# friendlymatthew/heif

Hardware: NVIDIA B200
Metric: decoded MP/s (12MP HEIC grid batch) (higher is better)
Workload: dtype u8

## Files before the change

### heif_b200/csrc/cuda/cabac_kernel.cu

```cuda
#include <cuda_runtime.h>

#include <cstdio>
#include <cstdlib>

#include "cabac_parse.cuh"
#include "kernels.h"

namespace heic {
namespace dev {

#if !defined(__CUDA_ARCH__)
extern __shared__ __align__(16) unsigned char heic_cabac_smem[];
#endif

namespace {

constexpr int kMaxRows = 512;
#ifndef HEIC_CABAC_MIN_CTAS
#define HEIC_CABAC_MIN_CTAS 3
#endif

struct CtaShared {
  CabacTabs tabs;
  alignas(16) Arenas arenas;
  int progress[kMaxRows];
  int aborted[32];
  unsigned group_slot[4];
};

static_assert(offsetof(CtaShared, arenas) == kSmemArenasOff, "Parser::arenas() expects the arena pointers right behind the tables");
constexpr size_t kCtaSharedBytes = (sizeof(CtaShared) + 15) & ~(size_t)15;
template <int TILES>
struct ColdBytes {
  static constexpr size_t value = (size_t)Parser<TILES>::CW_COUNT * (TILES == 32 ? 1024 : 64);
};

template <int TILES>
struct SmemSync {
  static constexpr int kSaveStride = 1;
  uint32_t lane, tile;
  int base;
  int use1;

  __device__ __forceinline__ CtaShared* sh() const { return reinterpret_cast<CtaShared*>(heic_cabac_smem); }
  __device__ __forceinline__ volatile int* progress() const { return sh()->progress; }
  __device__ __forceinline__ volatile int* aborted() const { return &sh()->aborted[TILES == 1 ? 0 : lane]; }

  __device__ __forceinline__ bool wait(int row, int n) {
    unsigned ns = 32;
    volatile int* pr = progress();
    if (TILES == 1) {
      while (pr[row] < base + n && *aborted() != use1) {
        __nanosleep(ns);
        if (ns < 2048) ns *= 2;
      }
    } else {
      __syncwarp();
      while (pr[row] < base + n) {
#pragma unroll
        for (int i = 0; i < 16; i++) __nanosleep(2048);
      }
      __syncwarp();
    }
    __threadfence_block();
    return *aborted() != use1;
  }
  __device__ __forceinline__ void publish(int row, int n) {
    __threadfence_block();
    if (TILES == 1) {
      progress()[row] = base + n;
    } else {
      __syncwarp();
      if (lane == 0) progress()[row] = base + n;
    }
  }
  __device__ __forceinline__ uint8_t* save_area(int row) {
    const Arenas& A = sh()->arenas;
    return A.wpp_save + A.tiles[tile].wpp_off + (size_t)row * NUM_CTX_PAD;
  }
  __device__ __forceinline__ void abort(int code) {
    if (code != -100) atomicCAS(&sh()->arenas.status[tile].code, 0, code);
    *aborted() = use1;
    __threadfence_block();
  }
};

}

template <int TILES>
__global__ void __launch_bounds__(TILES == 32 ? 256 : 512, TILES == 32 ? HEIC_CABAC_MIN_CTAS : 1) cabac_kernel(Arenas A, const CabacTabs* __restrict__ gtabs,
                                                    const uint32_t* __restrict__ order, int n_slots, uint32_t n_groups,
                                                    uint32_t* group_counter) {
  extern __shared__ __align__(16) unsigned char smem_raw[];
  CtaShared* sh = reinterpret_cast<CtaShared*>(smem_raw);
  uint8_t* ctx_all = smem_raw + kCtaSharedBytes + ColdBytes<TILES>::value;

  {
    const uint32_t* src = reinterpret_cast<const uint32_t*>(gtabs);
    uint32_t* dst = reinterpret_cast<uint32_t*>(&sh->tabs);
    for (int i = threadIdx.x; i < (int)(sizeof(CabacTabs) / 4); i += blockDim.x) dst[i] = src[i];
    for (int i = threadIdx.x; i < kMaxRows; i += blockDim.x) sh->progress[i] = 0;
    if (threadIdx.x < 32) sh->aborted[threadIdx.x] = 0;
    if (threadIdx.x < 4) sh->group_slot[threadIdx.x] = 0;
    if (threadIdx.x == 0) sh->arenas = A;
  }
  __syncthreads();

  const int slot = threadIdx.x >> 5, lane = threadIdx.x & 31;
  if (TILES == 1 && lane != 0) return;
  for (int use = 0;; use++) {
  uint32_t group = blockIdx.x;
  if (group_counter) {
    uint32_t g = 0;
    if (lane == 0) {
      volatile unsigned* gs = &sh->group_slot[use & 3];
      const unsigned tag = ((unsigned)(use + 1) & 0x7ffu) << 20;
      for (;;) {
        const unsigned e = *gs;
        if ((e & 0x7ff00000u) == tag) {
          if ((e & 0xfffffu) != 0xfffffu) {
            g = e & 0xfffffu;
            break;
          }
          __nanosleep(64);
        } else if (atomicCAS(const_cast<unsigned*>(gs), e, tag | 0xfffffu) == e) {
          g = min(atomicAdd(group_counter, 1u), 0xffffeu);
          *gs = tag | g;
          __threadfence_block();
          break;
        }
      }
    }
    group = __shfl_sync(0xffffffffu, g, 0);
    if (group >= n_groups) break;
  } else if (use > 0) {
    break;
  }
  const uint32_t my = order[group * TILES + (TILES == 1 ? 0 : lane)];
  const bool active = my != 0xffffffffu;
  const uint32_t tile = active ? my : order[group * TILES];
  const TileParams* tp = A.tiles + tile;
  const PicParams* pp = A.pics + tp->pic;

  Parser<TILES> P;
  P.sm = (uint32_t)__cvta_generic_to_shared(smem_raw);
  P.ctx_off = P.sm + (uint32_t)(kCtaSharedBytes + ColdBytes<TILES>::value) + (uint32_t)slot * NUM_CTX_PAD * TILES + (TILES == 1 ? 0u : (uint32_t)lane);
  P.cold_off = P.sm + (uint32_t)kCtaSharedBytes + (TILES == 32 ? threadIdx.x * 4u : (uint32_t)slot * 4u);
  asm volatile("" : "+r"(P.sm), "+r"(P.ctx_off), "+r"(P.cold_off));
  P.cold(Parser<TILES>::CW_TP_LO) = (int)(uint32_t)(unsigned long long)tp;
  P.cold(Parser<TILES>::CW_TP_HI) = (int)(uint32_t)((unsigned long long)tp >> 32);
  P.cold(Parser<TILES>::CW_PP_LO) = (int)(uint32_t)(unsigned long long)pp;
  P.cold(Parser<TILES>::CW_PP_HI) = (int)(uint32_t)((unsigned long long)pp >> 32);
  P.e.data = A.bitstream + tp->bs_off;
  P.err = active ? 0 : -100;

  SmemSync<TILES> sync;
  sync.lane = (uint32_t)lane;
  sync.tile = tile;
  sync.base = use << 12;
  sync.use1 = use + 1;
  if (!active) *sync.aborted() = use + 1;

#if HEIC_CABAC_TRACE
  unsigned long long t_begin;
  asm volatile("mov.u64 %0, %%globaltimer;" : "=l"(t_begin));
#endif
  const uint32_t ctus = parse_rows<TILES>(P, A.substreams + tp->sub_first, slot, n_slots, sync);
#if HEIC_CABAC_TRACE
  {
    unsigned long long t_end;
    asm volatile("mov.u64 %0, %%globaltimer;" : "=l"(t_end));
    const unsigned bins_w = __reduce_add_sync(0xffffffffu, active ? P.e.bins : 0u);
    if (lane == 0) printf("CT %u %u %d %d %llu %llu %u %u\n", blockIdx.x, group, use, slot, t_begin, t_end, bins_w, tp->bs_len);
  }
#endif
  if (active) {
    atomicAdd(&A.status[tile].bins, P.e.bins);
    atomicAdd(&A.status[tile].ctus, ctus);
  }
  }
}

size_t cabac_smem_bytes(int tiles_per_cta, int n_slots) {
  return kCtaSharedBytes + (tiles_per_cta == 32 ? ColdBytes<32>::value : ColdBytes<1>::value) + (size_t)n_slots * NUM_CTX_PAD * tiles_per_cta;
}

cudaError_t launch_cabac(const Arenas& A, const CabacTabs* tabs, const uint32_t* order, uint32_t n_groups,
                         int tiles_per_cta, int n_slots, uint32_t* group_counter, int n_sm, int resident_ctas, cudaStream_t stream) {
  if (!n_groups) return cudaSuccess;
  static const size_t pad = []() { const char* e = getenv("HEIC_B200_CABAC_SMEM_PAD"); return e ? (size_t)atol(e) : (size_t)0; }();
  const size_t smem = cabac_smem_bytes(tiles_per_cta, n_slots) + pad;
  const int threads = 32 * n_slots;
  if (tiles_per_cta == 32) {
    {
      cudaError_t e = cudaFuncSetAttribute(cabac_kernel<32>, cudaFuncAttributeMaxDynamicSharedMemorySize, 200 * 1024);
      if (e != cudaSuccess) return e;
    }
    const uint32_t resident = resident_ctas > 0 ? (uint32_t)resident_ctas : (uint32_t)n_sm * (uint32_t)(HEIC_CABAC_MIN_CTAS * 8 / n_slots);
    if (group_counter && n_groups > resident && n_groups < 0xffff0u)
      cabac_kernel<32><<<resident, threads, smem, stream>>>(A, tabs, order, n_slots, n_groups, group_counter);
    else
      cabac_kernel<32><<<n_groups, threads, smem, stream>>>(A, tabs, order, n_slots, n_groups, nullptr);
  } else {
    cabac_kernel<1><<<n_groups, threads, smem, stream>>>(A, tabs, order, n_slots, n_groups, nullptr);
  }
  return cudaGetLastError();
}

}
}
```

### heif_b200/csrc/cuda/deblock_kernel.cu

```cuda
#include <cuda_runtime.h>

#include "kernels.h"

namespace heic {
namespace dev {

namespace {

__device__ const uint8_t kBetaTable[52] = {0,  0,  0,  0,  0,  0,  0,  0,  0,  0,  0,  0,  0,  0,  0,  0,  6,  7,
                                           8,  9,  10, 11, 12, 13, 14, 15, 16, 17, 18, 20, 22, 24, 26, 28, 30, 32,
                                           34, 36, 38, 40, 42, 44, 46, 48, 50, 52, 54, 56, 58, 60, 62, 64};
__device__ const uint8_t kTcTable[54] = {0, 0, 0, 0, 0, 0, 0, 0, 0, 0, 0,  0,  0,  0,  0,  0,  0,  0,
                                         1, 1, 1, 1, 1, 1, 1, 1, 1, 2, 2,  2,  2,  3,  3,  3,  3,  4,
                                         4, 4, 5, 5, 6, 6, 7, 8, 9, 10, 11, 13, 14, 16, 18, 20, 22, 24};
__device__ const uint8_t kChromaQp[14] = {29, 30, 31, 32, 33, 33, 34, 34, 35, 35, 36, 36, 37, 37};

__device__ __forceinline__ int clip3(int lo, int hi, int v) { return min(hi, max(lo, v)); }
__device__ __forceinline__ int clip8(int v) { return min(255, max(0, v)); }

__device__ __forceinline__ uint32_t interleave4(uint32_t v) {
  v &= 0x0fu;
  v = (v | (v << 2)) & 0x33u;
  v = (v | (v << 1)) & 0x55u;
  return v;
}

struct Pic {
  const uint32_t* tu_map;
  const uint8_t* qp_map;
  int w8, log2_ctb, wctb;
};

__device__ __forceinline__ bool is_tu_edge(const Pic& p, int x, int y, int pos) {
  const int ctb4 = 1 << (p.log2_ctb - 2);
  const int rx = x >> p.log2_ctb, ry = y >> p.log2_ctb;
  const uint32_t z = interleave4((uint32_t)(x >> 2) & (ctb4 - 1)) | (interleave4((uint32_t)(y >> 2) & (ctb4 - 1)) << 1);
  const uint32_t* tu = p.tu_map + (size_t)(ry * p.wctb + rx) * (ctb4 * ctb4);
  const uint32_t w3 = tu[z & ~63u], w2 = tu[z & ~15u];
  const bool in32 = (w3 & 7u) == (TU_ORIGIN | (3u << 1)) && (pos & 31) != 0;
  const bool in16 = (w2 & 7u) == (TU_ORIGIN | (2u << 1)) && (pos & 15) != 0;
  return !(in32 || in16);
}
__device__ __forceinline__ int qp_at(const Pic& p, int x, int y) { return p.qp_map[(y >> 3) * p.w8 + (x >> 3)]; }

__device__ __forceinline__ int dp4(uint32_t samples, uint32_t weights, int acc) {
  int d;
  asm("dp4a.u32.s32 %0, %1, %2, %3;" : "=r"(d) : "r"(samples), "r"(weights), "r"(acc));
  return d;
}
__host__ __device__ constexpr uint32_t W(int a, int b, int c, int d) {
  return ((uint32_t)a & 0xffu) | (((uint32_t)b & 0xffu) << 8) | (((uint32_t)c & 0xffu) << 16) | (((uint32_t)d & 0xffu) << 24);
}
__device__ __forceinline__ int lin(uint32_t P, uint32_t Q, uint32_t wp, uint32_t wq, int c) { return dp4(Q, wq, dp4(P, wp, c)); }

__device__ __forceinline__ bool filter_luma_segment(uint32_t (&rw)[8][2], int qp_sum, int beta_off2, int tc_off2) {
  const int qpl = (qp_sum + 1) >> 1;
  const int beta = kBetaTable[clip3(0, 51, qpl + beta_off2)];
  const int tc = kTcTable[clip3(0, 53, qpl + 2 + tc_off2)];
  const uint32_t P0 = rw[0][0], Q0 = rw[0][1], P3 = rw[3][0], Q3 = rw[3][1];
  const int dp0 = abs(dp4(P0, W(0, 1, -2, 1), 0)), dp3 = abs(dp4(P3, W(0, 1, -2, 1), 0));
  const int dq0 = abs(dp4(Q0, W(1, -2, 1, 0), 0)), dq3 = abs(dp4(Q3, W(1, -2, 1, 0), 0));
  const int dpq0 = dp0 + dq0, dpq3 = dp3 + dq3, dp = dp0 + dp3, dq = dq0 + dq3;
  if (dpq0 + dpq3 >= beta) return false;
  const int tc25 = (5 * tc + 1) >> 1;
  const bool s0 = 2 * dpq0 < (beta >> 2) && abs(dp4(P0, W(1, 0, 0, -1), 0)) + abs(dp4(Q0, W(1, 0, 0, -1), 0)) < (beta >> 3) &&
                  abs(lin(P0, Q0, W(0, 0, 0, 1), W(-1, 0, 0, 0), 0)) < tc25;
  const bool s3 = 2 * dpq3 < (beta >> 2) && abs(dp4(P3, W(1, 0, 0, -1), 0)) + abs(dp4(Q3, W(1, 0, 0, -1), 0)) < (beta >> 3) &&
                  abs(lin(P3, Q3, W(0, 0, 0, 1), W(-1, 0, 0, 0), 0)) < tc25;
  const bool strong = s0 && s3;
  const bool dep = dp < ((beta + (beta >> 1)) >> 3), deq = dq < ((beta + (beta >> 1)) >> 3);
#pragma unroll
  for (int l = 0; l < 4; l++) {
    const uint32_t P = rw[l][0], Q = rw[l][1];
    if (strong) {
      const int t2 = 2 * tc;
      const int e_p0 = clip3(-t2, t2, lin(P, Q, W(0, 1, 2, 2 - 8), W(2, 1, 0, 0), 4) >> 3);
      const int e_p1 = clip3(-t2, t2, lin(P, Q, W(0, 1, 1 - 4, 1), W(1, 0, 0, 0), 2) >> 2);
      const int e_p2 = clip3(-t2, t2, lin(P, Q, W(2, 3 - 8, 1, 1), W(1, 0, 0, 0), 4) >> 3);
      const int e_q0 = clip3(-t2, t2, lin(P, Q, W(0, 0, 1, 2), W(2 - 8, 2, 1, 0), 4) >> 3);
      const int e_q1 = clip3(-t2, t2, lin(P, Q, W(0, 0, 0, 1), W(1, 1 - 4, 1, 0), 2) >> 2);
      const int e_q2 = clip3(-t2, t2, lin(P, Q, W(0, 0, 0, 1), W(1, 1, 3 - 8, 2), 4) >> 3);
      rw[l][0] = P + (uint32_t)e_p2 * 256u + (uint32_t)e_p1 * 65536u + (uint32_t)e_p0 * 16777216u;
      rw[l][1] = Q + (uint32_t)e_q0 + (uint32_t)e_q1 * 256u + (uint32_t)e_q2 * 65536u;
    } else {
      int delta = lin(P, Q, W(0, 0, 3, -9), W(9, -3, 0, 0), 8) >> 4;
      if (abs(delta) < tc * 10) {
        delta = clip3(-tc, tc, delta);
        const int p0 = dp4(P, W(0, 0, 0, 1), 0), q0 = dp4(Q, W(1, 0, 0, 0), 0);
        const int ep = clip8(p0 + delta) - p0, eq = clip8(q0 - delta) - q0;
        uint32_t addp = (uint32_t)ep * 16777216u, addq = (uint32_t)eq;
        if (dep) {
          const int p1 = dp4(P, W(0, 0, 1, 0), 0);
          const int e = clip3(-(tc >> 1), tc >> 1, (((dp4(P, W(0, 1, 0, 1), 1) >> 1) - p1 + delta) >> 1));
          addp += (uint32_t)(clip8(p1 + e) - p1) * 65536u;
        }
        if (deq) {
          const int q1 = dp4(Q, W(0, 1, 0, 0), 0);
          const int e = clip3(-(tc >> 1), tc >> 1, (((dp4(Q, W(1, 0, 1, 0), 1) >> 1) - q1 - delta) >> 1));
          addq += (uint32_t)(clip8(q1 + e) - q1) * 256u;
        }
        rw[l][0] = P + addp;
        rw[l][1] = Q + addq;
      }
    }
  }
  return true;
}

__device__ __forceinline__ bool filter_chroma_segment(uint32_t (&rw)[8][2], int qp_sum, int c_qp_off, int tc_off2) {
  const int qpi = ((qp_sum + 1) >> 1) + c_qp_off;
  const int qpc = qpi < 30 ? qpi : (qpi >= 43 ? qpi - 6 : kChromaQp[qpi - 30]);
  const int tc = kTcTable[clip3(0, 53, qpc + 2 + tc_off2)];
  if (!tc) return false;
#pragma unroll
  for (int l = 0; l < 4; l++) {
    const uint32_t P = rw[l][0], Q = rw[l][1];
    const int delta = clip3(-tc, tc, lin(P, Q, W(0, 0, 1, -4), W(4, -1, 0, 0), 4) >> 3);
    const int p0 = dp4(P, W(0, 0, 0, 1), 0), q0 = dp4(Q, W(1, 0, 0, 0), 0);
    rw[l][0] = P + (uint32_t)(clip8(p0 + delta) - p0) * 16777216u;
    rw[l][1] = Q + (uint32_t)(clip8(q0 - delta) - q0);
  }
  return true;
}

__device__ __forceinline__ void transpose4(uint32_t a, uint32_t b, uint32_t c, uint32_t d, uint32_t& o0, uint32_t& o1, uint32_t& o2, uint32_t& o3) {
  const uint32_t t0 = __byte_perm(a, b, 0x5140), t1 = __byte_perm(c, d, 0x5140);
  const uint32_t t2 = __byte_perm(a, b, 0x7362), t3 = __byte_perm(c, d, 0x7362);
  o0 = __byte_perm(t0, t1, 0x5410);
  o1 = __byte_perm(t0, t1, 0x7632);
  o2 = __byte_perm(t2, t3, 0x5410);
  o3 = __byte_perm(t2, t3, 0x7632);
}
__device__ __forceinline__ void transpose_cell(uint32_t (&rw)[8][2]) {
  uint32_t t[8][2];
  transpose4(rw[0][0], rw[1][0], rw[2][0], rw[3][0], t[0][0], t[1][0], t[2][0], t[3][0]);
  transpose4(rw[4][0], rw[5][0], rw[6][0], rw[7][0], t[0][1], t[1][1], t[2][1], t[3][1]);
  transpose4(rw[0][1], rw[1][1], rw[2][1], rw[3][1], t[4][0], t[5][0], t[6][0], t[7][0]);
  transpose4(rw[4][1], rw[5][1], rw[6][1], rw[7][1], t[4][1], t[5][1], t[6][1], t[7][1]);
#pragma unroll
  for (int r = 0; r < 8; r++) rw[r][0] = t[r][0], rw[r][1] = t[r][1];
}

template <int CIDX>
__device__ __forceinline__ void deblock_cell(const Pic& pic, uint8_t* plane, int pitch, int pw, int ph, int k, int j,
                                             int beta_off2, int tc_off2, int c_qp_off) {
  constexpr int SUB = CIDX ? 1 : 0;
  const int x0 = 8 * k - 4, y0 = 8 * j - 4;
  const bool has_left = k > 0, has_right = 8 * k < pw, has_top = j > 0, has_bottom = 8 * j < ph;
  uint32_t rw[8][2];
#pragma unroll
  for (int r = 0; r < 8; r++) {
    const bool row_ok = r < 4 ? has_top : has_bottom;
    rw[r][0] = rw[r][1] = 0;
    if (row_ok) {
      const uint8_t* row = plane + (size_t)(y0 + r) * pitch;
      if (has_left) rw[r][0] = *reinterpret_cast<const uint32_t*>(row + x0);
      if (has_right) rw[r][1] = *reinterpret_cast<const uint32_t*>(row + x0 + 4);
    }
  }
  const int xe = (8 * k) << SUB, ye = (8 * j) << SUB;
  uint32_t seg_do = 0, seg_qp = 0;
#pragma unroll
  for (int g = 0; g < 4; g++) {
    const bool vert = g < 2;
    const int half = g & 1;
    bool ok;
    if (vert) ok = has_left && has_right && (half == 0 ? has_top : has_bottom);
    else ok = has_top && has_bottom && (half == 0 ? has_left : has_right);
    if (ok) {
      const int xl = vert ? xe : (x0 + 4 * half) << SUB, yl = vert ? (y0 + 4 * half) << SUB : ye;
      seg_qp |= (uint32_t)(qp_at(pic, xl, yl) + (vert ? qp_at(pic, xl - 1, yl) : qp_at(pic, xl, yl - 1))) << (8 * g);
      seg_do |= (is_tu_edge(pic, xl, yl, vert ? xl : yl) ? 1u : 0u) << g;
    }
  }
  if (!seg_do) return;
  bool changed = false;
#pragma unroll 1
  for (int g = 0; g < 4; g++) {
    if ((seg_do >> g) & 1u) {
      const int qp_sum = (int)((seg_qp >> (8 * g)) & 0xffu);
      changed |= CIDX == 0 ? filter_luma_segment(rw, qp_sum, beta_off2, tc_off2) : filter_chroma_segment(rw, qp_sum, c_qp_off, tc_off2);
    }
#pragma unroll
    for (int r = 0; r < 4; r++) {
      uint32_t t0 = rw[r][0], t1 = rw[r][1];
      rw[r][0] = rw[r + 4][0], rw[r][1] = rw[r + 4][1];
      rw[r + 4][0] = t0, rw[r + 4][1] = t1;
    }
    if (g & 1) transpose_cell(rw);
  }
  if (!changed) return;
#pragma unroll
  for (int r = 0; r < 8; r++) {
    const bool row_ok = r < 4 ? has_top : has_bottom;
    if (!row_ok) continue;
    uint8_t* row = plane + (size_t)(y0 + r) * pitch;
    if (has_left) *reinterpret_cast<uint32_t*>(row + x0) = rw[r][0];
    if (has_right) *reinterpret_cast<uint32_t*>(row + x0 + 4) = rw[r][1];
  }
}

#ifndef HEIC_DEBLOCK_MIN_CTAS
#define HEIC_DEBLOCK_MIN_CTAS 12
#endif
template <int KIND>
__global__ void __launch_bounds__(128, HEIC_DEBLOCK_MIN_CTAS) deblock_kernel(Arenas A, uint32_t blocks_per_tile) {
  const uint32_t tile = blockIdx.x / blocks_per_tile;
  const TileParams* tp = A.tiles + tile;
  const PicParams* pp = A.pics + tp->pic;
  if (A.status[tile].code != 0 || tp->deblock_disabled) return;
  if (KIND == 1 && !pp->chroma) return;
  uint32_t g = (blockIdx.x % blocks_per_tile) * blockDim.x + threadIdx.x;
  const int pw = pp->w >> KIND, ph = pp->h >> KIND;
  const uint32_t cx = (uint32_t)((pw + 7) >> 3) + 1, cy = (uint32_t)((ph + 7) >> 3) + 1;
  int cidx = KIND;
  if (g >= cx * cy) {
    if (KIND == 0) return;
    g -= cx * cy;
    cidx = 2;
    if (g >= cx * cy) return;
  }
  const int k = (int)(g % cx), j = (int)(g / cx);
  if (8 * k - 4 >= pw || 8 * j - 4 >= ph) return;
  Pic pic;
  pic.tu_map = A.tu_map + tp->tu_off;
  pic.qp_map = A.qp_map + tp->map8_off;
  pic.w8 = pp->w8;
  pic.log2_ctb = pp->log2_ctb;
  pic.wctb = pp->wctb;
  const int beta_off2 = tp->beta_offset_div2 * 2, tc_off2 = tp->tc_offset_div2 * 2;
  deblock_cell<KIND>(pic, A.recon + tp->plane_off[cidx], KIND ? pp->pitch_c : pp->pitch_y, pw, ph, k, j, beta_off2, tc_off2,
                     cidx == 0 ? 0 : (cidx == 1 ? pp->pps_cb_qp_offset : pp->pps_cr_qp_offset));
}

}

cudaError_t launch_deblock(const Arenas& A, uint32_t max_w, uint32_t max_h, cudaStream_t stream) {
  if (!A.n_tiles) return cudaSuccess;
  const uint32_t cells_y = (((max_w + 7) >> 3) + 1) * (((max_h + 7) >> 3) + 1);
  const uint32_t cells_c = 2 * ((((max_w >> 1) + 7) >> 3) + 1) * ((((max_h >> 1) + 7) >> 3) + 1);
  const uint32_t by = (cells_y + 127) / 128, bc = (cells_c + 127) / 128;
  deblock_kernel<0><<<A.n_tiles * by, 128, 0, stream>>>(A, by);
  deblock_kernel<1><<<A.n_tiles * bc, 128, 0, stream>>>(A, bc);
  return cudaGetLastError();
}

}
}
```

### heif_b200/csrc/cuda/intra_kernel.cu

```cuda
#include <cuda_runtime.h>

#include "kernels.h"

namespace heic {
namespace dev {

namespace {

__constant__ int8_t kIntraPredAngle[35] = {0,   0,   32,  26,  21,  17, 13, 9,  5,  2,  0,  -2, -5, -9, -13, -17, -21, -26,
                                               -32, -26, -21, -17, -13, -9, -5, -2, 0,  2,  5,  9,  13, 17, 21,  26,  32};
__constant__ int16_t kInvAngle[15] = {-4096, -1638, -910, -630, -482, -390, -315, -256,
                                          -315,  -390,  -482, -630, -910, -1638, -4096};

__device__ __forceinline__ uint32_t compact1(uint32_t v) {
  v &= 0x55u;
  v = (v | (v >> 1)) & 0x33u;
  v = (v | (v >> 2)) & 0x0fu;
  return v;
}
__device__ __forceinline__ int clip8(int v) { return min(255, max(0, v)); }

__device__ __forceinline__ void cp_async16s(uint32_t smem_addr, const void* gmem_src) {
  asm volatile("cp.async.cg.shared.global [%0], [%1], 16;\n" ::"r"(smem_addr), "l"(gmem_src) : "memory");
}
__device__ __forceinline__ void cp_async_wait_all() { asm volatile("cp.async.wait_all;\n" ::: "memory"); }

template <class T>
struct SP {
  uint32_t a;
  __device__ __forceinline__ operator T*() const { return reinterpret_cast<T*>(__cvta_shared_to_generic(a)); }
  __device__ __forceinline__ T& operator[](int i) const { return reinterpret_cast<T*>(__cvta_shared_to_generic(a))[i]; }
  __device__ __forceinline__ SP operator+(int i) const { return SP{a + (uint32_t)(i * (int)sizeof(T))}; }
  __device__ __forceinline__ int operator-(SP o) const { return (int)(a - o.a) / (int)sizeof(T); }
};
struct Ctu {
  int w, h, ctb, ctb4, x_ctb, y_ctb;
  SP<uint8_t> buf[3];
  int stride[3];
  SP<uint8_t> ref;
  SP<uint8_t> refa;
  SP<int16_t> res[3];
  SP<uint32_t> tuw;
  int lane;
  int strong_flag;
};
constexpr int kRefSpan = 144, kRefaSpan = 104;
constexpr int kApron = 4;

__device__ __forceinline__ uint32_t pack4(int a, int b, int c, int d) {
  return (uint32_t)a | ((uint32_t)b << 8) | ((uint32_t)c << 16) | ((uint32_t)d << 24);
}

__device__ __forceinline__ uint32_t block_availability(const Ctu& c, int sub, int bx, int by, int log2) {
  const int N = 1 << log2;
  const int units = (c.ctb >> sub) >> log2;
  const int cx = bx >> log2, cy = by >> log2;
  const int X0 = (c.x_ctb >> sub) + bx, Y0 = (c.y_ctb >> sub) + by;
  const bool left_ok = X0 > 0, top_ok = Y0 > 0;
  int n_bl = 0, n_tr = 0;
  if (left_ok && __ffs(cx | units) > __ffs(cy + 1)) n_bl = min(N, max(0, (c.h >> sub) - (Y0 + N)));
  if (top_ok && __ffs(cy | units) >= __ffs(cx + 1)) n_tr = min(N, max(0, (c.w >> sub) - (X0 + N)));
  const int lo = left_ok ? N - n_bl : 2 * N + 1;
  const int hi = top_ok ? 3 * N + n_tr : 2 * N - 1;
  return (uint32_t)lo | ((uint32_t)hi << 8);
}

__device__ __forceinline__ void predict_block(const Ctu& c, bool pair, uint8_t* buf, int buf_delta, int stride, int bx, int by,
                                              int log2, int mode, bool cbf_a, bool cbf_b, const int16_t* __restrict__ resid,
                                              int res_delta, int lo, int hi) {
  const int N = 1 << log2, lane = c.lane;
  const int total = 4 * N, cnt = total + 1;
  uint8_t* ref = c.ref;
  if (log2 == 2) {
    const uint8_t* corner = buf + by * stride + bx + kApron - 1;
    int r = 128, r2 = 128;
    if (lane <= 16 && lo <= hi) {
      const int d = min(max(lane, lo), hi) - 8;
      const int off = d <= 0 ? -d * stride : d;
      r = corner[off];
      if (pair) r2 = corner[off + buf_delta];
    }
    const int x = lane & 3, y = (lane >> 2) & 3;
    const bool luma = !pair;
    int v, v2 = 0;
    const int L = __shfl_sync(0xffffffffu, r, 7 - y), T = __shfl_sync(0xffffffffu, r, 9 + x);
    int L2 = 0, T2 = 0;
    if (pair) L2 = __shfl_sync(0xffffffffu, r2, 7 - y), T2 = __shfl_sync(0xffffffffu, r2, 9 + x);
    if (mode == 0) {
      const int tr = __shfl_sync(0xffffffffu, r, 13), bl = __shfl_sync(0xffffffffu, r, 3);
      v = ((3 - x) * L + (x + 1) * tr + (3 - y) * T + (y + 1) * bl + 4) >> 3;
      if (pair) {
        const int tr2 = __shfl_sync(0xffffffffu, r2, 13), bl2 = __shfl_sync(0xffffffffu, r2, 3);
        v2 = ((3 - x) * L2 + (x + 1) * tr2 + (3 - y) * T2 + (y + 1) * bl2 + 4) >> 3;
      }
    } else if (mode == 1) {
      const bool in_sum = (lane >= 4 && lane <= 7) || (lane >= 9 && lane <= 12);
      const unsigned sums = __reduce_add_sync(0xffffffffu, in_sum ? (unsigned)r | ((unsigned)r2 << 16) : 0u);
      const int dc = ((int)(sums & 0xffffu) + 4) >> 3;
      v = dc;
      v2 = ((int)(sums >> 16) + 4) >> 3;
      if (luma) {
        if (y == 0) v = x == 0 ? (L + 2 * dc + T + 2) >> 2 : (T + 3 * dc + 2) >> 2;
        else if (x == 0) v = (L + 3 * dc + 2) >> 2;
      }
    } else {
      const int angle = kIntraPredAngle[mode];
      const bool vertical = mode >= 18;
      const int dir = vertical ? 1 : -1;
      const int t = ((vertical ? y : x) + 1) * angle, fact = t & 31;
      const int t1 = (vertical ? x : y) + (t >> 5) + 1;
      int la = 8 + dir * t1, lb = la + dir;
      if (angle < 0) {
        const int inv = kInvAngle[mode - 11];
        if (t1 < 0) la = 8 - dir * ((t1 * inv + 128) >> 8);
        if (t1 + 1 < 0) lb = 8 - dir * (((t1 + 1) * inv + 128) >> 8);
      }
      const int a = __shfl_sync(0xffffffffu, r, la), b = __shfl_sync(0xffffffffu, r, lb);
      v = ((32 - fact) * a + fact * b + 16) >> 5;
      if (pair) {
        const int a2 = __shfl_sync(0xffffffffu, r2, la), b2 = __shfl_sync(0xffffffffu, r2, lb);
        v2 = ((32 - fact) * a2 + fact * b2 + 16) >> 5;
      } else if (mode == 26 || mode == 10) {
        const int c0 = __shfl_sync(0xffffffffu, r, 8), t1s = __shfl_sync(0xffffffffu, r, 9), l1s = __shfl_sync(0xffffffffu, r, 7);
        if (mode == 26 && x == 0) v = clip8(t1s + ((L - c0) >> 1));
        if (mode == 10 && y == 0) v = clip8(l1s + ((T - c0) >> 1));
      }
    }
    if (lane < 16) {
      uint8_t* o = buf + (by + 1 + y) * stride + bx + kApron + x;
      if (cbf_a) v = clip8(v + (int)resid[lane]);
      o[0] = (uint8_t)v;
      if (pair) {
        if (cbf_b) v2 = clip8(v2 + (int)resid[res_delta + lane]);
        o[buf_delta] = (uint8_t)v2;
      }
    }
    __syncwarp();
    return;
  }
  {
    const uint8_t* corner = buf + by * stride + bx + kApron - 1;
    const int n_ref = pair ? 2 * cnt : cnt;
    const int lo_d = lo - 2 * N, hi_d = hi - 2 * N;
    if (lo > hi) {
      for (int s = lane; s < 2 * kRefSpan; s += 32) ref[s] = 128;
    } else {
#pragma unroll 1
      for (int s = lane - 2 * N; s < n_ref - 2 * N; s += 32) {
        const bool second = s > 2 * N;
        const int ss = second ? s - cnt : s;
        const int d = min(max(ss, lo_d), hi_d);
        const uint8_t* src = corner + (d <= 0 ? -d * stride : d);
        if (second) src += buf_delta;
        ref[(second ? ss + kRefSpan : ss) + 2 * N] = *src;
      }
    }
  }
  __syncwarp();
  const uint8_t* R = ref;
  if (N > 4 && !pair && mode != 1) {
    const int min_dist = min(abs(mode - 26), abs(mode - 10));
    const int thr = N == 8 ? 7 : (N == 16 ? 1 : 0);
    if (min_dist > thr) {
      const bool strong = N == 32 && c.strong_flag && abs((int)ref[64] + ref[128] - 2 * ref[96]) < 8 &&
                          abs((int)ref[64] + ref[0] - 2 * ref[32]) < 8;
      uint8_t* reff = ref + kRefSpan;
#pragma unroll 1
      for (int s = lane; s <= total; s += 32) {
        int v;
        if (s == 0 || s == total) v = ref[s];
        else if (strong) {
          if (s == 64) v = ref[64];
          else if (s < 64) v = (s * ref[64] + (64 - s) * ref[0] + 32) >> 6;
          else v = ((128 - s) * ref[64] + (s - 64) * ref[128] + 32) >> 6;
        } else {
          v = (ref[s - 1] + 2 * ref[s] + ref[s + 1] + 2) >> 2;
        }
        reff[s] = (uint8_t)v;
      }
      __syncwarp();
      R = reff;
    }
  }
  const int quads = (N * N) >> 2;
  const int n_items = pair ? 2 * quads : quads;
  const int lq = log2 - 2;
  const bool edge = !pair && N < 32;
  uint8_t* out = buf + (by + 1) * stride + bx + kApron;
  int dc_pack = 0;
  const int angle = kIntraPredAngle[mode];
  const bool vertical = mode >= 18;
  if (mode == 1) {
    if (lane < N) {
      dc_pack = (int)R[2 * N - 1 - lane] + R[2 * N + 1 + lane];
      if (pair) dc_pack += ((int)R[kRefSpan + 2 * N - 1 - lane] + R[kRefSpan + 2 * N + 1 + lane]) << 16;
    }
#pragma unroll
    for (int o = 16; o; o >>= 1) dc_pack += __shfl_xor_sync(0xffffffffu, dc_pack, o);
  } else if (mode >= 2) {
    const int top_i = angle < 0 ? N : 2 * N;
    const int dir = vertical ? 1 : -1;
#pragma unroll 1
    for (int second = 0; second < (pair ? 2 : 1); second++) {
      const uint8_t* Rp = R + second * kRefSpan + 2 * N;
      uint8_t* ra = c.refa + second * kRefaSpan;
#pragma unroll 1
      for (int i = lane; i <= top_i; i += 32) ra[i] = Rp[dir * i];
      if (angle < 0) {
        const int last = (N * angle) >> 5;
        const int i = -1 - lane;
        if (last < -1 && i >= last) ra[i] = Rp[-dir * ((i * (int)kInvAngle[mode - 11] + 128) >> 8)];
      }
    }
    __syncwarp();
  }
#pragma unroll 1
  for (int q = lane; q < n_items; q += 32) {
    const int second = q >= quads ? 1 : 0, qq = q - second * quads;
    const int y = qq >> lq, x0 = (qq & ((1 << lq) - 1)) << 2;
    const uint8_t* Rp = R + second * kRefSpan + 2 * N;
    int v0, v1, v2, v3;
    if (mode == 0) {
      const int L = Rp[-1 - y], tr = Rp[1 + N], bl = Rp[-1 - N];
      const int a = N - 1 - y, base = (N - 1 - x0) * L + (x0 + 1) * tr + (y + 1) * bl + N, step = tr - L, sh = log2 + 1;
      v0 = (base + a * Rp[1 + x0]) >> sh;
      v1 = (base + step + a * Rp[2 + x0]) >> sh;
      v2 = (base + 2 * step + a * Rp[3 + x0]) >> sh;
      v3 = (base + 3 * step + a * Rp[4 + x0]) >> sh;
    } else if (mode == 1) {
      const int dc = (((dc_pack >> (16 * second)) & 0xffff) + N) >> (log2 + 1);
      v0 = v1 = v2 = v3 = dc;
      if (edge) {
        if (y == 0) {
          v0 = (Rp[1 + x0] + 3 * dc + 2) >> 2;
          v1 = (Rp[2 + x0] + 3 * dc + 2) >> 2;
          v2 = (Rp[3 + x0] + 3 * dc + 2) >> 2;
          v3 = (Rp[4 + x0] + 3 * dc + 2) >> 2;
          if (x0 == 0) v0 = (Rp[-1] + 2 * dc + Rp[1] + 2) >> 2;
        } else if (x0 == 0) {
          v0 = (Rp[-1 - y] + 3 * dc + 2) >> 2;
        }
      }
    } else {
      const uint8_t* ra = c.refa + second * kRefaSpan;
      if (vertical) {
        const int t = (y + 1) * angle, fact = t & 31;
        const uint8_t* r5 = ra + x0 + (t >> 5) + 1;
        const int a0 = r5[0], a1 = r5[1], a2 = r5[2], a3 = r5[3], a4 = r5[4];
        v0 = ((32 - fact) * a0 + fact * a1 + 16) >> 5;
        v1 = ((32 - fact) * a1 + fact * a2 + 16) >> 5;
        v2 = ((32 - fact) * a2 + fact * a3 + 16) >> 5;
        v3 = ((32 - fact) * a3 + fact * a4 + 16) >> 5;
        if (edge && mode == 26 && x0 == 0) v0 = clip8(Rp[1] + ((Rp[-1 - y] - Rp[0]) >> 1));
      } else {
        const uint8_t* ry = ra + y + 1;
        int t = (x0 + 1) * angle;
        v0 = ((32 - (t & 31)) * ry[t >> 5] + (t & 31) * ry[(t >> 5) + 1] + 16) >> 5;
        t += angle;
        v1 = ((32 - (t & 31)) * ry[t >> 5] + (t & 31) * ry[(t >> 5) + 1] + 16) >> 5;
        t += angle;
        v2 = ((32 - (t & 31)) * ry[t >> 5] + (t & 31) * ry[(t >> 5) + 1] + 16) >> 5;
        t += angle;
        v3 = ((32 - (t & 31)) * ry[t >> 5] + (t & 31) * ry[(t >> 5) + 1] + 16) >> 5;
        if (edge && mode == 10 && y == 0) {
          const int l1 = Rp[-1], c0 = Rp[0];
          v0 = clip8(l1 + ((Rp[1 + x0] - c0) >> 1));
          v1 = clip8(l1 + ((Rp[2 + x0] - c0) >> 1));
          v2 = clip8(l1 + ((Rp[3 + x0] - c0) >> 1));
          v3 = clip8(l1 + ((Rp[4 + x0] - c0) >> 1));
        }
      }
    }
    if (second ? cbf_b : cbf_a) {
      const uint2 r = *reinterpret_cast<const uint2*>(resid + second * res_delta + (qq << 2));
      v0 = clip8(v0 + (int)(int16_t)(r.x & 0xffffu));
      v1 = clip8(v1 + ((int)r.x >> 16));
      v2 = clip8(v2 + (int)(int16_t)(r.y & 0xffffu));
      v3 = clip8(v3 + ((int)r.y >> 16));
    }
    *reinterpret_cast<uint32_t*>(out + second * buf_delta + y * stride + x0) = pack4(v0, v1, v2, v3);
  }
  __syncwarp();
}

struct IntraLayout {
  int res1, res2, tuw, ref, refa, buf0, buf1, buf2;
  int stride_y, stride_c;
  int warp_bytes;
};

#ifndef HEIC_INTRA_MAXNREG
#define HEIC_INTRA_MAXNREG 72
#endif
__global__ void __maxnreg__(HEIC_INTRA_MAXNREG) intra_kernel(Arenas A, const uint32_t* __restrict__ order, int n_slots, IntraLayout L, int clear_coeff) {
  extern __shared__ __align__(16) unsigned char smem_raw[];
  const uint32_t tile = order[blockIdx.x];
  const TileParams* tp = A.tiles + tile;
  const PicParams* pp = A.pics + tp->pic;
  if (A.status[tile].code != 0) {
    if (clear_coeff) {
      uint4* z = reinterpret_cast<uint4*>(A.coeff + tp->coeff_off[0]);
      const size_t n16 = (size_t)pp->n_tu * 24 * 2 / 16;
      for (size_t i = threadIdx.x; i < n16; i += blockDim.x) z[i] = make_uint4(0u, 0u, 0u, 0u);
    }
    return;
  }
  const int wctb = pp->wctb, hctb = pp->hctb;
  volatile int* progress = reinterpret_cast<volatile int*>(smem_raw);
  const int progress_bytes = n_slots > 1 ? ((hctb * 4 + 15) & ~15) : 0;
  if (n_slots > 1) {
    for (int i = threadIdx.x; i < hctb; i += blockDim.x) progress[i] = 0;
    __syncthreads();
  }
  const int slot = threadIdx.x >> 5, lane = threadIdx.x & 31;

  Ctu c;
  c.w = pp->w;
  c.h = pp->h;
  c.ctb = 1 << pp->log2_ctb;
  c.ctb4 = c.ctb >> 2;
  c.lane = lane;
  c.strong_flag = pp->strong_intra_smoothing;
  const int n_planes = pp->chroma ? 3 : 1;
  const int n4sq = c.ctb4 * c.ctb4;
  {
    uint32_t wbase = (uint32_t)progress_bytes + (uint32_t)slot * (uint32_t)L.warp_bytes;
    asm volatile("" : "+r"(wbase));
    uint32_t p = (uint32_t)__cvta_generic_to_shared(smem_raw) + wbase;
    asm volatile("" : "+r"(p));
    c.res[0].a = p;
    c.res[1].a = p + (uint32_t)L.res1;
    c.res[2].a = p + (uint32_t)L.res2;
    c.tuw.a = p + (uint32_t)L.tuw;
    c.ref.a = p + (uint32_t)L.ref;
    c.refa.a = p + (uint32_t)L.refa + 32u;
    c.buf[0].a = p + (uint32_t)L.buf0;
    c.buf[1].a = p + (uint32_t)L.buf1;
    c.buf[2].a = p + (uint32_t)L.buf2;
    c.stride[0] = L.stride_y;
    c.stride[1] = c.stride[2] = L.stride_c;
  }
  const uint32_t* tu_map = A.tu_map + tp->tu_off;
  uint8_t* plane[3] = {A.recon + tp->plane_off[0], A.recon + tp->plane_off[1], A.recon + tp->plane_off[2]};
  const int pitch[3] = {pp->pitch_y, pp->pitch_c, pp->pitch_c};

  for (int ry = slot; ry < hctb; ry += n_slots) {
    for (int rx = 0; rx < wctb; rx++) {
      const uint32_t ctb_addr = (uint32_t)(ry * wctb + rx);
      {
        const char* g0 = reinterpret_cast<const char*>(A.coeff + tp->coeff_off[0] + (size_t)ctb_addr * n4sq * 16);
        for (int i = lane * 16; i < n4sq * 32; i += 512) cp_async16s(c.res[0].a + i, g0 + i);
        if (n_planes == 3) {
          const char* g1 = reinterpret_cast<const char*>(A.coeff + tp->coeff_off[1] + (size_t)ctb_addr * n4sq * 4);
          const char* g2 = reinterpret_cast<const char*>(A.coeff + tp->coeff_off[2] + (size_t)ctb_addr * n4sq * 4);
          for (int i = lane * 16; i < n4sq * 8; i += 512) {
            cp_async16s(c.res[1].a + i, g1 + i);
            cp_async16s(c.res[2].a + i, g2 + i);
          }
        }
        const char* gt = reinterpret_cast<const char*>(tu_map + (size_t)ctb_addr * n4sq);
        for (int i = lane * 16; i < n4sq * 4; i += 512) cp_async16s(c.tuw.a + i, gt + i);
      }
      if (n_slots > 1 && ry > 0) {
        const int need = min(rx + 2, wctb);
        if (lane == 0) {
          unsigned ns = 32;
          while (progress[ry - 1] < need) {
            __nanosleep(ns);
            if (ns < 1024) ns *= 2;
          }
        }
        __syncwarp();
        __threadfence_block();
      }
      c.x_ctb = rx * c.ctb;
      c.y_ctb = ry * c.ctb;
#pragma unroll
      for (int pl = 0; pl < 3; pl++) {
        if (pl >= n_planes) break;
        const int sub = pl ? 1 : 0, cs = c.ctb >> sub, st = c.stride[pl];
        uint8_t* b = c.buf[pl];
        if (rx > 0)
          for (int y = lane; y < cs; y += 32) b[(y + 1) * st + kApron - 1] = b[(y + 1) * st + kApron + cs - 1];
        if (ry > 0) {
          const int wp = c.w >> sub, x0 = (c.x_ctb >> sub) - 1, y0 = (c.y_ctb >> sub) - 1;
          const uint8_t* src = plane[pl] + (size_t)y0 * pitch[pl];
          for (int j = lane; j <= cs / 2; j += 32) {
            const int x = x0 - 3 + 4 * j;
            if (x >= 0 && x < wp) *reinterpret_cast<uint32_t*>(b + kApron - 4 + 4 * j) = __ldcg(reinterpret_cast<const uint32_t*>(src + x));
          }
        }
      }
      cp_async_wait_all();
      __syncwarp();
      if (clear_coeff) {
        const uint4 zero = make_uint4(0u, 0u, 0u, 0u);
        char* g0 = reinterpret_cast<char*>(A.coeff + tp->coeff_off[0] + (size_t)ctb_addr * n4sq * 16);
        for (int i = lane * 16; i < n4sq * 32; i += 512) *reinterpret_cast<uint4*>(g0 + i) = zero;
        if (n_planes == 3) {
          char* g1 = reinterpret_cast<char*>(A.coeff + tp->coeff_off[1] + (size_t)ctb_addr * n4sq * 4);
          char* g2 = reinterpret_cast<char*>(A.coeff + tp->coeff_off[2] + (size_t)ctb_addr * n4sq * 4);
          for (int i = lane * 16; i < n4sq * 8; i += 512) {
            *reinterpret_cast<uint4*>(g1 + i) = zero;
            *reinterpret_cast<uint4*>(g2 + i) = zero;
          }
        }
      }
      {
        const int buf_delta = (int)(c.buf[2] - c.buf[1]), res_delta = (int)(c.res[2] - c.res[1]);
#pragma unroll 1
        for (int base = 0; base < n4sq; base += 32) {
          const int idx_l = base + lane;
          const uint32_t wl = idx_l < n4sq ? c.tuw[idx_l] : 0u;
          uint32_t pa = 0, pb = 0, pc = 0;
          if (wl & TU_ORIGIN) {
            const int lg = (int)tu_log2(wl);
            const int bxl = (int)compact1((uint32_t)idx_l) << 2, byl = (int)compact1((uint32_t)idx_l >> 1) << 2;
            pa = (uint32_t)bxl | ((uint32_t)byl << 6) | ((uint32_t)lg << 12) | (tu_luma_mode(wl) << 15) | ((wl & TU_CBF_Y) ? 1u << 21 : 0u);
            pb = block_availability(c, 0, bxl, byl, lg);
            if ((wl & TU_HAS_CHROMA) && n_planes == 3) {
              const int lgc = lg > 2 ? lg - 1 : 2;
              const int bxc = (lg > 2 ? bxl : bxl - 4) >> 1, byc = (lg > 2 ? byl : byl - 4) >> 1;
              pa |= (1u << 22) | ((wl & TU_CBF_CB) ? 1u << 23 : 0u) | ((wl & TU_CBF_CR) ? 1u << 24 : 0u);
              pb |= block_availability(c, 1, bxc, byc, lgc) << 16;
              pc = tu_chroma_mode(wl) | ((uint32_t)bxc << 6) | ((uint32_t)byc << 12) | ((uint32_t)lgc << 18);
            }
          }
          uint32_t todo = __ballot_sync(0xffffffffu, (wl & TU_ORIGIN) != 0);
          while (todo) {
            const int src = __ffs(todo) - 1;
            todo &= todo - 1;
            const uint32_t a = __shfl_sync(0xffffffffu, pa, src), b = __shfl_sync(0xffffffffu, pb, src);
            const uint32_t cc = __shfl_sync(0xffffffffu, pc, src);
            const int idx = base + src;
            const int n_calls = (int)((a >> 22) & 1u) + 1;
#pragma unroll 1
            for (int k = 0; k < n_calls; k++) {
              const bool pr = k != 0;
              const uint32_t geo = pr ? cc >> 6 : a;
              const uint32_t av = pr ? b >> 16 : b;
              predict_block(c, pr, pr ? c.buf[1] : c.buf[0], pr ? buf_delta : 0, pr ? c.stride[1] : c.stride[0], (int)(geo & 63u),
                            (int)((geo >> 6) & 63u), (int)((geo >> 12) & 7u), (int)((pr ? cc : a >> 15) & 63u), ((a >> (pr ? 23 : 21)) & 1u) != 0,
                            pr && ((a >> 24) & 1u), pr ? c.res[1] + (idx >> 2) * 16 : c.res[0] + idx * 16, pr ? res_delta : 0,
                            (int)(av & 0xffu), (int)((av >> 8) & 0xffu));
            }
          }
        }
      }
#pragma unroll
      for (int pl = 0; pl < 3; pl++) {
        if (pl >= n_planes) break;
        const int sub = pl ? 1 : 0, cs = c.ctb >> sub, st = c.stride[pl];
        const int xo = c.x_ctb >> sub, yo = c.y_ctb >> sub;
        const int wv = min(cs, (c.w >> sub) - xo), hv = min(cs, (c.h >> sub) - yo);
        const int lw = pp->log2_ctb - sub - 2;
        const uint8_t* b = c.buf[pl];
        for (int i = lane; i < (hv << lw); i += 32) {
          const int y = i >> lw, xw = (i & ((1 << lw) - 1)) << 2;
          if (xw < wv)
            *reinterpret_cast<uint32_t*>(plane[pl] + (size_t)(yo + y) * pitch[pl] + xo + xw) =
                *reinterpret_cast<const uint32_t*>(b + (y + 1) * st + kApron + xw);
        }
      }
      if (n_slots > 1) {
        __threadfence_block();
        __syncwarp();
        if (lane == 0) progress[ry] = rx + 1;
      } else {
        __syncwarp();
      }
    }
  }
}

IntraLayout intra_layout(int log2_ctb) {
  const int ctb = 1 << log2_ctb, n4 = (ctb >> 2) * (ctb >> 2);
  IntraLayout L;
  int o = n4 * 16 * 2;
  L.res1 = o;
  o += n4 * 4 * 2;
  L.res2 = o;
  o += n4 * 4 * 2;
  L.tuw = o;
  o += n4 * 4;
  L.ref = o;
  o += 2 * kRefSpan;
  L.refa = o;
  o += 2 * kRefaSpan;
  L.stride_y = 2 * ctb + kApron;
  L.stride_c = ctb + kApron;
  L.buf0 = o;
  o += (ctb + 1) * L.stride_y;
  L.buf1 = o;
  o += (ctb / 2 + 1) * L.stride_c;
  L.buf2 = o;
  o += (ctb / 2 + 1) * L.stride_c;
  L.warp_bytes = (o + 15) & ~15;
  return L;
}

}

cudaError_t launch_intra(const Arenas& A, const uint32_t* order, int max_log2_ctb, int max_hctb, int n_slots, bool clear_coeff,
                         cudaStream_t stream) {
  if (!A.n_tiles) return cudaSuccess;
  const IntraLayout L = intra_layout(max_log2_ctb);
  const size_t smem = (n_slots > 1 ? (((size_t)max_hctb * 4 + 15) & ~(size_t)15) : 0) + (size_t)n_slots * L.warp_bytes;
  if (smem > 48 * 1024) {
    cudaError_t e = cudaFuncSetAttribute(intra_kernel, cudaFuncAttributeMaxDynamicSharedMemorySize, (int)smem);
    if (e != cudaSuccess) return e;
  }
  intra_kernel<<<A.n_tiles, 32 * n_slots, smem, stream>>>(A, order, n_slots, L, clear_coeff ? 1 : 0);
  return cudaGetLastError();
}

}
}
```

### heif_b200/csrc/cuda/kernels.h

```cpp
#pragma once
#include <cuda_runtime.h>

#include "dev_types.h"

namespace heic {
namespace dev {

struct CabacTabs;

size_t cabac_smem_bytes(int tiles_per_cta, int n_slots);
cudaError_t launch_cabac(const Arenas& A, const CabacTabs* tabs, const uint32_t* order, uint32_t n_groups,
                         int tiles_per_cta, int n_slots, uint32_t* group_counter, int n_sm, int resident_ctas ,
                         cudaStream_t stream);

cudaError_t launch_unescape(const Arenas& A, TileParams* tiles, uint32_t* substreams, cudaStream_t stream);
cudaError_t launch_transform(const Arenas& A, uint32_t max_tu_per_tile, int max_log2_tb, int n_sm, cudaStream_t stream);
size_t transform_list_layout(size_t total_tu, uint32_t off[LIST_CLASSES]);
int transform_launches(int max_log2_tb);

cudaError_t launch_intra(const Arenas& A, const uint32_t* order, int max_log2_ctb, int max_hctb, int n_slots, bool clear_coeff,
                         cudaStream_t stream);

cudaError_t launch_deblock(const Arenas& A, uint32_t max_w, uint32_t max_h, cudaStream_t stream);

cudaError_t launch_sao(const Arenas& A, uint32_t max_pitch, uint32_t max_h, cudaStream_t stream);
cudaError_t launch_sao_sparse(const Arenas& A, int max_hctb, cudaStream_t stream);

struct ColorJob {
  const uint8_t* planes;
  uint64_t tile_stride;
  uint64_t cb_off, cr_off;
  uint32_t pitch_y, pitch_c;
  uint32_t tile_w, tile_h;
  uint32_t grid_cols, grid_rows;
  uint32_t out_w, out_h;
  uint32_t n_images;
  uint32_t chroma;
  uint32_t full_range, matrix_coeffs;
  uint32_t orientation;
  uint8_t* rgb;
  uint64_t pitch, image_stride;
  uint32_t fused;
  const uint8_t* planes_sao;
  const uint32_t* sao;
  uint32_t sao_stride;
  uint32_t log2_ctb, wctb;
};
struct ColorWindow {
  uint32_t crop_x, crop_y, crop_w, crop_h;
  uint32_t win_x, win_y;
};
cudaError_t launch_color(const ColorJob& job, const ColorWindow& win, cudaStream_t stream);

}
}
```

### heif_b200/csrc/cuda/pipeline.cu

```cuda
#include <cuda_runtime.h>

#include <chrono>
#include <cstdio>
#include <cstdlib>

#include <algorithm>
#include <cstdlib>
#include <cstring>
#include <map>
#include <memory>
#include <string>
#include <tuple>
#include <vector>

#include "../host/capi_common.h"
#include "../host/heic_decoder.h"
#include "cabac_tables.h"
#include "host_params.h"
#include "kernels.h"

using namespace heic;
using namespace heic::dev;

namespace {

[[noreturn]] void cuda_fail(cudaError_t e, const char* what) {
  int code = (e == cudaErrorNoDevice || e == cudaErrorInsufficientDriver || e == cudaErrorInvalidDevice) ? HEIC_E_NO_DEVICE
             : (e == cudaErrorMemoryAllocation)                                                          ? HEIC_E_NOMEM
                                                                                                         : HEIC_E_CUDA;
  bail(code, std::string(what) + ": " + cudaGetErrorString(e));
}
#define CU(call)                               \
  do {                                         \
    cudaError_t e__ = (call);                  \
    if (e__ != cudaSuccess) cuda_fail(e__, #call); \
  } while (0)

struct DevBuf {
  void* p = nullptr;
  size_t cap = 0;
  void ensure(size_t n) {
    if (n <= cap) return;
    if (p) cudaFree(p);
    p = nullptr;
    cap = 0;
    size_t want = n + n / 8 + 256;
    CU(cudaMalloc(&p, want));
    cap = want;
  }
  ~DevBuf() {
    if (p) cudaFree(p);
  }
};
struct PinnedBuf {
  void* p = nullptr;
  size_t cap = 0;
  void ensure(size_t n) {
    if (n <= cap) return;
    if (p) cudaFreeHost(p);
    p = nullptr;
    cap = 0;
    size_t want = n + n / 8 + 256;
    CU(cudaMallocHost(&p, want));
    cap = want;
  }
  ~PinnedBuf() {
    if (p) cudaFreeHost(p);
  }
};

size_t up(size_t v, size_t a) { return (v + a - 1) / a * a; }

int env_int(const char* name, int dflt) {
  const char* s = std::getenv(name);
  return (s && *s) ? std::atoi(s) : dflt;
}

}

struct heic_b200_job {
  heic_b200_ctx* ctx = nullptr;
  heic_tile_status* status = nullptr;
  std::vector<heic_tile_status> local;
  size_t n_tiles = 0;
};

struct PipePending {
  heic_b200_job* job = nullptr;
  size_t tile0 = 0, n_tiles = 0;
  cudaEvent_t ev[5] = {};
  double host_ms = 0;
};

struct heic_b200_ctx {
  int device = 0;
  int n_sm = 148;
  cudaStream_t stream = nullptr;
  CabacTabs* d_tabs = nullptr;
  uint64_t launches = 0;
  int cabac_tiles_per_cta = 32;
  int cabac_slots = 0;
  int low_latency_tiles = 384;
  int cabac_group_factor = 1;
  int intra_slots = 0;
  int intra_single_warp_tiles = 2048;
  int cabac_group_cap_pct = 0;
  int cabac_plain_sort = 0;
  int cabac_resident = 0;
  int cabac_persistent = 1;
  int fuse_sao = 1;
  static constexpr int kPipe = 16;
  int pipe_chunk = 0;
  int pipe_slots = 0;
  cudaEvent_t trace_base = nullptr;
  int pipe_order = 1;
  cudaEvent_t ev_cabac = nullptr, ev_d2h = nullptr;
  bool d2h_recorded = false;
  cudaStream_t pipe_stream[kPipe] = {};
  std::unique_ptr<heic_b200_batch> pipe_batch[kPipe];
  PipePending pipe_pending[kPipe];
  uint32_t pipe_next = 0;
  ~heic_b200_ctx();
};

struct ImageInfo {
  uint32_t first_tile, n_tiles, pic;
  uint32_t grid_rows, grid_cols, out_w, out_h, rot_w, rot_h;
  uint32_t tile_w, tile_h, win_x, win_y;
  uint32_t crop_x, crop_y, crop_w, crop_h, orientation;
  uint32_t full_range, matrix_coeffs;
};

namespace {

struct TileWindow {
  uint32_t x, y, w, h;
};

void image_geometry(const heic_image_desc& im, PicParams& pp, TileWindow& tw, uint32_t& out_w, uint32_t& out_h) {
  if (!im.tiles || im.n_tiles == 0 || im.n_tiles != im.grid_rows * im.grid_cols)
    bail(HEIC_E_INVALID_ARG, "image descriptor: n_tiles must equal grid_rows * grid_cols");
  make_pic_params(im.sps, im.pps, pp);
  tw = {0, 0, (uint32_t)pp.w, (uint32_t)pp.h};
  if (im.sps.conformance_window_flag) {
    const uint64_t sub = pp.chroma ? 2 : 1;
    const uint64_t l = sub * im.sps.conf_win_left_offset, r = sub * im.sps.conf_win_right_offset;
    const uint64_t t = sub * im.sps.conf_win_top_offset, b = sub * im.sps.conf_win_bottom_offset;
    if (l + r >= (uint64_t)pp.w || t + b >= (uint64_t)pp.h) bail(HEIC_E_BITSTREAM, "conformance window is empty");
    tw = {(uint32_t)l, (uint32_t)t, (uint32_t)(pp.w - l - r), (uint32_t)(pp.h - t - b)};
  }
  const uint64_t mosaic_w = (uint64_t)im.grid_cols * tw.w, mosaic_h = (uint64_t)im.grid_rows * tw.h;
  const uint64_t ow = im.output_width ? im.output_width : mosaic_w, oh = im.output_height ? im.output_height : mosaic_h;
  if (ow > mosaic_w || oh > mosaic_h) bail(HEIC_E_BITSTREAM, "grid canvas is larger than the tile mosaic");
  out_w = (uint32_t)ow;
  out_h = (uint32_t)oh;
}

void check_transform(const heic_image_transform& x, uint32_t out_w, uint32_t out_h) {
  if (x.orientation > 7 || !x.crop_w || !x.crop_h || (uint64_t)x.crop_x + x.crop_w > out_w || (uint64_t)x.crop_y + x.crop_h > out_h)
    bail(HEIC_E_INVALID_ARG, "image transform: crop rectangle not inside the canvas, or orientation above 7");
}

std::vector<heic_image_transform> canvas_transforms(const heic_image_desc* imgs, uint32_t n_imgs, int32_t apply_transforms) {
  if (!imgs) bail(HEIC_E_INVALID_ARG, "null argument");
  std::vector<heic_image_transform> x(n_imgs);
  for (uint32_t i = 0; i < n_imgs; i++) {
    PicParams pp;
    TileWindow tw;
    uint32_t ow, oh;
    image_geometry(imgs[i], pp, tw, ow, oh);
    x[i] = {0, 0, ow, oh, apply_transforms ? (imgs[i].rotation_ccw_quarter_turns & 3u) : 0u};
  }
  return x;
}

}

struct CabacClass {
  int n_slots, hctb;
  uint32_t order_off, n_groups, n_tiles;
};

struct heic_b200_batch {
  heic_b200_ctx* ctx = nullptr;
  cudaStream_t stream = nullptr;
  int tiles_per_cta = 32;
  std::vector<PicParams> pics;
  std::vector<ScalingSet> scaling;
  std::vector<TileParams> tiles;
  std::vector<ImageInfo> images;
  std::vector<uint32_t> substreams, order, heavy_first;
  std::vector<CabacClass> classes;
  size_t raw_bytes = 0;
  bool any_plain = false;
  size_t bs_bytes = 0, tu_words = 0, coeff_elems = 0, plane_bytes = 0, map4_bytes = 0, map8_bytes = 0, sao_words = 0, wpp_bytes = 0;
  size_t rgb_pitch = 0, rgb_image_stride = 0;
  uint32_t max_tu = 0, max_w = 0, max_h = 0, max_pitch = 0;
  int max_log2_ctb = 4, max_log2_tb = 2, intra_slots = 1, max_hctb = 1;
  uint32_t stages_run = 0;
  bool final_stale = false;
  bool coeff_clean = false;
  PinnedBuf h_bitstream, h_status, h_params;
  size_t off_sub = 0, off_order = 0, off_heavy = 0, off_pics = 0, off_tiles = 0, off_scaling = 0;
  DevBuf d_bitstream, d_params, d_tu, d_coeff, d_recon, d_final, d_ipm, d_ctd,
      d_qp, d_sao, d_wpp, d_status, d_rgb, d_list, d_list_count, d_raw, d_counters;
  PinnedBuf h_raw;
  uint32_t list_off[LIST_CLASSES] = {};
  Arenas arenas() const {
    Arenas a;
    a.bitstream = (const uint8_t*)d_bitstream.p;
    a.raw = (const uint8_t*)d_raw.p;
    const uint8_t* pb = (const uint8_t*)d_params.p;
    a.substreams = (const uint32_t*)(pb + off_sub);
    a.pics = (const PicParams*)(pb + off_pics);
    a.tiles = (const TileParams*)(pb + off_tiles);
    a.scaling = (const ScalingSet*)(pb + off_scaling);
    a.tu_map = (uint32_t*)d_tu.p;
    a.coeff = (int16_t*)d_coeff.p;
    a.recon = (uint8_t*)d_recon.p;
    a.final_ = (uint8_t*)d_final.p;
    a.ipm = (uint8_t*)d_ipm.p;
    a.ct_depth = (uint8_t*)d_ctd.p;
    a.qp_map = (uint8_t*)d_qp.p;
    a.sao = (uint32_t*)d_sao.p;
    a.wpp_save = (uint8_t*)d_wpp.p;
    a.status = (TileStatusDev*)d_status.p;
    a.n_tiles = (uint32_t)tiles.size();
    a.tu_list = (uint2_t*)d_list.p;
    a.list_count = (uint32_t*)d_list_count.p;
    for (int k = 0; k < LIST_CLASSES; k++) a.list_off[k] = list_off[k];
    return a;
  }
  void load(const heic_image_desc* imgs, const heic_image_transform* xforms, uint32_t n_imgs, bool with_rgb);
  void run(uint32_t mask);
};

heic_b200_ctx::~heic_b200_ctx() {
  if (trace_base) cudaEventDestroy(trace_base);
  if (ev_cabac) cudaEventDestroy(ev_cabac);
  if (ev_d2h) cudaEventDestroy(ev_d2h);
  for (int i = 0; i < kPipe; i++) {
    for (cudaEvent_t e : pipe_pending[i].ev)
      if (e) cudaEventDestroy(e);
    pipe_batch[i].reset();
    if (pipe_stream[i]) cudaStreamDestroy(pipe_stream[i]);
  }
  if (d_tabs) cudaFree(d_tabs);
  if (stream) cudaStreamDestroy(stream);
}

void heic_b200_batch::load(const heic_image_desc* imgs, const heic_image_transform* xforms, uint32_t n_imgs, bool with_rgb) {
  pics.clear();
  scaling.clear();
  tiles.clear();
  images.clear();
  substreams.clear();
  order.clear();
  heavy_first.clear();
  classes.clear();
  raw_bytes = 0;
  any_plain = false;
  bs_bytes = tu_words = coeff_elems = plane_bytes = map4_bytes = map8_bytes = sao_words = wpp_bytes = 0;
  max_tu = max_w = max_h = max_pitch = 0;
  max_log2_ctb = 4;
  max_log2_tb = 2;
  intra_slots = 1;
  max_hctb = 1;
  stages_run = 0;
  size_t max_rgb_rows = 0, max_rgb_pitch = 0, n_tiles_hint = 0;
  for (uint32_t i = 0; i < n_imgs; i++) n_tiles_hint += imgs[i].n_tiles;
  for (uint32_t i = 0; i < n_imgs; i++) {
    const heic_image_desc& im = imgs[i];
    if (!im.tiles || im.n_tiles == 0 || im.n_tiles != im.grid_rows * im.grid_cols)
      bail(HEIC_E_INVALID_ARG, "image descriptor: n_tiles must equal grid_rows * grid_cols");
    PicParams pp;
    TileWindow win;
    uint32_t out_w, out_h;
    image_geometry(im, pp, win, out_w, out_h);
    const heic_image_transform& xf = xforms[i];
    check_transform(xf, out_w, out_h);
    ScalingSet ss;
    build_scaling_set(im.sps, im.pps, ss);
    size_t s = 0;
    for (; s < scaling.size(); s++)
      if (!std::memcmp(&scaling[s], &ss, sizeof ss)) break;
    if (s == scaling.size()) scaling.push_back(ss);
    pp.scaling_set = (int)s;
    if (pics.empty() || std::memcmp(&pics.back(), &pp, sizeof pp)) pics.push_back(pp);
    const uint32_t pic = (uint32_t)pics.size() - 1;
    ImageInfo info;
    info.first_tile = (uint32_t)tiles.size();
    info.n_tiles = im.n_tiles;
    info.pic = pic;
    info.grid_rows = im.grid_rows;
    info.grid_cols = im.grid_cols;
    info.out_w = out_w;
    info.out_h = out_h;
    info.tile_w = win.w;
    info.tile_h = win.h;
    info.win_x = win.x;
    info.win_y = win.y;
    info.crop_x = xf.crop_x;
    info.crop_y = xf.crop_y;
    info.crop_w = xf.crop_w;
    info.crop_h = xf.crop_h;
    info.orientation = xf.orientation;
    info.rot_w = (xf.orientation & 1u) ? xf.crop_h : xf.crop_w;
    info.rot_h = (xf.orientation & 1u) ? xf.crop_w : xf.crop_h;
    info.full_range = im.sps.vui_parameters_present_flag ? im.sps.video_full_range_flag : 0u;
    info.matrix_coeffs = im.sps.vui_parameters_present_flag ? im.sps.matrix_coeffs : 2u;
    images.push_back(info);
    const size_t pitch = up((size_t)info.rot_w * 3, 16);
    max_rgb_pitch = std::max(max_rgb_pitch, pitch);
    max_rgb_rows = std::max(max_rgb_rows, (size_t)info.rot_h);
    const int ctb4 = 1 << (pp.log2_ctb - 2);
    for (uint32_t t = 0; t < im.n_tiles; t++) {
      TileParams tp;
      std::memset(&tp, 0, sizeof tp);
      make_tile_params(pp, im.pps, im.tiles[t], tp);
      tp.pic = pic;
      tp.image = i;
      tp.tile_in_image = t;
      tp.bs_off = (uint32_t)bs_bytes;
      bs_bytes = up(bs_bytes + tp.bs_len + 8, 16);
      tp.escaped = im.tiles[t].escaped ? 1u : 0u;
      if (tp.escaped) {
        tp.raw_off = raw_bytes;
        raw_bytes = up(raw_bytes + tp.bs_len + 8, 16);
      } else {
        any_plain = true;
      }
      if (bs_bytes > 0xfff00000ull) bail(HEIC_E_UNSUPPORTED, "more than 4 GiB of slice data in one batch");
      tp.sub_first = (uint32_t)substreams.size();
      for (uint32_t k = 0; k < tp.n_sub; k++) substreams.push_back(im.tiles[t].header.substream_offset[k]);
      tp.tu_off = tu_words;
      tu_words += (size_t)pp.n_tu;
      tp.coeff_off[0] = coeff_elems;
      tp.coeff_off[1] = tp.coeff_off[0] + (size_t)pp.n_tu * 16;
      tp.coeff_off[2] = tp.coeff_off[1] + (size_t)pp.n_tu * 4;
      coeff_elems = tp.coeff_off[2] + (size_t)pp.n_tu * 4;
      const size_t ysz = (size_t)pp.pitch_y * (size_t)pp.h, csz = (size_t)pp.pitch_c * (size_t)(pp.h >> 1);
      tp.plane_off[0] = plane_bytes;
      tp.plane_off[1] = tp.plane_off[0] + ysz;
      tp.plane_off[2] = tp.plane_off[1] + csz;
      plane_bytes = up(tp.plane_off[2] + csz, 256);
      tp.map4_off = map4_bytes;
      map4_bytes = up(map4_bytes + (size_t)pp.w4 * pp.h4, 64);
      tp.map8_off = map8_bytes;
      map8_bytes = up(map8_bytes + (size_t)pp.w8 * pp.h8, 64);
      tp.sao_off = sao_words;
      sao_words += (size_t)pp.wctb * pp.hctb * 4;
      tp.wpp_off = wpp_bytes;
      wpp_bytes += (size_t)pp.hctb * NUM_CTX_PAD;
      tiles.push_back(tp);
      (void)ctb4;
    }
    max_tu = std::max(max_tu, (uint32_t)pp.n_tu);
    max_w = std::max(max_w, (uint32_t)pp.w);
    max_h = std::max(max_h, (uint32_t)pp.h);
    max_pitch = std::max(max_pitch, (uint32_t)pp.pitch_y);
    max_log2_ctb = std::max(max_log2_ctb, pp.log2_ctb);
    max_log2_tb = std::max(max_log2_tb, pp.log2_max_tb);
    max_hctb = std::max(max_hctb, pp.hctb);
    intra_slots = std::max(intra_slots, std::min(8, std::min(pp.hctb, (pp.wctb + 1) / 2 + 1)));
  }
  rgb_pitch = max_rgb_pitch;
  rgb_image_stride = up(max_rgb_pitch * max_rgb_rows, 256);
  if (tiles.size() >= (1u << 24)) bail(HEIC_E_UNSUPPORTED, "more than 2^24 tiles in one batch (the transform lists keep the tile index in 24 bits)");

  tiles_per_cta = (ctx->cabac_tiles_per_cta == 32 && n_tiles_hint > (size_t)ctx->low_latency_tiles) ? 32 : 1;
  const int tpc = tiles_per_cta;
  std::vector<uint64_t> fingerprint(tiles.size(), 0);
  {
    size_t t = 0;
    for (uint32_t i = 0; i < n_imgs; i++)
      for (uint32_t k = 0; k < imgs[i].n_tiles; k++, t++) {
        const uint8_t* p = imgs[i].tiles[k].rbsp;
        const size_t len = imgs[i].tiles[k].rbsp_len;
        uint64_t h = 0x9e3779b97f4a7c15ull ^ len;
        if (len >= 8)
          for (int q = 0; q < 4; q++) {
            uint64_t w8;
            std::memcpy(&w8, p + (len - 8) * q / 3, 8);
            h = (h ^ w8) * 0xbf58476d1ce4e5b9ull;
            h ^= h >> 29;
          }
        fingerprint[t] = h;
      }
  }
  std::map<std::tuple<int, int, int, int>, std::vector<uint32_t>> by_shape;
  for (uint32_t t = 0; t < tiles.size(); t++) {
    const PicParams& pp = pics[tiles[t].pic];
    by_shape[std::make_tuple(pp.wpp, pp.wctb, pp.hctb, pp.log2_ctb)].push_back(t);
  }
  for (auto& kv : by_shape) {
    std::vector<uint32_t>& v = kv.second;
    std::stable_sort(v.begin(), v.end(), [&](uint32_t a, uint32_t b) {
      return tiles[a].bs_len != tiles[b].bs_len ? tiles[a].bs_len > tiles[b].bs_len : fingerprint[a] < fingerprint[b];
    });
    const int wpp = std::get<0>(kv.first), wctb = std::get<1>(kv.first), hctb = std::get<2>(kv.first);
    CabacClass c;
    c.n_slots = wpp ? std::max(1, std::min(hctb, (wctb + 1) / 2)) : 1;
    if (ctx->cabac_slots > 0 && wpp) c.n_slots = std::min(hctb, ctx->cabac_slots);
    c.n_slots = std::min(c.n_slots, tpc == 32 ? 8 : 16);
    c.order_off = (uint32_t)order.size();
    c.n_groups = 0;
    if (tpc == 1) {
      for (uint32_t t : v) order.push_back(t);
      c.n_groups = (uint32_t)v.size();
    } else {
      if (ctx->cabac_group_factor == 1) {
        struct Run {
          size_t first, left;
        };
        std::vector<Run> runs;
        for (size_t i = 0; i < v.size();) {
          size_t j = i + 1;
          while (!ctx->cabac_plain_sort && j < v.size() && tiles[v[j]].bs_len == tiles[v[i]].bs_len && fingerprint[v[j]] == fingerprint[v[i]]) j++;
          runs.push_back({i, j - i});
          i = j;
        }
        uint64_t cap = ~0ull;
        if (ctx->cabac_group_cap_pct > 0) {
          uint64_t total = 0;
          for (uint32_t t : v) total += tiles[t].bs_len;
          cap = total / (uint64_t)(ctx->n_sm * 3) * (uint64_t)ctx->cabac_group_cap_pct / 100u;
        }
        size_t head = 0;
        while (head < runs.size()) {
          int n = 0;
          uint64_t wsum = 0;
          for (size_t r = head; r < runs.size() && n < tpc; r++) {
            if (!runs[r].left) continue;
            if (n > 0 && wsum + tiles[v[runs[r].first]].bs_len > cap) break;
            wsum += tiles[v[runs[r].first]].bs_len;
            order.push_back(v[runs[r].first++]);
            runs[r].left--;
            n++;
          }
          while (head < runs.size() && !runs[head].left) head++;
          if (!n) break;
          for (; n < tpc; n++) order.push_back(0xffffffffu);
          c.n_groups++;
        }
      } else {
        uint64_t total = 0;
        for (uint32_t t : v) total += tiles[t].bs_len;
        const uint64_t target_groups = std::max<uint64_t>(1, (uint64_t)ctx->cabac_group_factor * ((v.size() + tpc - 1) / tpc));
        const uint64_t w_target = std::max<uint64_t>(1, total / target_groups);
        size_t i = 0;
        while (i < v.size()) {
          uint64_t wsum = 0;
          int n = 0;
          while (i < v.size() && n < tpc && (n == 0 || wsum + tiles[v[i]].bs_len <= w_target)) {
            wsum += tiles[v[i]].bs_len;
            order.push_back(v[i]);
            i++;
            n++;
          }
          for (; n < tpc; n++) order.push_back(0xffffffffu);
          c.n_groups++;
        }
      }
    }
    c.hctb = hctb;
    c.n_tiles = (uint32_t)v.size();
    classes.push_back(c);
  }

  heavy_first.resize(tiles.size());
  for (uint32_t t = 0; t < tiles.size(); t++) heavy_first[t] = t;
  std::stable_sort(heavy_first.begin(), heavy_first.end(), [&](uint32_t a, uint32_t b) { return tiles[a].bs_len > tiles[b].bs_len; });

  cudaStream_t st = stream;
  if (any_plain) h_bitstream.ensure(bs_bytes + 16);
  if (raw_bytes) h_raw.ensure(raw_bytes + 16);
  {
    size_t t = 0;
    uint8_t* hb = (uint8_t*)h_bitstream.p;
    uint8_t* hr = (uint8_t*)h_raw.p;
    for (uint32_t i = 0; i < n_imgs; i++)
      for (uint32_t k = 0; k < imgs[i].n_tiles; k++, t++) {
        const size_t len = imgs[i].tiles[k].rbsp_len;
        if (tiles[t].escaped) {
          std::memcpy(hr + tiles[t].raw_off, imgs[i].tiles[k].rbsp, len);
          std::memset(hr + tiles[t].raw_off + len, 0, up(len + 8, 16) - len);
          continue;
        }
        std::memcpy(hb + tiles[t].bs_off, imgs[i].tiles[k].rbsp, len);
        const size_t end = tiles[t].bs_off + len;
        const size_t next = t + 1 < tiles.size() ? tiles[t + 1].bs_off : bs_bytes + 16;
        std::memset(hb + end, 0, next - end);
      }
  }
  off_sub = 0;
  off_order = up(off_sub + substreams.size() * 4, 256);
  off_heavy = up(off_order + order.size() * 4, 256);
  off_pics = up(off_heavy + heavy_first.size() * 4, 256);
  off_tiles = up(off_pics + pics.size() * sizeof(PicParams), 256);
  off_scaling = up(off_tiles + tiles.size() * sizeof(TileParams), 256);
  const size_t params_bytes = up(off_scaling + scaling.size() * sizeof(ScalingSet), 256);
  h_params.ensure(params_bytes);
  {
    uint8_t* hp = (uint8_t*)h_params.p;
    std::memcpy(hp + off_sub, substreams.data(), substreams.size() * 4);
    std::memcpy(hp + off_order, order.data(), order.size() * 4);
    std::memcpy(hp + off_heavy, heavy_first.data(), heavy_first.size() * 4);
    std::memcpy(hp + off_pics, pics.data(), pics.size() * sizeof(PicParams));
    std::memcpy(hp + off_tiles, tiles.data(), tiles.size() * sizeof(TileParams));
    std::memcpy(hp + off_scaling, scaling.data(), scaling.size() * sizeof(ScalingSet));
  }
  d_bitstream.ensure(bs_bytes + 16);
  d_params.ensure(params_bytes);
  d_tu.ensure(tu_words * 4);
  if (tu_words >= (1ull << 31)) bail(HEIC_E_UNSUPPORTED, "batch too large: more than 2^31 4x4 blocks in one load");
  d_list.ensure(transform_list_layout(tu_words, list_off) * sizeof(uint2_t));
  d_list_count.ensure(LIST_CLASSES * LIST_COUNT_STRIDE * sizeof(uint32_t));
  if (coeff_elems * 2 > d_coeff.cap) coeff_clean = false;
  d_coeff.ensure(coeff_elems * 2);
  d_recon.ensure(plane_bytes);
  d_final.ensure(plane_bytes);
  d_ipm.ensure(map4_bytes);
  d_ctd.ensure(map8_bytes);
  d_qp.ensure(map8_bytes);
  d_sao.ensure(sao_words * 4);
  d_wpp.ensure(wpp_bytes);
  d_status.ensure(tiles.size() * sizeof(TileStatusDev));
  h_status.ensure(tiles.size() * sizeof(TileStatusDev));
  if (with_rgb) d_rgb.ensure(rgb_image_stride * images.size());
  d_raw.ensure(raw_bytes ? raw_bytes + 16 : 0);
  if (any_plain) CU(cudaMemcpyAsync(d_bitstream.p, h_bitstream.p, bs_bytes + 16, cudaMemcpyHostToDevice, st));
  if (raw_bytes) CU(cudaMemcpyAsync(d_raw.p, h_raw.p, raw_bytes + 16, cudaMemcpyHostToDevice, st));
  CU(cudaMemcpyAsync(d_params.p, h_params.p, params_bytes, cudaMemcpyHostToDevice, st));
}

void heic_b200_batch::run(uint32_t mask) {
  cudaStream_t st = stream;
  const Arenas A = arenas();
  if (!A.n_tiles) return;
  if (mask & HEIC_STAGE_CABAC) {
    CU(cudaMemsetAsync(d_tu.p, 0, tu_words * 4, st));
    if (!coeff_clean) CU(cudaMemsetAsync(d_coeff.p, 0, coeff_elems * 2, st));
    coeff_clean = false;
    CU(cudaMemsetAsync(d_status.p, 0, tiles.size() * sizeof(TileStatusDev), st));
    CU(cudaMemsetAsync(d_sao.p, 0, sao_words * 4, st));
    if (raw_bytes) {
      uint8_t* pb = (uint8_t*)d_params.p;
      CU(launch_unescape(A, (TileParams*)(pb + off_tiles), (uint32_t*)(pb + off_sub), st));
      ctx->launches++;
    }
    constexpr size_t kCounters = 64;
    d_counters.ensure(kCounters * sizeof(uint32_t));
    const bool persistent = ctx->cabac_persistent && classes.size() <= kCounters;
    if (persistent) CU(cudaMemsetAsync(d_counters.p, 0, kCounters * sizeof(uint32_t), st));
    size_t ci = 0;
    for (const CabacClass& c : classes) {
      CU(launch_cabac(A, ctx->d_tabs, (const uint32_t*)((const uint8_t*)d_params.p + off_order) + c.order_off, c.n_groups, tiles_per_cta,
                      c.n_slots, (persistent && c.hctb > c.n_slots) ? (uint32_t*)d_counters.p + ci : nullptr, ctx->n_sm, ctx->cabac_resident, st));
      ctx->launches++;
      ci++;
    }
  }
  if (mask & HEIC_STAGE_TRANSFORM) {
    CU(launch_transform(A, max_tu, max_log2_tb, ctx->n_sm, st));
    ctx->launches += transform_launches(max_log2_tb);
  }
  if (mask & HEIC_STAGE_INTRA) {
    int slots = tiles.size() >= (size_t)ctx->intra_single_warp_tiles ? 1 : intra_slots;
    if (ctx->intra_slots > 0) slots = std::min(ctx->intra_slots, std::max(1, max_hctb));
    CU(launch_intra(A, (const uint32_t*)((const uint8_t*)d_params.p + off_heavy), max_log2_ctb, max_hctb, slots, true, st));
    coeff_clean = true;
    ctx->launches++;
  }
  if (mask & HEIC_STAGE_DEBLOCK) {
    CU(launch_deblock(A, max_w, max_h, st));
    ctx->launches += 2;
  }
  const bool fuse = ctx->fuse_sao && (mask & HEIC_STAGE_SAO) && (mask & HEIC_STAGE_COLOR) && d_rgb.p;
  if ((mask & HEIC_STAGE_SAO) && !fuse) {
    CU(launch_sao(A, max_pitch, max_h, st));
    final_stale = false;
    ctx->launches++;
  }
  if (fuse) {
    CU(launch_sao_sparse(A, max_hctb, st));
    ctx->launches++;
    final_stale = true;
  }
  if ((mask & HEIC_STAGE_COLOR) && d_rgb.p) {
    size_t i = 0;
    while (i < images.size()) {
      size_t j = i + 1;
      auto same = [&](const ImageInfo& a, const ImageInfo& b) {
        return a.pic == b.pic && a.n_tiles == b.n_tiles && a.grid_cols == b.grid_cols && a.out_w == b.out_w &&
               a.out_h == b.out_h && a.tile_w == b.tile_w && a.tile_h == b.tile_h && a.win_x == b.win_x && a.win_y == b.win_y &&
               a.crop_x == b.crop_x && a.crop_y == b.crop_y && a.crop_w == b.crop_w && a.crop_h == b.crop_h &&
               a.orientation == b.orientation && a.full_range == b.full_range && a.matrix_coeffs == b.matrix_coeffs;
      };
      while (j < images.size() && same(images[i], images[j])) j++;
      const ImageInfo& im = images[i];
      const PicParams& pp = pics[im.pic];
      const TileParams& t0 = tiles[im.first_tile];
      ColorJob job;
      job.planes = (const uint8_t*)(fuse ? d_recon.p : d_final.p) + t0.plane_off[0];
      job.fused = fuse ? 1u : 0u;
      job.planes_sao = (const uint8_t*)d_final.p + t0.plane_off[0];
      job.sao = A.sao + t0.sao_off;
      job.sao_stride = (uint32_t)((size_t)pp.wctb * pp.hctb * 4);
      job.log2_ctb = (uint32_t)pp.log2_ctb;
      job.wctb = (uint32_t)pp.wctb;
      job.tile_stride = im.n_tiles > 1 || j - i > 1
                            ? (size_t)(tiles[std::min<size_t>(im.first_tile + 1, tiles.size() - 1)].plane_off[0] - t0.plane_off[0])
                            : 0;
      job.cb_off = t0.plane_off[1] - t0.plane_off[0];
      job.cr_off = t0.plane_off[2] - t0.plane_off[0];
      job.pitch_y = (uint32_t)pp.pitch_y;
      job.pitch_c = (uint32_t)pp.pitch_c;
      job.tile_w = im.tile_w;
      job.tile_h = im.tile_h;
      job.grid_cols = im.grid_cols;
      job.grid_rows = im.grid_rows;
      job.out_w = im.out_w;
      job.out_h = im.out_h;
      job.n_images = (uint32_t)(j - i);
      job.chroma = (uint32_t)pp.chroma;
      job.full_range = im.full_range;
      job.matrix_coeffs = im.matrix_coeffs;
      job.orientation = im.orientation;
      job.rgb = (uint8_t*)d_rgb.p + i * rgb_image_stride;
      job.pitch = rgb_pitch;
      job.image_stride = rgb_image_stride;
      const ColorWindow win = {im.crop_x, im.crop_y, im.crop_w, im.crop_h, im.win_x, im.win_y};
      CU(launch_color(job, win, st));
      ctx->launches++;
      i = j;
    }
  }
  stages_run |= mask;
}

namespace {

void collect_status(heic_b200_batch* b, heic_tile_status* status) {
  cudaStream_t st = b->stream;
  const size_t n = b->tiles.size();
  CU(cudaMemcpyAsync(b->h_status.p, b->d_status.p, n * sizeof(TileStatusDev), cudaMemcpyDeviceToHost, st));
  CU(cudaStreamSynchronize(st));
  const TileStatusDev* s = (const TileStatusDev*)b->h_status.p;
  for (size_t i = 0; i < n; i++) {
    status[i].code = s[i].code;
    status[i].bins_decoded = s[i].bins;
    status[i].ctus_decoded = s[i].ctus;
    status[i].reserved = 0;
  }
}

}

extern "C" {

int32_t heic_b200_create(int32_t device, heic_b200_ctx** out_ctx) {
  return static_cast<int32_t>(guard([&]() -> int64_t {
    if (!out_ctx) bail(HEIC_E_INVALID_ARG, "null argument");
    *out_ctx = nullptr;
    int n = 0;
    cudaError_t e = cudaGetDeviceCount(&n);
    if (e != cudaSuccess || n == 0)
      bail(HEIC_E_NO_DEVICE, std::string("no CUDA device (this library has no CPU path): ") + cudaGetErrorString(e));
    auto c = std::make_unique<heic_b200_ctx>();
    if (device < 0) CU(cudaGetDevice(&c->device));
    else c->device = device;
    CU(cudaSetDevice(c->device));
    cudaDeviceProp prop;
    CU(cudaGetDeviceProperties(&prop, c->device));
    if (prop.major < 10)
      bail(HEIC_E_NO_DEVICE, std::string("device '") + prop.name + "' is not sm_100 class; the kernels are built for sm_100a only");
    CU(cudaDeviceGetAttribute(&c->n_sm, cudaDevAttrMultiProcessorCount, c->device));
    CU(cudaStreamCreateWithFlags(&c->stream, cudaStreamNonBlocking));
    static CabacTabs tabs;
    build_cabac_tabs(tabs);
    CU(cudaMalloc((void**)&c->d_tabs, sizeof(CabacTabs)));
    CU(cudaMemcpy(c->d_tabs, &tabs, sizeof tabs, cudaMemcpyHostToDevice));
    c->cabac_tiles_per_cta = env_int("HEIC_B200_CABAC_TILES_PER_CTA", 32) == 1 ? 1 : 32;
    c->cabac_slots = env_int("HEIC_B200_CABAC_SLOTS", 0);
    c->intra_slots = std::min(8, env_int("HEIC_B200_INTRA_SLOTS", 0));
    c->cabac_group_factor = std::max(1, env_int("HEIC_B200_CABAC_GROUP_FACTOR", 1));
    c->pipe_chunk = std::max(0, env_int("HEIC_B200_PIPE_CHUNK", 0));
    c->low_latency_tiles = env_int("HEIC_B200_LOW_LATENCY_TILES", 384);
    c->fuse_sao = env_int("HEIC_B200_FUSE_SAO", 1) != 0;
    c->cabac_persistent = env_int("HEIC_B200_CABAC_PERSISTENT", 1) != 0;
    c->cabac_resident = std::max(0, env_int("HEIC_B200_CABAC_RESIDENT", 0));
    c->cabac_plain_sort = env_int("HEIC_B200_CABAC_PLAIN_SORT", 0) != 0;
    c->cabac_group_cap_pct = std::max(0, env_int("HEIC_B200_CABAC_GROUP_CAP", 0));
    c->pipe_slots = std::min((int)heic_b200_ctx::kPipe, std::max(0, env_int("HEIC_B200_PIPE_SLOTS", 0)));
    c->pipe_order = env_int("HEIC_B200_PIPE_ORDER", 1) != 0;
    *out_ctx = c.release();
    return 0;
  }));
}

void heic_b200_destroy(heic_b200_ctx* ctx) {
  if (!ctx) return;
  cudaSetDevice(ctx->device);
  if (ctx->stream) cudaStreamSynchronize(ctx->stream);
  delete ctx;
}

uint64_t heic_b200_launch_count(const heic_b200_ctx* ctx) { return ctx ? ctx->launches : 0; }

int32_t heic_b200_batch_create(heic_b200_ctx* ctx, const heic_image_desc* imgs, uint32_t n_imgs, heic_b200_batch** out) {
  return heic_b200_batch_create_ex(ctx, imgs, n_imgs, 0, out);
}

static int64_t batch_create(heic_b200_ctx* ctx, const heic_image_desc* imgs, const heic_image_transform* xforms, uint32_t n_imgs,
                            heic_b200_batch** out) {
  if (!ctx || !imgs || !xforms || !out || !n_imgs) bail(HEIC_E_INVALID_ARG, "null argument");
  *out = nullptr;
  CU(cudaSetDevice(ctx->device));
  auto b = std::make_unique<heic_b200_batch>();
  b->ctx = ctx;
  b->stream = ctx->stream;
  b->load(imgs, xforms, n_imgs, true);
  CU(cudaStreamSynchronize(ctx->stream));
  *out = b.release();
  return 0;
}

int32_t heic_b200_batch_create_ex(heic_b200_ctx* ctx, const heic_image_desc* imgs, uint32_t n_imgs, int32_t apply_transforms,
                                  heic_b200_batch** out) {
  return static_cast<int32_t>(guard([&]() -> int64_t {
    if (!ctx || !imgs || !out || !n_imgs) bail(HEIC_E_INVALID_ARG, "null argument");
    *out = nullptr;
    return batch_create(ctx, imgs, canvas_transforms(imgs, n_imgs, apply_transforms).data(), n_imgs, out);
  }));
}

int32_t heic_b200_batch_create_transformed(heic_b200_ctx* ctx, const heic_image_desc* imgs, const heic_image_transform* xforms,
                                           uint32_t n_imgs, heic_b200_batch** out) {
  return static_cast<int32_t>(guard([&]() -> int64_t { return batch_create(ctx, imgs, xforms, n_imgs, out); }));
}

void heic_b200_batch_destroy(heic_b200_batch* b) {
  if (!b) return;
  cudaSetDevice(b->ctx->device);
  cudaStreamSynchronize(b->stream);
  delete b;
}

int32_t heic_b200_batch_run_stages(heic_b200_batch* b, uint32_t stage_mask) {
  return static_cast<int32_t>(guard([&]() -> int64_t {
    if (!b) bail(HEIC_E_INVALID_ARG, "null batch");
    CU(cudaSetDevice(b->ctx->device));
    b->run(stage_mask & HEIC_STAGE_ALL);
    return 0;
  }));
}

int32_t heic_b200_batch_decode(heic_b200_batch* b) { return heic_b200_batch_run_stages(b, HEIC_STAGE_ALL); }

int32_t heic_b200_batch_sync(heic_b200_batch* b) {
  return static_cast<int32_t>(guard([&]() -> int64_t {
    if (!b) bail(HEIC_E_INVALID_ARG, "null batch");
    CU(cudaStreamSynchronize(b->stream));
    return 0;
  }));
}

void* heic_b200_batch_stream(heic_b200_batch* b) { return b ? (void*)b->stream : nullptr; }

int32_t heic_b200_batch_rgb(heic_b200_batch* b, void** dev_ptr, size_t* pitch, size_t* image_stride) {
  if (!b) {
    set_last_error("null batch");
    return HEIC_E_INVALID_ARG;
  }
  if (dev_ptr) *dev_ptr = b->d_rgb.p;
  if (pitch) *pitch = b->rgb_pitch;
  if (image_stride) *image_stride = b->rgb_image_stride;
  return 0;
}

int32_t heic_b200_batch_download_rgb(heic_b200_batch* b, uint8_t* rgb_out, size_t pitch, size_t image_stride) {
  return static_cast<int32_t>(guard([&]() -> int64_t {
    if (!b || !rgb_out) bail(HEIC_E_INVALID_ARG, "null argument");
    CU(cudaSetDevice(b->ctx->device));
    cudaStream_t st = b->stream;
    for (size_t i = 0; i < b->images.size(); i++) {
      const ImageInfo& im = b->images[i];
      if (pitch < (size_t)im.rot_w * 3) bail(HEIC_E_INVALID_ARG, "output pitch smaller than a row of RGB");
      if (b->images.size() > 1 && (size_t)im.rot_h * pitch > image_stride)
        bail(HEIC_E_INVALID_ARG, "image_stride smaller than one image (rows x pitch)");
    }
    for (size_t i = 0; i < b->images.size(); i++) {
      const ImageInfo& im = b->images[i];
      CU(cudaMemcpy2DAsync(rgb_out + i * image_stride, pitch, (const uint8_t*)b->d_rgb.p + i * b->rgb_image_stride,
                           b->rgb_pitch, (size_t)im.rot_w * 3, im.rot_h, cudaMemcpyDeviceToHost, st));
    }
    CU(cudaStreamSynchronize(st));
    return 0;
  }));
}

int32_t heic_b200_batch_download_image(heic_b200_batch* b, uint32_t image_index, uint8_t* rgb_out, size_t pitch) {
  return static_cast<int32_t>(guard([&]() -> int64_t {
    if (!b || !rgb_out || image_index >= b->images.size()) bail(HEIC_E_INVALID_ARG, "invalid argument");
    if (!b->d_rgb.p) bail(HEIC_E_INVALID_ARG, "the batch has no RGB output");
    CU(cudaSetDevice(b->ctx->device));
    const ImageInfo& im = b->images[image_index];
    if (pitch < (size_t)im.rot_w * 3) bail(HEIC_E_INVALID_ARG, "output pitch smaller than a row of RGB");
    CU(cudaMemcpy2DAsync(rgb_out, pitch, (const uint8_t*)b->d_rgb.p + (size_t)image_index * b->rgb_image_stride, b->rgb_pitch,
                         (size_t)im.rot_w * 3, im.rot_h, cudaMemcpyDeviceToHost, b->stream));
    CU(cudaStreamSynchronize(b->stream));
    return 0;
  }));
}

int32_t heic_b200_batch_status(heic_b200_batch* b, heic_tile_status* status) {
  return static_cast<int32_t>(guard([&]() -> int64_t {
    if (!b || !status) bail(HEIC_E_INVALID_ARG, "null argument");
    CU(cudaSetDevice(b->ctx->device));
    collect_status(b, status);
    return 0;
  }));
}

uint32_t heic_b200_batch_tile_count(const heic_b200_batch* b) { return b ? (uint32_t)b->tiles.size() : 0; }

size_t heic_b200_batch_cabac_order(const heic_b200_batch* b, uint32_t* out, size_t cap, uint32_t* tiles_per_group) {
  if (!b) return 0;
  if (tiles_per_group) *tiles_per_group = (uint32_t)b->tiles_per_cta;
  if (out)
    for (size_t i = 0; i < b->order.size() && i < cap; i++) out[i] = b->order[i];
  return b->order.size();
}

int32_t heic_b200_batch_dump_tile(heic_b200_batch* b, uint32_t tile_index, heic_tile_dump* dump) {
  return static_cast<int32_t>(guard([&]() -> int64_t {
    if (!b || !dump || tile_index >= b->tiles.size()) bail(HEIC_E_INVALID_ARG, "invalid argument");
    CU(cudaSetDevice(b->ctx->device));
    cudaStream_t st = b->stream;
    CU(cudaStreamSynchronize(st));
    const TileParams& tp = b->tiles[tile_index];
    const PicParams& pp = b->pics[tp.pic];
    if (dump->tu_map) {
      if (dump->tu_map_len < (uint32_t)pp.n_tu) bail(HEIC_E_INVALID_ARG, "tu_map buffer too small");
      CU(cudaMemcpy(dump->tu_map, (const uint32_t*)b->d_tu.p + tp.tu_off, (size_t)pp.n_tu * 4, cudaMemcpyDeviceToHost));
    }
    for (int c = 0; c < (pp.chroma ? 3 : 1); c++)
      if (dump->coeff[c]) {
        const size_t n = (size_t)pp.n_tu * (c ? 4 : 16);
        if (dump->coeff_len[c] < n) bail(HEIC_E_INVALID_ARG, "coefficient buffer too small");
        CU(cudaMemcpy(dump->coeff[c], (const int16_t*)b->d_coeff.p + tp.coeff_off[c], n * 2, cudaMemcpyDeviceToHost));
      }
    if (dump->qp_map) {
      const size_t wq = (size_t)pp.w >> 3, hq = (size_t)pp.h >> 3;
      if (dump->qp_map_len < wq * hq) bail(HEIC_E_INVALID_ARG, "qp_map buffer too small");
      CU(cudaMemcpy2D(dump->qp_map, wq, (const uint8_t*)b->d_qp.p + tp.map8_off, (size_t)pp.w8, wq, hq, cudaMemcpyDeviceToHost));
    }
    if (dump->sao) {
      const size_t n = (size_t)pp.wctb * pp.hctb * 4;
      if (dump->sao_len < n) bail(HEIC_E_INVALID_ARG, "sao buffer too small");
      CU(cudaMemcpy(dump->sao, (const uint32_t*)b->d_sao.p + tp.sao_off, n * 4, cudaMemcpyDeviceToHost));
    }
    if ((b->stages_run & HEIC_STAGE_SAO) && b->final_stale) {
      CU(launch_sao(b->arenas(), b->max_pitch, b->max_h, b->stream));
      CU(cudaStreamSynchronize(b->stream));
      b->final_stale = false;
    }
    const uint8_t* src = (const uint8_t*)((b->stages_run & HEIC_STAGE_SAO) ? b->d_final.p : b->d_recon.p);
    for (int c = 0; c < (pp.chroma ? 3 : 1); c++)
      if (dump->plane[c]) {
        const size_t w = (size_t)pp.w >> (c ? 1 : 0), h = (size_t)pp.h >> (c ? 1 : 0);
        if (dump->plane_len[c] < w * h) bail(HEIC_E_INVALID_ARG, "plane buffer too small");
        CU(cudaMemcpy2D(dump->plane[c], w, src + tp.plane_off[c], (size_t)(c ? pp.pitch_c : pp.pitch_y), w, h,
                        cudaMemcpyDeviceToHost));
      }
    return 0;
  }));
}

static void harvest_slot(heic_b200_ctx* ctx, int slot) {
  PipePending& pd = ctx->pipe_pending[slot];
  if (!pd.job) return;
  heic_b200_batch* b = ctx->pipe_batch[slot].get();
  CU(cudaStreamSynchronize(b->stream));
  if (pd.ev[0] && ctx->trace_base) {
    float t[5];
    for (int k = 0; k < 5; k++) cudaEventElapsedTime(&t[k], ctx->trace_base, pd.ev[k]);
    std::fprintf(stderr, "[heic_b200] chunk slot %2d tiles %6zu: queued %8.1f  h2d %8.1f  cabac %8.1f  kernels %8.1f  d2h %8.1f ms\n", slot,
                 pd.n_tiles, t[0], t[1], t[2], t[3], t[4]);
  }
  const TileStatusDev* s = (const TileStatusDev*)b->h_status.p;
  heic_tile_status* out = pd.job->status + pd.tile0;
  for (size_t i = 0; i < pd.n_tiles; i++) {
    out[i].code = s[i].code;
    out[i].bins_decoded = s[i].bins;
    out[i].ctus_decoded = s[i].ctus;
    out[i].reserved = 0;
  }
  pd.job = nullptr;
}

static heic_b200_job* submit_grids(heic_b200_ctx* ctx, const heic_image_desc* imgs, const heic_image_transform* xforms,
                                   uint32_t n_imgs, uint8_t* rgb_out, size_t pitch, size_t image_stride, uint8_t* y_out,
                                   uint8_t* cb_out, uint8_t* cr_out, heic_tile_status* status) {
  if (!ctx || !imgs || !xforms || !n_imgs) bail(HEIC_E_INVALID_ARG, "null argument");
  CU(cudaSetDevice(ctx->device));
  std::vector<size_t> first_tile(n_imgs + 1, 0), y_off(n_imgs + 1, 0), c_off(n_imgs + 1, 0);
  for (uint32_t i = 0; i < n_imgs; i++) {
    const heic_image_desc& im = imgs[i];
    PicParams pp;
    TileWindow win;
    uint32_t out_w, out_h;
    image_geometry(im, pp, win, out_w, out_h);
    check_transform(xforms[i], out_w, out_h);
    TileParams tp;
    for (uint32_t t = 0; t < im.n_tiles; t++) make_tile_params(pp, im.pps, im.tiles[t], tp);
    const size_t ow = out_w, oh = out_h;
    if (rgb_out) {
      const bool turn = xforms[i].orientation & 1u;
      const size_t rw = turn ? xforms[i].crop_h : xforms[i].crop_w, rh = turn ? xforms[i].crop_w : xforms[i].crop_h;
      if (pitch < rw * 3) bail(HEIC_E_INVALID_ARG, "output pitch smaller than a row of RGB");
      if (n_imgs > 1 && rh * pitch > image_stride) bail(HEIC_E_INVALID_ARG, "image_stride smaller than one image (rows x pitch)");
    }
    first_tile[i + 1] = first_tile[i] + im.n_tiles;
    y_off[i + 1] = y_off[i] + ow * oh;
    c_off[i + 1] = c_off[i] + ((ow + 1) / 2) * ((oh + 1) / 2);
  }
  static const bool trace = std::getenv("HEIC_B200_TRACE") != nullptr;
  static const bool trace2 = trace && std::atoi(std::getenv("HEIC_B200_TRACE")) >= 2;
  using clk = std::chrono::steady_clock;
  auto ms_since = [](clk::time_point t0) { return std::chrono::duration<double, std::milli>(clk::now() - t0).count(); };
  const clk::time_point t_call = clk::now();
  double t_wait = 0, t_load = 0, t_run = 0;
  auto job = std::make_unique<heic_b200_job>();
  job->ctx = ctx;
  job->n_tiles = first_tile[n_imgs];
  job->status = status;
  if (!job->status) {
    job->local.resize(job->n_tiles);
    job->status = job->local.data();
  }
  uint32_t chunk = (uint32_t)std::max(0, ctx->pipe_chunk);
  if (chunk == 0) {
    const uint32_t parts = (n_imgs + 295u) / 296u;
    chunk = (n_imgs + parts - 1) / parts;
  }
  const uint32_t n_slots_use = ctx->pipe_slots > 0 ? (uint32_t)ctx->pipe_slots : std::min(8u, std::max(3u, 900u / chunk));
  std::vector<uint32_t> chunk_start;
  for (uint32_t i = 0; i < n_imgs; i += chunk) chunk_start.push_back(i);
  chunk_start.push_back(n_imgs);
  const uint32_t n_chunks = (uint32_t)chunk_start.size() - 1;
  try {
  for (uint32_t k = 0; k < n_chunks; k++) {
    const int slot = (int)(ctx->pipe_next++ % n_slots_use);
    const uint32_t i0 = chunk_start[k], cnt = chunk_start[k + 1] - i0;
    if (!ctx->pipe_stream[slot]) CU(cudaStreamCreateWithFlags(&ctx->pipe_stream[slot], cudaStreamNonBlocking));
    if (!ctx->pipe_batch[slot]) {
      ctx->pipe_batch[slot] = std::make_unique<heic_b200_batch>();
      ctx->pipe_batch[slot]->ctx = ctx;
      ctx->pipe_batch[slot]->stream = ctx->pipe_stream[slot];
    }
    clk::time_point t0 = clk::now();
    harvest_slot(ctx, slot);
    t_wait += ms_since(t0);
    heic_b200_batch* b = ctx->pipe_batch[slot].get();
    cudaStream_t st = b->stream;
    t0 = clk::now();
    b->load(imgs + i0, xforms + i0, cnt, rgb_out != nullptr);
    t_load += ms_since(t0);
    t0 = clk::now();
    PipePending& pend = ctx->pipe_pending[slot];
    if (trace2) {
      if (!ctx->trace_base) {
        CU(cudaEventCreate(&ctx->trace_base));
        CU(cudaEventRecord(ctx->trace_base, st));
      }
      for (int e = 0; e < 5; e++)
        if (!pend.ev[e]) CU(cudaEventCreate(&pend.ev[e]));
      CU(cudaEventRecord(pend.ev[0], st));
      CU(cudaEventRecord(pend.ev[1], st));
    }
    if (ctx->pipe_order) {
      if (!ctx->ev_cabac) {
        CU(cudaEventCreateWithFlags(&ctx->ev_cabac, cudaEventDisableTiming));
        CU(cudaEventCreateWithFlags(&ctx->ev_d2h, cudaEventDisableTiming));
      } else {
        CU(cudaStreamWaitEvent(st, ctx->ev_cabac, 0));
      }
    }
    b->run(HEIC_STAGE_CABAC);
    if (ctx->pipe_order) CU(cudaEventRecord(ctx->ev_cabac, st));
    if (trace2) CU(cudaEventRecord(pend.ev[2], st));
    b->run((rgb_out ? HEIC_STAGE_ALL : (HEIC_STAGE_ALL & ~HEIC_STAGE_COLOR)) & ~HEIC_STAGE_CABAC);
    if (trace2) CU(cudaEventRecord(pend.ev[3], st));
    if (ctx->pipe_order && ctx->d2h_recorded) CU(cudaStreamWaitEvent(st, ctx->ev_d2h, 0));
    t_run += ms_since(t0);
    if (rgb_out) {
      bool one_copy = image_stride == b->rgb_image_stride && pitch == b->rgb_pitch;
      for (size_t i = 0; i < b->images.size() && one_copy; i++)
        one_copy = (size_t)b->images[i].rot_w * 3 == pitch && (size_t)b->images[i].rot_h * pitch == image_stride;
      if (one_copy) {
        CU(cudaMemcpyAsync(rgb_out + (size_t)i0 * image_stride, b->d_rgb.p, (size_t)cnt * image_stride, cudaMemcpyDeviceToHost, st));
      } else {
        for (size_t i = 0; i < b->images.size(); i++) {
          const ImageInfo& im = b->images[i];
          if (pitch < (size_t)im.rot_w * 3) bail(HEIC_E_INVALID_ARG, "output pitch smaller than a row of RGB");
          CU(cudaMemcpy2DAsync(rgb_out + (i0 + i) * image_stride, pitch, (const uint8_t*)b->d_rgb.p + i * b->rgb_image_stride,
                               b->rgb_pitch, (size_t)im.rot_w * 3, im.rot_h, cudaMemcpyDeviceToHost, st));
        }
      }
    } else {
      for (size_t i = 0; i < b->images.size(); i++) {
        const ImageInfo& im = b->images[i];
        const PicParams& pp = b->pics[im.pic];
        const size_t yo = y_off[i0 + i], co = c_off[i0 + i];
        const size_t cw = (im.out_w + 1) / 2, chh = (im.out_h + 1) / 2;
        const uint8_t* fin = (const uint8_t*)b->d_final.p;
        for (uint32_t t = 0; t < im.n_tiles; t++) {
          const TileParams& tp = b->tiles[im.first_tile + t];
          const size_t tx = (size_t)(t % im.grid_cols) * im.tile_w, ty = (size_t)(t / im.grid_cols) * im.tile_h;
          if (tx >= im.out_w || ty >= im.out_h) continue;
          const size_t w = std::min<size_t>(im.tile_w, im.out_w - tx), h = std::min<size_t>(im.tile_h, im.out_h - ty);
          CU(cudaMemcpy2DAsync(y_out + yo + ty * im.out_w + tx, im.out_w,
                               fin + tp.plane_off[0] + (size_t)im.win_y * pp.pitch_y + im.win_x, pp.pitch_y, w, h,
                               cudaMemcpyDeviceToHost, st));
          if (pp.chroma && cb_out && cr_out) {
            const size_t wc = std::min<size_t>(im.tile_w / 2, cw - tx / 2), hc = std::min<size_t>(im.tile_h / 2, chh - ty / 2);
            const size_t wo = (size_t)(im.win_y / 2) * pp.pitch_c + im.win_x / 2;
            CU(cudaMemcpy2DAsync(cb_out + co + (ty / 2) * cw + tx / 2, cw, fin + tp.plane_off[1] + wo, pp.pitch_c, wc, hc,
                                 cudaMemcpyDeviceToHost, st));
            CU(cudaMemcpy2DAsync(cr_out + co + (ty / 2) * cw + tx / 2, cw, fin + tp.plane_off[2] + wo, pp.pitch_c, wc, hc,
                                 cudaMemcpyDeviceToHost, st));
          }
        }
      }
    }
    CU(cudaMemcpyAsync(b->h_status.p, b->d_status.p, b->tiles.size() * sizeof(TileStatusDev), cudaMemcpyDeviceToHost, st));
    if (ctx->pipe_order) {
      CU(cudaEventRecord(ctx->ev_d2h, st));
      ctx->d2h_recorded = true;
    }
    if (trace2) CU(cudaEventRecord(pend.ev[4], st));
    ctx->pipe_pending[slot].job = job.get();
    ctx->pipe_pending[slot].tile0 = first_tile[i0];
    ctx->pipe_pending[slot].n_tiles = b->tiles.size();
  }
  } catch (...) {
    for (int slot = 0; slot < heic_b200_ctx::kPipe; slot++) {
      if (!ctx->pipe_stream[slot]) continue;
      if (ctx->pipe_pending[slot].job == job.get() || !ctx->pipe_pending[slot].job) cudaStreamSynchronize(ctx->pipe_stream[slot]);
      if (ctx->pipe_pending[slot].job == job.get()) ctx->pipe_pending[slot].job = nullptr;
    }
    throw;
  }
  if (trace)
    std::fprintf(stderr, "[heic_b200] submit %u images: %.1f ms on the host (slot wait %.1f, load %.1f, launch %.1f)\n", n_imgs,
                 ms_since(t_call), t_wait, t_load, t_run);
  return job.release();
}

static int64_t job_wait(heic_b200_job* job) {
  std::unique_ptr<heic_b200_job> owner(job);
  heic_b200_ctx* ctx = job->ctx;
  CU(cudaSetDevice(ctx->device));
  for (int slot = 0; slot < heic_b200_ctx::kPipe; slot++)
    if (ctx->pipe_pending[slot].job == job) harvest_slot(ctx, slot);
  size_t bad = 0;
  for (size_t i = 0; i < job->n_tiles; i++)
    if (job->status[i].code != 0) bad++;
  if (bad) {
    set_last_error(std::to_string(bad) + " tile(s) failed to decode (malformed slice data); see the per-tile status");
    return HEIC_E_BITSTREAM;
  }
  return 0;
}

static int64_t decode_grids_impl(heic_b200_ctx* ctx, const heic_image_desc* imgs, const heic_image_transform* xforms,
                                 uint32_t n_imgs, uint8_t* rgb_out, size_t pitch, size_t image_stride, uint8_t* y_out,
                                 uint8_t* cb_out, uint8_t* cr_out, heic_tile_status* status) {
  return job_wait(submit_grids(ctx, imgs, xforms, n_imgs, rgb_out, pitch, image_stride, y_out, cb_out, cr_out, status));
}

int32_t heic_b200_decode_grids(heic_b200_ctx* ctx, const heic_image_desc* imgs, uint32_t n_imgs, uint8_t* rgb_out,
                               size_t pitch, size_t image_stride, int32_t apply_transforms, heic_tile_status* status) {
  return static_cast<int32_t>(guard([&]() -> int64_t {
    if (!ctx || !rgb_out) bail(HEIC_E_INVALID_ARG, "null argument");
    return decode_grids_impl(ctx, imgs, canvas_transforms(imgs, n_imgs, apply_transforms).data(), n_imgs, rgb_out, pitch,
                             image_stride, nullptr, nullptr, nullptr, status);
  }));
}

int32_t heic_b200_decode_grids_transformed(heic_b200_ctx* ctx, const heic_image_desc* imgs, const heic_image_transform* xforms,
                                           uint32_t n_imgs, uint8_t* rgb_out, size_t pitch, size_t image_stride,
                                           heic_tile_status* status) {
  return static_cast<int32_t>(guard([&]() -> int64_t {
    if (!rgb_out) bail(HEIC_E_INVALID_ARG, "null output buffer");
    return decode_grids_impl(ctx, imgs, xforms, n_imgs, rgb_out, pitch, image_stride, nullptr, nullptr, nullptr, status);
  }));
}

int32_t heic_b200_decode_grids_submit(heic_b200_ctx* ctx, const heic_image_desc* imgs, uint32_t n_imgs, uint8_t* rgb_out,
                                      size_t pitch, size_t image_stride, int32_t apply_transforms, heic_tile_status* status,
                                      heic_b200_job** out_job) {
  return static_cast<int32_t>(guard([&]() -> int64_t {
    if (!ctx || !rgb_out || !out_job) bail(HEIC_E_INVALID_ARG, "null argument");
    *out_job = submit_grids(ctx, imgs, canvas_transforms(imgs, n_imgs, apply_transforms).data(), n_imgs, rgb_out, pitch,
                            image_stride, nullptr, nullptr, nullptr, status);
    return 0;
  }));
}

int32_t heic_b200_decode_grids_submit_transformed(heic_b200_ctx* ctx, const heic_image_desc* imgs,
                                                  const heic_image_transform* xforms, uint32_t n_imgs, uint8_t* rgb_out,
                                                  size_t pitch, size_t image_stride, heic_tile_status* status,
                                                  heic_b200_job** out_job) {
  return static_cast<int32_t>(guard([&]() -> int64_t {
    if (!rgb_out || !out_job) bail(HEIC_E_INVALID_ARG, "null argument");
    *out_job = submit_grids(ctx, imgs, xforms, n_imgs, rgb_out, pitch, image_stride, nullptr, nullptr, nullptr, status);
    return 0;
  }));
}

int32_t heic_b200_job_wait(heic_b200_job* job) {
  return static_cast<int32_t>(guard([&]() -> int64_t {
    if (!job) bail(HEIC_E_INVALID_ARG, "null job");
    return job_wait(job);
  }));
}

int32_t heic_b200_decode_grids_yuv(heic_b200_ctx* ctx, const heic_image_desc* imgs, uint32_t n_imgs, uint8_t* y_out,
                                   uint8_t* cb_out, uint8_t* cr_out, heic_tile_status* status) {
  return static_cast<int32_t>(guard([&]() -> int64_t {
    if (!ctx || !y_out) bail(HEIC_E_INVALID_ARG, "null argument");
    return decode_grids_impl(ctx, imgs, canvas_transforms(imgs, n_imgs, 0).data(), n_imgs, nullptr, 0, 0, y_out, cb_out, cr_out,
                             status);
  }));
}

int32_t heic_b200_decode_file(heic_b200_ctx* ctx, const uint8_t* data, size_t len, uint8_t* rgb_out, size_t pitch,
                              int32_t apply_transforms) {
  return static_cast<int32_t>(guard([&]() -> int64_t {
    if (!ctx || !data || !rgb_out) bail(HEIC_E_INVALID_ARG, "null argument");
    std::unique_ptr<HeicFile> f = HeicDecoder::open(data, len);
    const heic_image_transform xf = apply_transforms ? f->primary.transform : canvas_transforms(&f->primary.desc, 1, 0)[0];
    return decode_grids_impl(ctx, &f->primary.desc, &xf, 1, rgb_out, pitch, 0, nullptr, nullptr, nullptr, nullptr);
  }));
}

int32_t heic_b200_unescape(heic_b200_ctx* ctx, const uint8_t* nal_payload, size_t len, uint32_t slice_data_byte_offset,
                           const uint32_t* substream_offset, uint32_t n_substreams, uint8_t* rbsp_out, size_t* rbsp_len,
                           uint32_t* slice_data_byte_offset_out, uint32_t* substream_offset_out) {
  return static_cast<int32_t>(guard([&]() -> int64_t {
    if (!ctx || !nal_payload || !rbsp_out || !rbsp_len || (n_substreams && (!substream_offset || !substream_offset_out)))
      bail(HEIC_E_INVALID_ARG, "null argument");
    if (len > 0x7fffffffu || slice_data_byte_offset > len) bail(HEIC_E_INVALID_ARG, "payload too large or data offset outside it");
    CU(cudaSetDevice(ctx->device));
    const size_t padded = up(len + 8, 16) + 16;
    DevBuf d_raw, d_out, d_tile, d_sub, d_status;
    d_raw.ensure(padded);
    d_out.ensure(padded);
    d_tile.ensure(sizeof(TileParams));
    d_sub.ensure((size_t)std::max(1u, n_substreams) * 4);
    d_status.ensure(sizeof(TileStatusDev));
    TileParams tp;
    std::memset(&tp, 0, sizeof tp);
    tp.bs_len = (uint32_t)len;
    tp.data_off = slice_data_byte_offset;
    tp.n_sub = n_substreams;
    tp.escaped = 1;
    cudaStream_t st = ctx->stream;
    CU(cudaMemsetAsync(d_raw.p, 0, padded, st));
    CU(cudaMemsetAsync(d_status.p, 0, sizeof(TileStatusDev), st));
    CU(cudaMemcpyAsync(d_raw.p, nal_payload, len, cudaMemcpyHostToDevice, st));
    CU(cudaMemcpyAsync(d_tile.p, &tp, sizeof tp, cudaMemcpyHostToDevice, st));
    if (n_substreams) CU(cudaMemcpyAsync(d_sub.p, substream_offset, (size_t)n_substreams * 4, cudaMemcpyHostToDevice, st));
    Arenas A;
    std::memset(&A, 0, sizeof A);
    A.raw = (const uint8_t*)d_raw.p;
    A.bitstream = (const uint8_t*)d_out.p;
    A.status = (TileStatusDev*)d_status.p;
    A.n_tiles = 1;
    CU(launch_unescape(A, (TileParams*)d_tile.p, (uint32_t*)d_sub.p, st));
    ctx->launches++;
    TileStatusDev sd;
    CU(cudaMemcpyAsync(&tp, d_tile.p, sizeof tp, cudaMemcpyDeviceToHost, st));
    CU(cudaMemcpyAsync(&sd, d_status.p, sizeof sd, cudaMemcpyDeviceToHost, st));
    CU(cudaStreamSynchronize(st));
    if (sd.code != 0) bail(HEIC_E_BITSTREAM, "more emulation prevention bytes in one NAL unit than the GPU path handles");
    *rbsp_len = tp.bs_len;
    if (slice_data_byte_offset_out) *slice_data_byte_offset_out = tp.data_off;
    CU(cudaMemcpy(rbsp_out, d_out.p, tp.bs_len, cudaMemcpyDeviceToHost));
    if (n_substreams) CU(cudaMemcpy(substream_offset_out, d_sub.p, (size_t)n_substreams * 4, cudaMemcpyDeviceToHost));
    return 0;
  }));
}

int32_t heic_b200_color_stitch(heic_b200_ctx* ctx, const void* dev_planes, uint32_t n_images, uint32_t grid_rows,
                               uint32_t grid_cols, uint32_t tile_w, uint32_t tile_h, uint32_t out_w, uint32_t out_h,
                               uint32_t full_range, uint32_t matrix_coeffs, void* dev_rgb, size_t pitch,
                               size_t image_stride) {
  return static_cast<int32_t>(guard([&]() -> int64_t {
    if (!ctx || !dev_planes || !dev_rgb) bail(HEIC_E_INVALID_ARG, "null argument");
    if (!n_images || !grid_rows || !grid_cols || (tile_w & 7) || (tile_h & 1) || !tile_w || !tile_h)
      bail(HEIC_E_INVALID_ARG, "tile width must be a multiple of 8 and tile height even");
    if (out_w > grid_cols * tile_w || out_h > grid_rows * tile_h || pitch < (size_t)out_w * 3)
      bail(HEIC_E_INVALID_ARG, "canvas larger than the tile mosaic, or pitch too small");
    CU(cudaSetDevice(ctx->device));
    ColorJob job;
    job.planes = (const uint8_t*)dev_planes;
    job.fused = 0;
    job.planes_sao = nullptr;
    job.sao = nullptr;
    job.sao_stride = 0;
    job.log2_ctb = job.wctb = 0;
    job.tile_stride = (size_t)tile_w * tile_h * 3 / 2;
    job.cb_off = (size_t)tile_w * tile_h;
    job.cr_off = job.cb_off + (size_t)(tile_w / 2) * (tile_h / 2);
    job.pitch_y = tile_w;
    job.pitch_c = tile_w / 2;
    job.tile_w = tile_w;
    job.tile_h = tile_h;
    job.grid_cols = grid_cols;
    job.grid_rows = grid_rows;
    job.out_w = out_w;
    job.out_h = out_h;
    job.n_images = n_images;
    job.chroma = 1;
    job.full_range = full_range;
    job.matrix_coeffs = matrix_coeffs;
    job.orientation = 0;
    job.rgb = (uint8_t*)dev_rgb;
    job.pitch = pitch;
    job.image_stride = image_stride;
    CU(launch_color(job, ColorWindow{0, 0, out_w, out_h, 0, 0}, ctx->stream));
    ctx->launches++;
    CU(cudaStreamSynchronize(ctx->stream));
    return 0;
  }));
}

}
```

### heif_b200/csrc/cuda/sao_kernel.cu

```cuda
#include <cuda_runtime.h>

#include "kernels.h"
#include "sao_common.cuh"

namespace heic {
namespace dev {

namespace {

using sao::sao8;

__global__ void __launch_bounds__(256) sao_kernel(Arenas A, uint32_t blocks_per_tile) {
  const uint32_t tile = blockIdx.x / blocks_per_tile;
  const TileParams* tp = A.tiles + tile;
  const PicParams* pp = A.pics + tp->pic;
  if (A.status[tile].code != 0) return;
  uint32_t g = (blockIdx.x % blocks_per_tile) * blockDim.x + threadIdx.x;
  const uint32_t gy = (uint32_t)(pp->w + 15) >> 4, gc = (uint32_t)((pp->w >> 1) + 15) >> 4;
  const uint32_t n_y = gy * (uint32_t)pp->h, n_c = pp->chroma ? gc * (uint32_t)(pp->h >> 1) : 0u;
  int cidx = 0;
  if (g >= n_y) {
    g -= n_y;
    cidx = 1;
    if (g >= n_c) {
      g -= n_c;
      cidx = 2;
      if (g >= n_c) return;
    }
  }
  const uint32_t gpr = cidx ? gc : gy;
  const int y = (int)(g / gpr);
  const int sub = cidx ? 1 : 0;
  const int pw = pp->w >> sub, ph = pp->h >> sub, pitch = cidx ? pp->pitch_c : pp->pitch_y;
  const int x = (int)(g % gpr) * 16;
  const uint8_t* src = A.recon + tp->plane_off[cidx];
  uint8_t* dst = A.final_ + tp->plane_off[cidx];
  const uint8_t* row = src + (size_t)y * pitch;
  const int log2_cs = pp->log2_ctb - sub;
  const bool enabled = cidx == 0 ? tp->sao_luma : tp->sao_chroma;
  const uint32_t* sao_row = A.sao + tp->sao_off + (size_t)((y >> log2_cs) * pp->wctb) * 4 + cidx;
  const uint4 center = *reinterpret_cast<const uint4*>(row + x);
  uint32_t lo[2] = {center.x, center.y}, hi[2] = {center.z, center.w};
  if (enabled) {
    const uint32_t w0 = sao_row[(size_t)(x >> log2_cs) * 4];
    if (w0 & 3u) sao8(lo, row, x, y, pw, ph, pitch, w0, (int)(w0 & 3u));
    if (x + 8 < pw) {
      const uint32_t w1 = sao_row[(size_t)((x + 8) >> log2_cs) * 4];
      if (w1 & 3u) sao8(hi, row, x + 8, y, pw, ph, pitch, w1, (int)(w1 & 3u));
    }
  }
  uint8_t* o = dst + (size_t)y * pitch + x;
  if (x + 16 <= pw) {
    *reinterpret_cast<uint4*>(o) = make_uint4(lo[0], lo[1], hi[0], hi[1]);
  } else {
    const int n = pw - x;
    *reinterpret_cast<uint32_t*>(o) = lo[0];
    if (n > 4) *reinterpret_cast<uint32_t*>(o + 4) = lo[1];
    if (n > 8) *reinterpret_cast<uint32_t*>(o + 8) = hi[0];
  }
}

__global__ void __launch_bounds__(128) sao_sparse_kernel(Arenas A, uint32_t max_hctb) {
  const uint32_t tile = blockIdx.x / max_hctb, ry = blockIdx.x % max_hctb;
  const TileParams* tp = A.tiles + tile;
  const PicParams* pp = A.pics + tp->pic;
  if (A.status[tile].code != 0 || ry >= (uint32_t)pp->hctb) return;
  const int lane = threadIdx.x & 31, warp = threadIdx.x >> 5;
  const int n_comp = pp->chroma ? 3 : 1;
  for (int rx = warp; rx < pp->wctb; rx += 4) {
    const uint4 sp = *reinterpret_cast<const uint4*>(A.sao + tp->sao_off + (size_t)(ry * pp->wctb + rx) * 4);
    if (!((sp.x | sp.y | sp.z) & 3u)) continue;
#pragma unroll 1
    for (int c = 0; c < n_comp; c++) {
      const uint32_t word = c == 0 ? sp.x : (c == 1 ? sp.y : sp.z);
      if (!(word & 3u)) continue;
      const int sub = c ? 1 : 0;
      const int cs = 1 << (pp->log2_ctb - sub), pw = pp->w >> sub, ph = pp->h >> sub, pitch = c ? pp->pitch_c : pp->pitch_y;
      const int x_ctb = rx * cs, y_ctb = (int)ry * cs;
      const uint8_t* src = A.recon + tp->plane_off[c];
      uint8_t* dst = A.final_ + tp->plane_off[c];
      const int gpr = cs >> 3;
#pragma unroll 1
      for (int it = lane; it < gpr * cs; it += 32) {
        const int x = x_ctb + (it % gpr) * 8, y = y_ctb + it / gpr;
        if (x >= pw || y >= ph) continue;
        const uint8_t* row = src + (size_t)y * pitch;
        const uint2 in = *reinterpret_cast<const uint2*>(row + x);
        uint32_t o[2] = {in.x, in.y};
        sao8(o, row, x, y, pw, ph, pitch, word, (int)(word & 3u));
        uint8_t* out = dst + (size_t)y * pitch + x;
        *reinterpret_cast<uint32_t*>(out) = o[0];
        if (x + 4 < pw) *reinterpret_cast<uint32_t*>(out + 4) = o[1];
      }
    }
  }
}

}

cudaError_t launch_sao_sparse(const Arenas& A, int max_hctb, cudaStream_t stream) {
  if (!A.n_tiles || max_hctb <= 0) return cudaSuccess;
  sao_sparse_kernel<<<A.n_tiles * (uint32_t)max_hctb, 128, 0, stream>>>(A, (uint32_t)max_hctb);
  return cudaGetLastError();
}

cudaError_t launch_sao(const Arenas& A, uint32_t max_pitch, uint32_t max_h, cudaStream_t stream) {
  if (!A.n_tiles) return cudaSuccess;
  const uint32_t groups = ((max_pitch + 15) / 16) * max_h * 2;
  const uint32_t bpt = (groups + 255) / 256;
  sao_kernel<<<A.n_tiles * bpt, 256, 0, stream>>>(A, bpt);
  return cudaGetLastError();
}

}
}
```

### heif_b200/csrc/cuda/transform_kernel.cu

```cuda
#include <cuda_runtime.h>

#include <algorithm>
#include <cstdlib>

#include "kernels.h"

namespace heic {
namespace dev {

namespace {

__host__ __device__ constexpr int dct_quarter(int m) {
  constexpr int q[33] = {64, 90, 90, 90, 89, 88, 87, 85, 83, 82, 80, 78, 75, 73, 70, 67, 64,
                         61, 57, 54, 50, 46, 43, 38, 36, 31, 25, 22, 18, 13, 9,  4,  0};
  return q[m];
}
__host__ __device__ constexpr int dct32(int k, int n) {
  int m = (k * (2 * n + 1)) & 127;
  return m <= 32 ? dct_quarter(m) : m <= 64 ? -dct_quarter(64 - m) : m < 96 ? -dct_quarter(m - 64) : dct_quarter(128 - m);
}

template <int N, int NZ>
struct Idct {
  static __device__ __forceinline__ void run(const int (&x)[N], int (&y)[N]) {
    constexpr int H = N / 2, HZ = (NZ + 1) / 2;
    int xe[H], e[H];
#pragma unroll
    for (int j = 0; j < H; j++) xe[j] = x[2 * j];
    Idct<H, (HZ < 1 ? 1 : HZ)>::run(xe, e);
#pragma unroll
    for (int k = 0; k < H; k++) {
      int o = 0;
#pragma unroll
      for (int j = 1; j < N; j += 2)
        if (j < NZ) o += dct32(j * (32 / N), k) * x[j];
      y[k] = e[k] + o;
      y[N - 1 - k] = e[k] - o;
    }
  }
};
template <int NZ>
struct Idct<2, NZ> {
  static __device__ __forceinline__ void run(const int (&x)[2], int (&y)[2]) {
    int a = 64 * x[0], b = NZ > 1 ? 64 * x[1] : 0;
    y[0] = a + b;
    y[1] = a - b;
  }
};

__device__ __forceinline__ void dst4(const int (&x)[4], int (&y)[4]) {
  y[0] = 29 * x[0] + 74 * x[1] + 84 * x[2] + 55 * x[3];
  y[1] = 55 * x[0] + 74 * x[1] - 29 * x[2] - 84 * x[3];
  y[2] = 74 * x[0] - 74 * x[2] + 74 * x[3];
  y[3] = 84 * x[0] - 74 * x[1] + 55 * x[2] - 29 * x[3];
}

__device__ __forceinline__ int clip16(int v) { return min(32767, max(-32768, v)); }

template <int N, bool DST>
__device__ __forceinline__ void transform_1d(const int (&x)[N], int (&y)[N], int nz) {
  if (DST) {
    int xx[4] = {x[0], x[1], x[2], x[3]}, yy[4];
    dst4(xx, yy);
#pragma unroll
    for (int i = 0; i < 4; i++) y[i] = yy[i];
  } else if (N >= 16 && nz <= N / 4) {
    Idct<N, (N / 4 < 1 ? 1 : N / 4)>::run(x, y);
  } else if (N >= 8 && nz <= N / 2) {
    Idct<N, N / 2>::run(x, y);
  } else {
    Idct<N, N>::run(x, y);
  }
}

__device__ const uint8_t kLevelScale[6] = {40, 45, 51, 57, 64, 72};
__device__ const uint8_t kChromaQp[14] = {29, 30, 31, 32, 33, 33, 34, 34, 35, 35, 36, 36, 37, 37};

constexpr int kWarpsPerCta = 8;
constexpr int kTmpPerWarp = 32 * 34;

constexpr int kListThreads = 256;
constexpr int kListIter = 4;
constexpr int kListPerCta = 4 * kListThreads * kListIter;

__device__ __forceinline__ uint32_t classify(uint32_t w, bool chroma) {
  uint32_t cy = 7, cb = 7, cr = 7;
  if (w & TU_ORIGIN) {
    const int lg = (int)tu_log2(w);
    if (w & TU_CBF_Y) cy = 5 - lg;
    if (chroma && (lg > 2 || (w & TU_HAS_CHROMA))) {
      const uint32_t cc = lg == 5 ? LIST_16 : lg == 4 ? LIST_8 : LIST_4C;
      if (w & TU_CBF_CB) cb = cc;
      if (w & TU_CBF_CR) cr = cc;
    }
  }
  return cy | (cb << 3) | (cr << 6);
}

#ifndef HEIC_LIST_MIN_CTAS
#define HEIC_LIST_MIN_CTAS 1
#endif
__global__ void __launch_bounds__(kListThreads, HEIC_LIST_MIN_CTAS) tu_list_kernel(Arenas A, uint32_t blocks_per_tile) {
  __shared__ uint32_t cta_cnt[LIST_CLASSES], cta_base[LIST_CLASSES], warp_base[kListThreads / 32][LIST_CLASSES];
  const uint32_t tile = blockIdx.x / blocks_per_tile;
  const uint32_t first = (blockIdx.x % blocks_per_tile) * kListPerCta;
  const TileParams* tp = A.tiles + tile;
  const PicParams* pp = A.pics + tp->pic;
  const int lane = threadIdx.x & 31, warp = threadIdx.x >> 5;
  if (A.status[tile].code != 0 || first >= (uint32_t)pp->n_tu) return;
  if (threadIdx.x < LIST_CLASSES) cta_cnt[threadIdx.x] = 0;
  __syncthreads();
  const bool chroma = pp->chroma != 0;
  uint32_t cls[kListIter][4], w_all[kListIter][4];
  unsigned long long mine = 0;
#pragma unroll
  for (int it = 0; it < kListIter; it++) {
    const uint32_t i0 = first + (uint32_t)it * (4 * kListThreads) + threadIdx.x * 4;
    uint4 wv = make_uint4(0u, 0u, 0u, 0u);
    if (i0 < (uint32_t)pp->n_tu) wv = *reinterpret_cast<const uint4*>(A.tu_map + tp->tu_off + i0);
    const uint32_t w[4] = {wv.x, wv.y, wv.z, wv.w};
#pragma unroll
    for (int e = 0; e < 4; e++) {
      w_all[it][e] = w[e];
      cls[it][e] = 0x1ffu;
      if (w[e]) {
        cls[it][e] = classify(w[e], chroma);
#pragma unroll
        for (int c = 0; c < 3; c++) {
          const uint32_t k = (cls[it][e] >> (3 * c)) & 7u;
          if (k < LIST_CLASSES) mine += 1ull << (12 * k);
        }
      }
    }
  }
  unsigned long long incl = mine;
#pragma unroll
  for (int o = 1; o < 32; o <<= 1) {
    const unsigned long long v = __shfl_up_sync(0xffffffffu, incl, o);
    if (lane >= o) incl += v;
  }
  const unsigned long long total = __shfl_sync(0xffffffffu, incl, 31);
  if (lane < LIST_CLASSES) {
    const uint32_t n = (uint32_t)(total >> (12 * lane)) & 0xfffu;
    warp_base[warp][lane] = n ? atomicAdd(cta_cnt + lane, n) : 0u;
  }
  __syncthreads();
  if (threadIdx.x < LIST_CLASSES)
    cta_base[threadIdx.x] = A.list_off[threadIdx.x] +
                            (cta_cnt[threadIdx.x] ? atomicAdd(A.list_count + threadIdx.x * LIST_COUNT_STRIDE, cta_cnt[threadIdx.x]) : 0u);
  __syncthreads();
  if (!mine) return;
  unsigned long long run = incl - mine;
#pragma unroll
  for (int it = 0; it < kListIter; it++) {
    const uint32_t i0 = first + (uint32_t)it * (4 * kListThreads) + threadIdx.x * 4;
#pragma unroll
    for (int e = 0; e < 4; e++) {
      if (cls[it][e] == 0x1ffu) continue;
#pragma unroll
      for (int c = 0; c < 3; c++) {
        const uint32_t k = (cls[it][e] >> (3 * c)) & 7u;
        if (k < LIST_CLASSES) {
          const uint32_t we = w_all[it][e];
          uint2_t v;
          v.x = tile | (tu_qp(we) << 24) | (tu_tskip(we, c) << 30);
          v.y = (i0 + e) | ((uint32_t)c << 30);
          A.tu_list[(size_t)cta_base[k] + warp_base[warp][k] + ((uint32_t)(run >> (12 * k)) & 0xfffu)] = v;
          run += 1ull << (12 * k);
        }
      }
    }
  }
}

struct Item {
  const PicParams* pp;
  const TileParams* tp;
  int16_t* blk;
  int qp, tskip;
  int cidx;
};
__device__ __forceinline__ Item fetch_item(const Arenas& A, uint2_t it) {
  Item r;
  r.tp = A.tiles + (it.x & 0xffffffu);
  r.pp = A.pics + r.tp->pic;
  const uint32_t entry = it.y & 0x3fffffffu;
  r.cidx = (int)(it.y >> 30);
  r.qp = (int)((it.x >> 24) & 63u);
  r.tskip = (int)((it.x >> 30) & 1u);
  r.blk = A.coeff + r.tp->coeff_off[r.cidx] + (r.cidx ? (size_t)(entry & ~3u) * 4 : (size_t)entry * 16);
  return r;
}
__device__ __forceinline__ int item_scale(const Item& t) {
  int qp = t.qp;
  if (t.cidx) {
    int qpi = qp + (t.cidx == 1 ? t.pp->pps_cb_qp_offset + t.tp->slice_cb_qp_offset : t.pp->pps_cr_qp_offset + t.tp->slice_cr_qp_offset);
    qpi = min(57, max(0, qpi));
    qp = qpi < 30 ? qpi : (qpi >= 43 ? qpi - 6 : kChromaQp[qpi - 30]);
  }
  return (int)kLevelScale[qp % 6] << (qp / 6);
}

template <int N>
__global__ void __launch_bounds__(kWarpsPerCta * 32) transform_kernel(Arenas A, int cls) {
  constexpr int K = 32 / N;
  constexpr int LOG2 = N == 8 ? 3 : N == 16 ? 4 : 5;
  constexpr int S = N + 2;
  __shared__ __align__(16) int16_t tmp_all[kWarpsPerCta][kTmpPerWarp];
  __shared__ int16_t* blk_of[kWarpsPerCta][4];
  const int warp = threadIdx.x >> 5, lane = threadIdx.x & 31;
  const int k = lane / N, col = lane % N;
  const uint32_t count = A.list_count[cls * LIST_COUNT_STRIDE];
  const uint2_t* list = A.tu_list + A.list_off[cls];
  int16_t* tmp = tmp_all[warp];
  int16_t* t = tmp + k * (N * S);
  const uint32_t steps = (count + K - 1) / K;
  for (uint32_t step = blockIdx.x * kWarpsPerCta + warp; step < steps; step += gridDim.x * kWarpsPerCta) {
    const uint32_t idx = step * K + k;
    const bool active = idx < count;
    uint2_t it;
    it.x = it.y = 0;
    if (active) it = list[idx];
    const Item item = fetch_item(A, it);
    int16_t* blk = item.blk;
    if (col == 0) blk_of[warp][k] = blk;
    const bool tskip = active && item.tskip;
    int x[N], y[N];
#pragma unroll
    for (int j = 0; j < N; j++) x[j] = active ? (int)blk[j * N + col] : 0;
    {
      int any_other = 0;
#pragma unroll
      for (int j = 0; j < N; j++) any_other |= (j == 0 && col == 0) ? 0 : x[j];
      if (!__any_sync(0xffffffffu, any_other != 0 || tskip)) {
        int v = 0;
        if (active && col == 0) {
          const int lvl = x[0];
          const int scale = item_scale(item);
          int mf = 16;
          if (item.pp->scaling_enabled) {
            const ScalingSet* sc = A.scaling + item.pp->scaling_set;
            mf = N == 8 ? sc->f8[item.cidx][0] : N == 16 ? sc->f16[item.cidx][0] : sc->f32[item.cidx][0];
          }
          constexpr int BD_SHIFT = LOG2 + 3;
          long long p = ((long long)lvl * (mf * scale) + (1ll << (BD_SHIFT - 1))) >> BD_SHIFT;
          const int dc = (int)min(32767ll, max(-32768ll, p));
          const int t1 = clip16((64 * dc + 64) >> 7);
          v = clip16((64 * t1 + 2048) >> 12);
        }
        v = __shfl_sync(0xffffffffu, v, k * N);
        const uint32_t vv = ((uint32_t)v & 0xffffu) * 0x10001u;
        constexpr int PAIRS = N * N / 2;
        const uint32_t n_active = min((uint32_t)K, count - step * K);
#pragma unroll
        for (int g = 0; g < K; g++) {
          if ((uint32_t)g >= n_active) break;
          const uint32_t vg = __shfl_sync(0xffffffffu, vv, g * N);
          uint4* dst = reinterpret_cast<uint4*>(__shfl_sync(0xffffffffu, (unsigned long long)blk, g * N));
#pragma unroll 4
          for (int q = lane; q < PAIRS / 4; q += 32) dst[q] = make_uint4(vg, vg, vg, vg);
        }
        continue;
      }
    }
    int nz2 = 0;
    constexpr int UNROLL = N == 32 ? 1 : 2;
#pragma unroll UNROLL
    for (int pass = 0; pass < 2; pass++) {
      int nz;
      if (pass == 0) {
        int nz_rows = 0;
#pragma unroll
        for (int j = 0; j < N; j++) nz_rows = x[j] ? j + 1 : nz_rows;
        int nz1 = nz_rows;
#pragma unroll
        for (int o = 16; o; o >>= 1) nz1 = max(nz1, __shfl_xor_sync(0xffffffffu, nz1, o));
        const uint32_t col_mask = __ballot_sync(0xffffffffu, nz_rows > 0);
#pragma unroll
        for (int g = 0; g < K; g++) {
          uint32_t mg = (col_mask >> (g * N)) & (N == 32 ? 0xffffffffu : ((1u << N) - 1u));
          nz2 = max(nz2, 32 - __clz(mg));
        }
        if (active) {
          const int scale = item_scale(item);
          const uint8_t* m = nullptr;
          if (item.pp->scaling_enabled && !tskip) {
            const ScalingSet* sc = A.scaling + item.pp->scaling_set;
            m = N == 8 ? sc->f8[item.cidx] : N == 16 ? sc->f16[item.cidx] : sc->f32[item.cidx];
          }
          constexpr int BD_SHIFT = LOG2 + 3;
#pragma unroll
          for (int j = 0; j < N; j++) {
            if (j < nz1) {
              const int lvl = x[j];
              const int ms = (m ? (int)m[j * N + col] : 16) * scale;
              int v;
              if ((unsigned)(lvl + 255) <= 510u) {
                v = (lvl * ms + (1 << (BD_SHIFT - 1))) >> BD_SHIFT;
              } else {
                long long p = (long long)lvl * ms + (1ll << (BD_SHIFT - 1));
                p >>= BD_SHIFT;
                v = (int)min(32767ll, max(-32768ll, p));
              }
              x[j] = min(32767, max(-32768, v));
            }
          }
        }
        nz = nz1;
      } else {
        const int16_t* row = t + col * S;
#pragma unroll
        for (int j = 0; j < N; j += 2) {
          uint32_t two = *reinterpret_cast<const uint32_t*>(row + j);
          x[j] = (int)(int16_t)(two & 0xffffu);
          x[j + 1] = (int)(int16_t)(two >> 16);
        }
        nz = nz2;
      }
      if (tskip) {
#pragma unroll
        for (int i = 0; i < N; i++) y[i] = pass ? ((x[i] << 7) + 2048) >> 12 : x[i];
      } else {
        transform_1d<N, false>(x, y, nz);
        const int add = pass ? 2048 : 64, sh = pass ? 12 : 7;
#pragma unroll
        for (int i = 0; i < N; i++) y[i] = clip16((y[i] + add) >> sh);
      }
      __syncwarp();
      if (pass == 0) {
#pragma unroll
        for (int i = 0; i < N; i++) t[i * S + col] = (int16_t)y[i];
      } else {
        int16_t* row = t + col * S;
#pragma unroll
        for (int j = 0; j < N; j += 2)
          *reinterpret_cast<uint32_t*>(row + j) = ((uint32_t)y[j] & 0xffffu) | ((uint32_t)y[j + 1] << 16);
      }
      __syncwarp();
    }
    {
      constexpr int PAIRS = N * N / 2;
      const uint32_t n_active = min((uint32_t)K, count - step * K);
#pragma unroll
      for (int g = 0; g < K; g++) {
        if ((uint32_t)g >= n_active) break;
        uint32_t* dst = reinterpret_cast<uint32_t*>(blk_of[warp][g]);
        const int16_t* src = tmp + g * (N * S);
#pragma unroll 4
        for (int q = lane; q < PAIRS; q += 32) {
          const int r = q / (N / 2), cp = q % (N / 2);
          dst[q] = *reinterpret_cast<const uint32_t*>(src + r * S + 2 * cp);
        }
      }
    }
    __syncwarp();
  }
}

struct DctBytes {
  int8_t m[32][32];
};
constexpr DctBytes make_dct_bytes() {
  DctBytes t{};
  for (int j = 0; j < 32; j++)
    for (int i = 0; i < 32; i++) t.m[j][i] = (int8_t)dct32(j, i);
  return t;
}
__device__ const DctBytes kDctBytes = make_dct_bytes();

__device__ __forceinline__ void mma_k32(int (&d)[4], uint32_t a0, uint32_t a1, uint32_t a2, uint32_t a3, uint32_t b0, uint32_t b1, int a_unsigned,
                                        int b_unsigned) {
  if (b_unsigned)
    asm volatile("mma.sync.aligned.m16n8k32.row.col.s32.s8.u8.s32 {%0,%1,%2,%3}, {%4,%5,%6,%7}, {%8,%9}, {%0,%1,%2,%3};"
                 : "+r"(d[0]), "+r"(d[1]), "+r"(d[2]), "+r"(d[3])
                 : "r"(a0), "r"(a1), "r"(a2), "r"(a3), "r"(b0), "r"(b1));
  else if (a_unsigned)
    asm volatile("mma.sync.aligned.m16n8k32.row.col.s32.u8.s8.s32 {%0,%1,%2,%3}, {%4,%5,%6,%7}, {%8,%9}, {%0,%1,%2,%3};"
                 : "+r"(d[0]), "+r"(d[1]), "+r"(d[2]), "+r"(d[3])
                 : "r"(a0), "r"(a1), "r"(a2), "r"(a3), "r"(b0), "r"(b1));
  else
    asm volatile("mma.sync.aligned.m16n8k32.row.col.s32.s8.s8.s32 {%0,%1,%2,%3}, {%4,%5,%6,%7}, {%8,%9}, {%0,%1,%2,%3};"
                 : "+r"(d[0]), "+r"(d[1]), "+r"(d[2]), "+r"(d[3])
                 : "r"(a0), "r"(a1), "r"(a2), "r"(a3), "r"(b0), "r"(b1));
}
__device__ __forceinline__ void mma_k16(int (&d)[4], uint32_t a0, uint32_t a1, uint32_t b0, int a_unsigned, int b_unsigned) {
  if (b_unsigned)
    asm volatile("mma.sync.aligned.m16n8k16.row.col.s32.s8.u8.s32 {%0,%1,%2,%3}, {%4,%5}, {%6}, {%0,%1,%2,%3};"
                 : "+r"(d[0]), "+r"(d[1]), "+r"(d[2]), "+r"(d[3])
                 : "r"(a0), "r"(a1), "r"(b0));
  else if (a_unsigned)
    asm volatile("mma.sync.aligned.m16n8k16.row.col.s32.u8.s8.s32 {%0,%1,%2,%3}, {%4,%5}, {%6}, {%0,%1,%2,%3};"
                 : "+r"(d[0]), "+r"(d[1]), "+r"(d[2]), "+r"(d[3])
                 : "r"(a0), "r"(a1), "r"(b0));
  else
    asm volatile("mma.sync.aligned.m16n8k16.row.col.s32.s8.s8.s32 {%0,%1,%2,%3}, {%4,%5}, {%6}, {%0,%1,%2,%3};"
                 : "+r"(d[0]), "+r"(d[1]), "+r"(d[2]), "+r"(d[3])
                 : "r"(a0), "r"(a1), "r"(b0));
}
__device__ __forceinline__ uint32_t hi_bytes(uint32_t p01, uint32_t p23) { return __byte_perm(p01, p23, 0x7531); }
__device__ __forceinline__ uint32_t lo_bytes(uint32_t p01, uint32_t p23) { return __byte_perm(p01, p23, 0x6420); }

__device__ __forceinline__ uint32_t sat_pack16(int lo, int hi) {
  uint32_t d;
  asm("cvt.pack.sat.s16.s32 %0, %1, %2;" : "=r"(d) : "r"(hi), "r"(lo));
  return d;
}

template <int BD_SHIFT, bool WIDE, bool TSKIP>
__device__ __forceinline__ uint4 scale_piece(uint4 raw, uint2 mm, int scale) {
  uint32_t w[4] = {raw.x, raw.y, raw.z, raw.w};
#pragma unroll
  for (int k = 0; k < 4; k++) {
    int v2[2];
#pragma unroll
    for (int hh = 0; hh < 2; hh++) {
      const int lvl = hh ? (int)w[k] >> 16 : (int)(int16_t)(w[k] & 0xffffu);
      const int mi = 2 * k + hh;
      const int ms = (int)(((mi < 4 ? mm.x : mm.y) >> (8 * (mi & 3))) & 0xffu) * scale;
      int v;
      if (!WIDE) {
        v = (lvl * ms + (1 << (BD_SHIFT - 1))) >> BD_SHIFT;
      } else {
        long long p = ((long long)lvl * ms + (1ll << (BD_SHIFT - 1))) >> BD_SHIFT;
        v = (int)min(32767ll, max(-32768ll, p));
      }
      if (TSKIP) v = ((clip16(v) << 7) + 2048) >> 12;
      v2[hh] = v;
    }
    w[k] = sat_pack16(v2[0], v2[1]);
  }
  return make_uint4(w[0], w[1], w[2], w[3]);
}
__device__ __forceinline__ bool products_fit(uint32_t mag, int max_ms) { return (32 - __clz(mag)) + (32 - __clz((uint32_t)max_ms)) <= 30; }
__device__ __forceinline__ uint32_t mag_bits(uint32_t w) {
  const int lo = (int)(int16_t)(w & 0xffffu), hi = (int)w >> 16;
  return (uint32_t)(lo ^ (lo >> 31)) | (uint32_t)(hi ^ (hi >> 31));
}

template <int N>
__global__ void __launch_bounds__(kWarpsPerCta * 32, N == 32 ? 4 : 8) transform_mma_kernel(Arenas A, int cls) {
  constexpr int LOG2 = N == 16 ? 4 : 5;
  constexpr int NT = N / 8;
  constexpr int MT = N / 16;
  constexpr int SB = 2 * N + 16;
  constexpr int VEC = N * N / 8 / 32;
  __shared__ __align__(16) unsigned char tile_all[kWarpsPerCta][N * SB];
  const int warp = threadIdx.x >> 5, lane = threadIdx.x & 31;
  const int g = lane >> 2, t = lane & 3;
  const uint32_t count = A.list_count[cls * LIST_COUNT_STRIDE];
  const uint2_t* list = A.tu_list + A.list_off[cls];
  unsigned char* tile = tile_all[warp];
  const uint32_t tile_s = (uint32_t)__cvta_generic_to_shared(tile);
  uint32_t cb[N / 16][NT];
#pragma unroll
  for (int h = 0; h < N / 16; h++)
#pragma unroll
    for (int n = 0; n < NT; n++) {
      uint32_t v = 0;
#pragma unroll
      for (int s4 = 0; s4 < 4; s4++) {
        const int j = 16 * h + 2 * t + (s4 & 1) + 8 * (s4 >> 1);
        v |= (uint32_t)(uint8_t)kDctBytes.m[j * (32 / N)][8 * n + g] << (8 * s4);
      }
      cb[h][n] = v;
    }
  for (uint32_t idx = blockIdx.x * kWarpsPerCta + warp; idx < count; idx += gridDim.x * kWarpsPerCta) {
    const Item item = fetch_item(A, list[idx]);
    uint4* blk = reinterpret_cast<uint4*>(item.blk);
    uint4 raw[VEC];
#pragma unroll
    for (int q = 0; q < VEC; q++) raw[q] = blk[q * 32 + lane];
    const bool tskip = item.tskip != 0;
    uint32_t other = 0, mag = 0;
#pragma unroll
    for (int q = 0; q < VEC; q++) {
      other |= (q == 0 && lane == 0 ? raw[q].x & 0xffff0000u : raw[q].x) | raw[q].y | raw[q].z | raw[q].w;
      mag |= mag_bits(raw[q].x) | mag_bits(raw[q].y) | mag_bits(raw[q].z) | mag_bits(raw[q].w);
    }
    const int scale = item_scale(item);
    const uint8_t* m = nullptr;
    if (item.pp->scaling_enabled && !tskip) {
      const ScalingSet* sc = A.scaling + item.pp->scaling_set;
      m = N == 16 ? sc->f16[item.cidx] : sc->f32[item.cidx];
    }
    constexpr int BD_SHIFT = LOG2 + 3;
    if (!__any_sync(0xffffffffu, other != 0) && !tskip) {
      const int lvl = (int)(int16_t)(__shfl_sync(0xffffffffu, raw[0].x, 0) & 0xffffu);
      const long long p = ((long long)lvl * ((m ? (int)m[0] : 16) * scale) + (1ll << (BD_SHIFT - 1))) >> BD_SHIFT;
      const int dc = (int)min(32767ll, max(-32768ll, p));
      const int t1 = clip16((64 * dc + 64) >> 7);
      const uint32_t vv = ((uint32_t)clip16((64 * t1 + 2048) >> 12) & 0xffffu) * 0x10001u;
#pragma unroll
      for (int q = 0; q < VEC; q++) blk[q * 32 + lane] = make_uint4(vv, vv, vv, vv);
      continue;
    }
    const bool narrow = products_fit(__reduce_or_sync(0xffffffffu, mag), (m ? 255 : 16) * scale);
    if (tskip) {
#pragma unroll
      for (int q = 0; q < VEC; q++) blk[q * 32 + lane] = scale_piece<BD_SHIFT, true, true>(raw[q], make_uint2(0x10101010u, 0x10101010u), scale);
      continue;
    }
#pragma unroll
    for (int q = 0; q < VEC; q++) {
      const int e0 = (q * 32 + lane) * 8;
      uint2 mm = make_uint2(0x10101010u, 0x10101010u);
      if (m) mm = *reinterpret_cast<const uint2*>(m + e0);
      const uint4 sc4 = narrow ? scale_piece<BD_SHIFT, false, false>(raw[q], mm, scale) : scale_piece<BD_SHIFT, true, false>(raw[q], mm, scale);
      *reinterpret_cast<uint4*>(tile + (e0 / N) * SB + (e0 % N) * 2) = sc4;
    }
    __syncwarp();
    int acc[MT][NT][4];
#pragma unroll
    for (int n = 0; n < NT; n++) {
      uint32_t r[4];
      if (N == 32) {
        asm volatile("ldmatrix.sync.aligned.m8n8.x4.trans.shared.b16 {%0,%1,%2,%3}, [%4];"
                     : "=r"(r[0]), "=r"(r[1]), "=r"(r[2]), "=r"(r[3])
                     : "r"(tile_s + (uint32_t)(lane * SB + n * 16)));
      } else {
        asm volatile("ldmatrix.sync.aligned.m8n8.x2.trans.shared.b16 {%0,%1}, [%2];"
                     : "=r"(r[0]), "=r"(r[1])
                     : "r"(tile_s + (uint32_t)((lane & 15) * SB + n * 16)));
        r[2] = r[3] = 0;
      }
      const uint32_t h0 = hi_bytes(r[0], r[1]), l0 = lo_bytes(r[0], r[1]);
      const uint32_t h1 = hi_bytes(r[2], r[3]), l1 = lo_bytes(r[2], r[3]);
#pragma unroll
      for (int mt = 0; mt < MT; mt++) {
#pragma unroll
        for (int k = 0; k < 4; k++) acc[mt][n][k] = 0;
        if (N == 32) {
          mma_k32(acc[mt][n], cb[0][2 * mt], cb[0][2 * mt + 1], cb[1][2 * mt], cb[1][2 * mt + 1], h0, h1, 0, 0);
#pragma unroll
          for (int k = 0; k < 4; k++) acc[mt][n][k] = acc[mt][n][k] * 256 + 64;
          mma_k32(acc[mt][n], cb[0][2 * mt], cb[0][2 * mt + 1], cb[1][2 * mt], cb[1][2 * mt + 1], l0, l1, 0, 1);
        } else {
          mma_k16(acc[mt][n], cb[0][2 * mt], cb[0][2 * mt + 1], h0, 0, 0);
#pragma unroll
          for (int k = 0; k < 4; k++) acc[mt][n][k] = acc[mt][n][k] * 256 + 64;
          mma_k16(acc[mt][n], cb[0][2 * mt], cb[0][2 * mt + 1], l0, 0, 1);
        }
      }
    }
#pragma unroll
    for (int mt = 0; mt < MT; mt++) {
      uint32_t ah[4], al[4];
#pragma unroll
      for (int hf = 0; hf < N / 16; hf++)
#pragma unroll
        for (int up = 0; up < 2; up++) {
          const uint32_t p01 = sat_pack16(acc[mt][2 * hf][2 * up] >> 7, acc[mt][2 * hf][2 * up + 1] >> 7);
          const uint32_t p23 = sat_pack16(acc[mt][2 * hf + 1][2 * up] >> 7, acc[mt][2 * hf + 1][2 * up + 1] >> 7);
          ah[2 * hf + up] = hi_bytes(p01, p23);
          al[2 * hf + up] = lo_bytes(p01, p23);
        }
#pragma unroll
      for (int n = 0; n < NT; n++) {
        int d[4] = {0, 0, 0, 0};
        if (N == 32) {
          mma_k32(d, ah[0], ah[1], ah[2], ah[3], cb[0][n], cb[1][n], 0, 0);
#pragma unroll
          for (int k = 0; k < 4; k++) d[k] = d[k] * 256 + 2048;
          mma_k32(d, al[0], al[1], al[2], al[3], cb[0][n], cb[1][n], 1, 0);
        } else {
          mma_k16(d, ah[0], ah[1], cb[0][n], 0, 0);
#pragma unroll
          for (int k = 0; k < 4; k++) d[k] = d[k] * 256 + 2048;
          mma_k16(d, al[0], al[1], cb[0][n], 1, 0);
        }
        uint32_t* out = reinterpret_cast<uint32_t*>(item.blk);
        out[((16 * mt + g) * N + 8 * n + 2 * t) >> 1] = sat_pack16(d[0] >> 12, d[1] >> 12);
        out[((16 * mt + g + 8) * N + 8 * n + 2 * t) >> 1] = sat_pack16(d[2] >> 12, d[3] >> 12);
      }
    }
    __syncwarp();
  }
}

__global__ void __launch_bounds__(kWarpsPerCta * 32, 8) transform_mma8_kernel(Arenas A, int cls) {
  __shared__ __align__(16) unsigned char tile_all[kWarpsPerCta][4 * 128];
  const int warp = threadIdx.x >> 5, lane = threadIdx.x & 31;
  const int g = lane >> 2, t = lane & 3;
  const uint32_t count = A.list_count[cls * LIST_COUNT_STRIDE];
  const uint2_t* list = A.tu_list + A.list_off[cls];
  unsigned char* tile = tile_all[warp];
  const uint32_t tile_s = (uint32_t)__cvta_generic_to_shared(tile);
  const uint32_t c2 = (uint32_t)(uint8_t)kDctBytes.m[4 * (2 * t)][g] | ((uint32_t)(uint8_t)kDctBytes.m[4 * (2 * t + 1)][g] << 8);
  const uint32_t c_lo = c2, c_hi = c2 << 16;
  const uint32_t steps = (count + 3) / 4;
  const int kb = lane >> 3;
  for (uint32_t step = blockIdx.x * kWarpsPerCta + warp; step < steps; step += gridDim.x * kWarpsPerCta) {
    const uint32_t idx = step * 4 + kb;
    const bool active = idx < count;
    uint2_t it;
    it.x = it.y = 0;
    if (active) it = list[idx];
    const Item item = fetch_item(A, it);
    uint4* row = reinterpret_cast<uint4*>(item.blk) + (lane & 7);
    uint4 raw = make_uint4(0u, 0u, 0u, 0u);
    if (active) raw = *row;
    const int scale = item_scale(item);
    const bool tskip = active && item.tskip;
    uint2 mm = make_uint2(0x10101010u, 0x10101010u);
    if (item.pp->scaling_enabled && !tskip) mm = *reinterpret_cast<const uint2*>((A.scaling + item.pp->scaling_set)->f8[item.cidx] + (lane & 7) * 8);
    const uint32_t mag = mag_bits(raw.x) | mag_bits(raw.y) | mag_bits(raw.z) | mag_bits(raw.w);
    const bool narrow = products_fit(__reduce_or_sync(0xffffffffu, mag), __reduce_max_sync(0xffffffffu, (item.pp->scaling_enabled ? 255 : 16) * scale));
    const bool any_tskip = __any_sync(0xffffffffu, tskip);
    uint4 sc4;
    if (any_tskip) {
      sc4 = tskip ? scale_piece<6, true, true>(raw, mm, scale) : scale_piece<6, true, false>(raw, mm, scale);
      if (tskip) {
        *row = sc4;
        sc4 = make_uint4(0u, 0u, 0u, 0u);
      }
    } else {
      sc4 = narrow ? scale_piece<6, false, false>(raw, mm, scale) : scale_piece<6, true, false>(raw, mm, scale);
    }
    *reinterpret_cast<uint4*>(tile + lane * 16) = sc4;
    __syncwarp();
    uint32_t r[4];
    asm volatile("ldmatrix.sync.aligned.m8n8.x4.trans.shared.b16 {%0,%1,%2,%3}, [%4];"
                 : "=r"(r[0]), "=r"(r[1]), "=r"(r[2]), "=r"(r[3])
                 : "r"(tile_s + (uint32_t)(lane * 16)));
#pragma unroll
    for (int pr = 0; pr < 2; pr++) {
      int acc[4] = {0, 0, 0, 0};
      mma_k16(acc, c_lo, c_hi, hi_bytes(r[2 * pr], r[2 * pr + 1]), 0, 0);
#pragma unroll
      for (int k = 0; k < 4; k++) acc[k] = acc[k] * 256 + 64;
      mma_k16(acc, c_lo, c_hi, lo_bytes(r[2 * pr], r[2 * pr + 1]), 0, 1);
      const uint32_t p0 = sat_pack16(acc[0] >> 7, acc[1] >> 7), p1 = sat_pack16(acc[2] >> 7, acc[3] >> 7);
      int d[4] = {0, 0, 0, 0};
      mma_k16(d, hi_bytes(p0, 0u), hi_bytes(p1, 0u), c_lo, 0, 0);
#pragma unroll
      for (int k = 0; k < 4; k++) d[k] = d[k] * 256 + 2048;
      mma_k16(d, lo_bytes(p0, 0u), lo_bytes(p1, 0u), c_lo, 1, 0);
#pragma unroll
      for (int b2 = 0; b2 < 2; b2++) {
        const int b = 2 * pr + b2;
        const bool b_active = step * 4 + b < count;
        const bool b_tskip = (__ballot_sync(0xffffffffu, tskip) >> (8 * b)) & 1u;
        uint32_t* out = reinterpret_cast<uint32_t*>(__shfl_sync(0xffffffffu, (unsigned long long)item.blk, 8 * b));
        if (b_active && !b_tskip) out[(g * 8 + 2 * t) >> 1] = sat_pack16(d[2 * b2] >> 12, d[2 * b2 + 1] >> 12);
      }
    }
    __syncwarp();
  }
}

__device__ __forceinline__ void idct4(const int (&x)[4], int (&y)[4]) {
  const int e0 = 64 * (x[0] + x[2]), e1 = 64 * (x[0] - x[2]);
  const int o0 = 83 * x[1] + 36 * x[3], o1 = 36 * x[1] - 83 * x[3];
  y[0] = e0 + o0;
  y[1] = e1 + o1;
  y[2] = e1 - o1;
  y[3] = e0 - o0;
}

template <bool DST>
__global__ void __launch_bounds__(256) transform4_kernel(Arenas A, int cls) {
  const uint32_t count = A.list_count[cls * LIST_COUNT_STRIDE];
  const uint2_t* list = A.tu_list + A.list_off[cls];
  for (uint32_t idx = blockIdx.x * blockDim.x + threadIdx.x; idx < count; idx += gridDim.x * blockDim.x) {
    const Item item = fetch_item(A, list[idx]);
    int16_t* blk = item.blk;
    const uint4 in0 = reinterpret_cast<const uint4*>(blk)[0], in1 = reinterpret_cast<const uint4*>(blk)[1];
    const uint32_t raw[8] = {in0.x, in0.y, in0.z, in0.w, in1.x, in1.y, in1.z, in1.w};
    const int scale = item_scale(item);
    uint32_t mraw[4] = {0x10101010u, 0x10101010u, 0x10101010u, 0x10101010u};
    if (item.pp->scaling_enabled) {
      const uint4 mv = *reinterpret_cast<const uint4*>((A.scaling + item.pp->scaling_set)->f4[item.cidx]);
      mraw[0] = mv.x, mraw[1] = mv.y, mraw[2] = mv.z, mraw[3] = mv.w;
    }
    int d[16];
#pragma unroll
    for (int i = 0; i < 16; i++) {
      const int lvl = (int)(int16_t)((raw[i >> 1] >> (16 * (i & 1))) & 0xffffu);
      const int ms = (int)((mraw[i >> 2] >> (8 * (i & 3))) & 0xffu) * scale;
      int v;
      if ((unsigned)(lvl + 255) <= 510u) {
        v = (lvl * ms + 16) >> 5;
      } else {
        long long p = ((long long)lvl * ms + 16) >> 5;
        v = (int)min(32767ll, max(-32768ll, p));
      }
      d[i] = min(32767, max(-32768, v));
    }
    int out[16];
    if (item.tskip) {
#pragma unroll
      for (int i = 0; i < 16; i++) out[i] = ((d[i] << 7) + 2048) >> 12;
    } else {
      int t[16];
#pragma unroll
      for (int cc = 0; cc < 4; cc++) {
        const int x[4] = {d[cc], d[4 + cc], d[8 + cc], d[12 + cc]};
        int y[4];
        if (DST) dst4(x, y);
        else idct4(x, y);
#pragma unroll
        for (int i = 0; i < 4; i++) t[i * 4 + cc] = clip16((y[i] + 64) >> 7);
      }
#pragma unroll
      for (int r = 0; r < 4; r++) {
        const int x[4] = {t[r * 4], t[r * 4 + 1], t[r * 4 + 2], t[r * 4 + 3]};
        int y[4];
        if (DST) dst4(x, y);
        else idct4(x, y);
#pragma unroll
        for (int i = 0; i < 4; i++) out[r * 4 + i] = clip16((y[i] + 2048) >> 12);
      }
    }
    uint32_t pk[8];
#pragma unroll
    for (int i = 0; i < 8; i++) pk[i] = ((uint32_t)out[2 * i] & 0xffffu) | ((uint32_t)out[2 * i + 1] << 16);
    reinterpret_cast<uint4*>(blk)[0] = make_uint4(pk[0], pk[1], pk[2], pk[3]);
    reinterpret_cast<uint4*>(blk)[1] = make_uint4(pk[4], pk[5], pk[6], pk[7]);
  }
}

}

size_t transform_list_layout(size_t total_tu, uint32_t off[LIST_CLASSES]) {
  const size_t cap[LIST_CLASSES] = {total_tu / 64 + 1, total_tu / 16 + total_tu / 32 + 1, total_tu / 4 + total_tu / 8 + 1,
                                    total_tu + 1, total_tu / 2 + 1};
  size_t o = 0;
  for (int k = 0; k < LIST_CLASSES; k++) {
    off[k] = (uint32_t)o;
    o += cap[k];
  }
  return o;
}

cudaError_t launch_transform(const Arenas& A, uint32_t max_tu_per_tile, int max_log2_tb, int n_sm, cudaStream_t stream) {
  if (!A.n_tiles) return cudaSuccess;
  cudaError_t e = cudaMemsetAsync(A.list_count, 0, LIST_CLASSES * LIST_COUNT_STRIDE * sizeof(uint32_t), stream);
  if (e != cudaSuccess) return e;
  const uint32_t bpt = (max_tu_per_tile + kListPerCta - 1) / kListPerCta;
  tu_list_kernel<<<A.n_tiles * bpt, kListThreads, 0, stream>>>(A, bpt);
  const size_t total = (size_t)A.n_tiles * max_tu_per_tile;
  auto grid = [&](size_t max_steps, int resident) {
    return (unsigned)std::max<size_t>(1, std::min<size_t>((max_steps + kWarpsPerCta - 1) / kWarpsPerCta, (size_t)n_sm * resident));
  };
  static const bool use_mma = []() { const char* e = getenv("HEIC_B200_TRANSFORM_MMA"); return !e || atoi(e) != 0; }();
  if (use_mma) {
    if (max_log2_tb >= 5) transform_mma_kernel<32><<<grid(total / 64 + 1, 4), kWarpsPerCta * 32, 0, stream>>>(A, LIST_32);
    if (max_log2_tb >= 4) transform_mma_kernel<16><<<grid(total / 16 + 1, 8), kWarpsPerCta * 32, 0, stream>>>(A, LIST_16);
  } else {
    if (max_log2_tb >= 5) transform_kernel<32><<<grid(total / 64 + 1, 3), kWarpsPerCta * 32, 0, stream>>>(A, LIST_32);
    if (max_log2_tb >= 4) transform_kernel<16><<<grid(total / 32 + 1, 4), kWarpsPerCta * 32, 0, stream>>>(A, LIST_16);
  }
  if (use_mma) transform_mma8_kernel<<<grid(total / 16 + 1, 8), kWarpsPerCta * 32, 0, stream>>>(A, LIST_8);
  else transform_kernel<8><<<grid(total / 16 + 1, 6), kWarpsPerCta * 32, 0, stream>>>(A, LIST_8);
  transform4_kernel<true><<<grid(total / 32 + 1, 8), 256, 0, stream>>>(A, LIST_4Y);
  transform4_kernel<false><<<grid(total / 64 + 1, 8), 256, 0, stream>>>(A, LIST_4C);
  return cudaGetLastError();
}
int transform_launches(int max_log2_tb) { return 4 + (max_log2_tb >= 4 ? 1 : 0) + (max_log2_tb >= 5 ? 1 : 0); }

}
}
```

Measured before the change: 29060.

## Split CABAC into two phases and overlap phase-A reconstruction with phase-B parsing

Tile groups are split per class into phase A (resident CTAs plus a configurable share of the rest) and phase B, with each phase's CABAC launched on its own stream. Reconstruction (transform, intra, deblock, fused SAO) for phase-A tiles runs on a high-priority side stream while phase-B parsing continues. Transform lists, list counters and CTA-group counters are duplicated per phase, and the reconstruction kernels now take a tile-id indirection list. The aim is to hide the serial CABAC tail behind reconstruction work, at the cost of extra launches and of the two phases competing for SMs.

New measurement: 28210 (median of 6 runs). -2.9%, worse.

```diff
diff --git a/heif_b200/csrc/cuda/cabac_kernel.cu b/heif_b200/csrc/cuda/cabac_kernel.cu
--- a/heif_b200/csrc/cuda/cabac_kernel.cu
+++ b/heif_b200/csrc/cuda/cabac_kernel.cu
@@ -185,6 +185,10 @@
   return kCtaSharedBytes + (tiles_per_cta == 32 ? ColdBytes<32>::value : ColdBytes<1>::value) + (size_t)n_slots * NUM_CTX_PAD * tiles_per_cta;
 }
 
+uint32_t cabac_resident_ctas(int n_slots, int n_sm, int resident_ctas) {
+  return resident_ctas > 0 ? (uint32_t)resident_ctas : (uint32_t)n_sm * (uint32_t)(HEIC_CABAC_MIN_CTAS * 8 / n_slots);
+}
+
 cudaError_t launch_cabac(const Arenas& A, const CabacTabs* tabs, const uint32_t* order, uint32_t n_groups,
                          int tiles_per_cta, int n_slots, uint32_t* group_counter, int n_sm, int resident_ctas, cudaStream_t stream) {
   if (!n_groups) return cudaSuccess;
@@ -196,7 +200,7 @@
       cudaError_t e = cudaFuncSetAttribute(cabac_kernel<32>, cudaFuncAttributeMaxDynamicSharedMemorySize, 200 * 1024);
       if (e != cudaSuccess) return e;
     }
-    const uint32_t resident = resident_ctas > 0 ? (uint32_t)resident_ctas : (uint32_t)n_sm * (uint32_t)(HEIC_CABAC_MIN_CTAS * 8 / n_slots);
+    const uint32_t resident = cabac_resident_ctas(n_slots, n_sm, resident_ctas);
     if (group_counter && n_groups > resident && n_groups < 0xffff0u)
       cabac_kernel<32><<<resident, threads, smem, stream>>>(A, tabs, order, n_slots, n_groups, group_counter);
     else
diff --git a/heif_b200/csrc/cuda/deblock_kernel.cu b/heif_b200/csrc/cuda/deblock_kernel.cu
--- a/heif_b200/csrc/cuda/deblock_kernel.cu
+++ b/heif_b200/csrc/cuda/deblock_kernel.cu
@@ -204,8 +204,9 @@
 #define HEIC_DEBLOCK_MIN_CTAS 12
 #endif
 template <int KIND>
-__global__ void __launch_bounds__(128, HEIC_DEBLOCK_MIN_CTAS) deblock_kernel(Arenas A, uint32_t blocks_per_tile) {
-  const uint32_t tile = blockIdx.x / blocks_per_tile;
+__global__ void __launch_bounds__(128, HEIC_DEBLOCK_MIN_CTAS) deblock_kernel(Arenas A, const uint32_t* __restrict__ tile_ids,
+                                                                           uint32_t blocks_per_tile) {
+  const uint32_t tile = tile_ids ? tile_ids[blockIdx.x / blocks_per_tile] : blockIdx.x / blocks_per_tile;
   const TileParams* tp = A.tiles + tile;
   const PicParams* pp = A.pics + tp->pic;
   if (A.status[tile].code != 0 || tp->deblock_disabled) return;
@@ -235,13 +236,14 @@
 
 }
 
-cudaError_t launch_deblock(const Arenas& A, uint32_t max_w, uint32_t max_h, cudaStream_t stream) {
-  if (!A.n_tiles) return cudaSuccess;
+cudaError_t launch_deblock(const Arenas& A, const uint32_t* tile_ids, uint32_t n_tiles, uint32_t max_w, uint32_t max_h,
+                           cudaStream_t stream) {
+  if (!n_tiles) return cudaSuccess;
   const uint32_t cells_y = (((max_w + 7) >> 3) + 1) * (((max_h + 7) >> 3) + 1);
   const uint32_t cells_c = 2 * ((((max_w >> 1) + 7) >> 3) + 1) * ((((max_h >> 1) + 7) >> 3) + 1);
   const uint32_t by = (cells_y + 127) / 128, bc = (cells_c + 127) / 128;
-  deblock_kernel<0><<<A.n_tiles * by, 128, 0, stream>>>(A, by);
-  deblock_kernel<1><<<A.n_tiles * bc, 128, 0, stream>>>(A, bc);
+  deblock_kernel<0><<<n_tiles * by, 128, 0, stream>>>(A, tile_ids, by);
+  deblock_kernel<1><<<n_tiles * bc, 128, 0, stream>>>(A, tile_ids, bc);
   return cudaGetLastError();
 }
 
diff --git a/heif_b200/csrc/cuda/intra_kernel.cu b/heif_b200/csrc/cuda/intra_kernel.cu
--- a/heif_b200/csrc/cuda/intra_kernel.cu
+++ b/heif_b200/csrc/cuda/intra_kernel.cu
@@ -501,16 +501,16 @@
 
 }
 
-cudaError_t launch_intra(const Arenas& A, const uint32_t* order, int max_log2_ctb, int max_hctb, int n_slots, bool clear_coeff,
-                         cudaStream_t stream) {
-  if (!A.n_tiles) return cudaSuccess;
+cudaError_t launch_intra(const Arenas& A, const uint32_t* order, uint32_t n_tiles, int max_log2_ctb, int max_hctb, int n_slots,
+                         bool clear_coeff, cudaStream_t stream) {
+  if (!n_tiles) return cudaSuccess;
   const IntraLayout L = intra_layout(max_log2_ctb);
   const size_t smem = (n_slots > 1 ? (((size_t)max_hctb * 4 + 15) & ~(size_t)15) : 0) + (size_t)n_slots * L.warp_bytes;
   if (smem > 48 * 1024) {
     cudaError_t e = cudaFuncSetAttribute(intra_kernel, cudaFuncAttributeMaxDynamicSharedMemorySize, (int)smem);
     if (e != cudaSuccess) return e;
   }
-  intra_kernel<<<A.n_tiles, 32 * n_slots, smem, stream>>>(A, order, n_slots, L, clear_coeff ? 1 : 0);
+  intra_kernel<<<n_tiles, 32 * n_slots, smem, stream>>>(A, order, n_slots, L, clear_coeff ? 1 : 0);
   return cudaGetLastError();
 }
 
diff --git a/heif_b200/csrc/cuda/kernels.h b/heif_b200/csrc/cuda/kernels.h
--- a/heif_b200/csrc/cuda/kernels.h
+++ b/heif_b200/csrc/cuda/kernels.h
@@ -12,19 +12,22 @@
 cudaError_t launch_cabac(const Arenas& A, const CabacTabs* tabs, const uint32_t* order, uint32_t n_groups,
                          int tiles_per_cta, int n_slots, uint32_t* group_counter, int n_sm, int resident_ctas ,
                          cudaStream_t stream);
+uint32_t cabac_resident_ctas(int n_slots, int n_sm, int resident_ctas);
 
 cudaError_t launch_unescape(const Arenas& A, TileParams* tiles, uint32_t* substreams, cudaStream_t stream);
-cudaError_t launch_transform(const Arenas& A, uint32_t max_tu_per_tile, int max_log2_tb, int n_sm, cudaStream_t stream);
+cudaError_t launch_transform(const Arenas& A, const uint32_t* tile_ids, uint32_t n_tiles, uint32_t max_tu_per_tile, int max_log2_tb,
+                             int n_sm, cudaStream_t stream);
 size_t transform_list_layout(size_t total_tu, uint32_t off[LIST_CLASSES]);
 int transform_launches(int max_log2_tb);
 
-cudaError_t launch_intra(const Arenas& A, const uint32_t* order, int max_log2_ctb, int max_hctb, int n_slots, bool clear_coeff,
-                         cudaStream_t stream);
+cudaError_t launch_intra(const Arenas& A, const uint32_t* order, uint32_t n_tiles, int max_log2_ctb, int max_hctb, int n_slots,
+                         bool clear_coeff, cudaStream_t stream);
 
-cudaError_t launch_deblock(const Arenas& A, uint32_t max_w, uint32_t max_h, cudaStream_t stream);
+cudaError_t launch_deblock(const Arenas& A, const uint32_t* tile_ids, uint32_t n_tiles, uint32_t max_w, uint32_t max_h,
+                           cudaStream_t stream);
 
 cudaError_t launch_sao(const Arenas& A, uint32_t max_pitch, uint32_t max_h, cudaStream_t stream);
-cudaError_t launch_sao_sparse(const Arenas& A, int max_hctb, cudaStream_t stream);
+cudaError_t launch_sao_sparse(const Arenas& A, const uint32_t* tile_ids, uint32_t n_tiles, int max_hctb, cudaStream_t stream);
 
 struct ColorJob {
   const uint8_t* planes;
diff --git a/heif_b200/csrc/cuda/phase_split.h b/heif_b200/csrc/cuda/phase_split.h
--- /dev/null
+++ b/heif_b200/csrc/cuda/phase_split.h
@@ -0,0 +1,37 @@
+#pragma once
+#include <stdint.h>
+
+#include <vector>
+
+namespace heic {
+
+struct CabacClass {
+  int n_slots, hctb;
+  uint32_t order_off, n_groups, n_tiles;
+  uint32_t n_groups_a;
+};
+
+inline uint32_t phase_a_groups(uint32_t n_groups, uint32_t resident, int split_pct) {
+  if (n_groups <= resident || split_pct >= 100) return n_groups;
+  const uint32_t extra = (uint32_t)((uint64_t)(n_groups - resident) * (uint32_t)(split_pct < 0 ? 0 : split_pct) / 100u);
+  return resident + (extra < n_groups - resident ? extra : n_groups - resident - 1);
+}
+
+inline bool phase_tile_orders(const std::vector<CabacClass>& classes, const std::vector<uint32_t>& order, int tiles_per_group,
+                              const std::vector<uint32_t>& heavy_first, std::vector<uint32_t> phase[2]) {
+  phase[0].clear();
+  phase[1].clear();
+  std::vector<uint8_t> in_b(heavy_first.size(), 0);
+  bool split = false;
+  for (const CabacClass& c : classes) {
+    if (c.n_groups_a >= c.n_groups) continue;
+    split = true;
+    const size_t first = c.order_off + (size_t)c.n_groups_a * tiles_per_group, end = c.order_off + (size_t)c.n_groups * tiles_per_group;
+    for (size_t i = first; i < end; i++)
+      if (order[i] != 0xffffffffu) in_b[order[i]] = 1;
+  }
+  for (uint32_t t : heavy_first) phase[in_b[t]].push_back(t);
+  return split;
+}
+
+}
diff --git a/heif_b200/csrc/cuda/pipeline.cu b/heif_b200/csrc/cuda/pipeline.cu
--- a/heif_b200/csrc/cuda/pipeline.cu
+++ b/heif_b200/csrc/cuda/pipeline.cu
@@ -18,6 +18,7 @@
 #include "cabac_tables.h"
 #include "host_params.h"
 #include "kernels.h"
+#include "phase_split.h"
 
 using namespace heic;
 using namespace heic::dev;
@@ -109,6 +110,8 @@
   int cabac_resident = 0;
   int cabac_persistent = 1;
   int fuse_sao = 1;
+  int overlap = 1;
+  int overlap_split = 50;
   static constexpr int kPipe = 16;
   int pipe_chunk = 0;
   int pipe_slots = 0;
@@ -176,11 +179,6 @@
 
 }
 
-struct CabacClass {
-  int n_slots, hctb;
-  uint32_t order_off, n_groups, n_tiles;
-};
-
 struct heic_b200_batch {
   heic_b200_ctx* ctx = nullptr;
   cudaStream_t stream = nullptr;
@@ -191,6 +189,13 @@
   std::vector<ImageInfo> images;
   std::vector<uint32_t> substreams, order, heavy_first;
   std::vector<CabacClass> classes;
+  bool split = false;
+  std::vector<uint32_t> phase_order[2];
+  size_t phase_tu[2] = {};
+  uint32_t phase_list_off[2][LIST_CLASSES] = {};
+  cudaStream_t side = nullptr;
+  cudaEvent_t ev_fork = nullptr, ev_join = nullptr;
+  cudaEvent_t ev_trace[6] = {};
   size_t raw_bytes = 0;
   bool any_plain = false;
   size_t bs_bytes = 0, tu_words = 0, coeff_elems = 0, plane_bytes = 0, map4_bytes = 0, map8_bytes = 0, sao_words = 0, wpp_bytes = 0;
@@ -201,7 +206,7 @@
   bool final_stale = false;
   bool coeff_clean = false;
   PinnedBuf h_bitstream, h_status, h_params;
-  size_t off_sub = 0, off_order = 0, off_heavy = 0, off_pics = 0, off_tiles = 0, off_scaling = 0;
+  size_t off_sub = 0, off_order = 0, off_heavy = 0, off_phase[2] = {}, off_pics = 0, off_tiles = 0, off_scaling = 0;
   DevBuf d_bitstream, d_params, d_tu, d_coeff, d_recon, d_final, d_ipm, d_ctd,
       d_qp, d_sao, d_wpp, d_status, d_rgb, d_list, d_list_count, d_raw, d_counters;
   PinnedBuf h_raw;
@@ -231,9 +236,26 @@
     for (int k = 0; k < LIST_CLASSES; k++) a.list_off[k] = list_off[k];
     return a;
   }
+  Arenas phase_arenas(int p) const {
+    Arenas a = arenas();
+    a.list_count += (size_t)p * LIST_CLASSES * LIST_COUNT_STRIDE;
+    for (int k = 0; k < LIST_CLASSES; k++) a.list_off[k] = phase_list_off[p][k];
+    return a;
+  }
+  const uint32_t* dev_params(size_t off) const { return (const uint32_t*)((const uint8_t*)d_params.p + off); }
   void load(const heic_image_desc* imgs, const heic_image_transform* xforms, uint32_t n_imgs, bool with_rgb);
   void run(uint32_t mask);
+  void reconstruct(const Arenas& A, const uint32_t* ids, uint32_t n, uint32_t mask, bool fuse, cudaStream_t st);
+  ~heic_b200_batch();
 };
+
+heic_b200_batch::~heic_b200_batch() {
+  for (cudaEvent_t e : ev_trace)
+    if (e) cudaEventDestroy(e);
+  if (ev_fork) cudaEventDestroy(ev_fork);
+  if (ev_join) cudaEventDestroy(ev_join);
+  if (side) cudaStreamDestroy(side);
+}
 
 heic_b200_ctx::~heic_b200_ctx() {
   if (trace_base) cudaEventDestroy(trace_base);
@@ -258,6 +280,7 @@
   order.clear();
   heavy_first.clear();
   classes.clear();
+  split = false;
   raw_bytes = 0;
   any_plain = false;
   bs_bytes = tu_words = coeff_elems = plane_bytes = map4_bytes = map8_bytes = sao_words = wpp_bytes = 0;
@@ -465,12 +488,20 @@
     }
     c.hctb = hctb;
     c.n_tiles = (uint32_t)v.size();
+    c.n_groups_a = c.n_groups;
+    if (ctx->overlap && tpc == 32)
+      c.n_groups_a = phase_a_groups(c.n_groups, cabac_resident_ctas(c.n_slots, ctx->n_sm, ctx->cabac_resident), ctx->overlap_split);
     classes.push_back(c);
   }
 
   heavy_first.resize(tiles.size());
   for (uint32_t t = 0; t < tiles.size(); t++) heavy_first[t] = t;
   std::stable_sort(heavy_first.begin(), heavy_first.end(), [&](uint32_t a, uint32_t b) { return tiles[a].bs_len > tiles[b].bs_len; });
+  split = phase_tile_orders(classes, order, tpc, heavy_first, phase_order);
+  for (int p = 0; p < 2; p++) {
+    phase_tu[p] = 0;
+    for (uint32_t t : phase_order[p]) phase_tu[p] += (size_t)pics[tiles[t].pic].n_tu;
+  }
 
   cudaStream_t st = stream;
   if (any_plain) h_bitstream.ensure(bs_bytes + 16);
@@ -496,7 +527,9 @@
   off_sub = 0;
   off_order = up(off_sub + substreams.size() * 4, 256);
   off_heavy = up(off_order + order.size() * 4, 256);
-  off_pics = up(off_heavy + heavy_first.size() * 4, 256);
+  off_phase[0] = up(off_heavy + heavy_first.size() * 4, 256);
+  off_phase[1] = up(off_phase[0] + phase_order[0].size() * 4, 256);
+  off_pics = up(off_phase[1] + phase_order[1].size() * 4, 256);
   off_tiles = up(off_pics + pics.size() * sizeof(PicParams), 256);
   off_scaling = up(off_tiles + tiles.size() * sizeof(TileParams), 256);
   const size_t params_bytes = up(off_scaling + scaling.size() * sizeof(ScalingSet), 256);
@@ -506,6 +539,7 @@
     std::memcpy(hp + off_sub, substreams.data(), substreams.size() * 4);
     std::memcpy(hp + off_order, order.data(), order.size() * 4);
     std::memcpy(hp + off_heavy, heavy_first.data(), heavy_first.size() * 4);
+    for (int p = 0; p < 2; p++) std::memcpy(hp + off_phase[p], phase_order[p].data(), phase_order[p].size() * 4);
     std::memcpy(hp + off_pics, pics.data(), pics.size() * sizeof(PicParams));
     std::memcpy(hp + off_tiles, tiles.data(), tiles.size() * sizeof(TileParams));
     std::memcpy(hp + off_scaling, scaling.data(), scaling.size() * sizeof(ScalingSet));
@@ -514,8 +548,15 @@
   d_params.ensure(params_bytes);
   d_tu.ensure(tu_words * 4);
   if (tu_words >= (1ull << 31)) bail(HEIC_E_UNSUPPORTED, "batch too large: more than 2^31 4x4 blocks in one load");
-  d_list.ensure(transform_list_layout(tu_words, list_off) * sizeof(uint2_t));
-  d_list_count.ensure(LIST_CLASSES * LIST_COUNT_STRIDE * sizeof(uint32_t));
+  size_t list_elems = transform_list_layout(tu_words, list_off);
+  if (split) {
+    const size_t n_a = transform_list_layout(phase_tu[0], phase_list_off[0]);
+    const size_t n_b = transform_list_layout(phase_tu[1], phase_list_off[1]);
+    for (int k = 0; k < LIST_CLASSES; k++) phase_list_off[1][k] += (uint32_t)n_a;
+    list_elems = std::max(list_elems, n_a + n_b);
+  }
+  d_list.ensure(list_elems * sizeof(uint2_t));
+  d_list_count.ensure(2 * LIST_CLASSES * LIST_COUNT_STRIDE * sizeof(uint32_t));
   if (coeff_elems * 2 > d_coeff.cap) coeff_clean = false;
   d_coeff.ensure(coeff_elems * 2);
   d_recon.ensure(plane_bytes);
@@ -534,10 +575,46 @@
   CU(cudaMemcpyAsync(d_params.p, h_params.p, params_bytes, cudaMemcpyHostToDevice, st));
 }
 
+void heic_b200_batch::reconstruct(const Arenas& A, const uint32_t* ids, uint32_t n, uint32_t mask, bool fuse, cudaStream_t st) {
+  if (mask & HEIC_STAGE_TRANSFORM) {
+    CU(launch_transform(A, ids, n, max_tu, max_log2_tb, ctx->n_sm, st));
+    ctx->launches += transform_launches(max_log2_tb);
+  }
+  if (mask & HEIC_STAGE_INTRA) {
+    int slots = tiles.size() >= (size_t)ctx->intra_single_warp_tiles ? 1 : intra_slots;
+    if (ctx->intra_slots > 0) slots = std::min(ctx->intra_slots, std::max(1, max_hctb));
+    CU(launch_intra(A, ids ? ids : dev_params(off_heavy), n, max_log2_ctb, max_hctb, slots, true, st));
+    ctx->launches++;
+  }
+  if (mask & HEIC_STAGE_DEBLOCK) {
+    CU(launch_deblock(A, ids, n, max_w, max_h, st));
+    ctx->launches += 2;
+  }
+  if (fuse) {
+    CU(launch_sao_sparse(A, ids, n, max_hctb, st));
+    ctx->launches++;
+  }
+}
+
 void heic_b200_batch::run(uint32_t mask) {
   cudaStream_t st = stream;
   const Arenas A = arenas();
   if (!A.n_tiles) return;
+  const bool overlap = mask == HEIC_STAGE_ALL && split && ctx->overlap;
+  const bool fuse = ctx->fuse_sao && (mask & HEIC_STAGE_SAO) && (mask & HEIC_STAGE_COLOR) && d_rgb.p;
+  static const bool trace2 = std::getenv("HEIC_B200_TRACE") && std::atoi(std::getenv("HEIC_B200_TRACE")) >= 2;
+  const bool trace = trace2 && mask == HEIC_STAGE_ALL;
+  if (trace)
+    for (cudaEvent_t& e : ev_trace)
+      if (!e) CU(cudaEventCreate(&e));
+  if (trace) CU(cudaEventRecord(ev_trace[0], st));
+  if (overlap && !side) {
+    int least = 0, greatest = 0;
+    CU(cudaDeviceGetStreamPriorityRange(&least, &greatest));
+    CU(cudaStreamCreateWithPriority(&side, cudaStreamNonBlocking, greatest));
+    CU(cudaEventCreateWithFlags(&ev_fork, cudaEventDisableTiming));
+    CU(cudaEventCreateWithFlags(&ev_join, cudaEventDisableTiming));
+  }
   if (mask & HEIC_STAGE_CABAC) {
     CU(cudaMemsetAsync(d_tu.p, 0, tu_words * 4, st));
     if (!coeff_clean) CU(cudaMemsetAsync(d_coeff.p, 0, coeff_elems * 2, st));
@@ -549,44 +626,45 @@
       CU(launch_unescape(A, (TileParams*)(pb + off_tiles), (uint32_t*)(pb + off_sub), st));
       ctx->launches++;
     }
-    constexpr size_t kCounters = 64;
-    d_counters.ensure(kCounters * sizeof(uint32_t));
-    const bool persistent = ctx->cabac_persistent && classes.size() <= kCounters;
-    if (persistent) CU(cudaMemsetAsync(d_counters.p, 0, kCounters * sizeof(uint32_t), st));
-    size_t ci = 0;
-    for (const CabacClass& c : classes) {
-      CU(launch_cabac(A, ctx->d_tabs, (const uint32_t*)((const uint8_t*)d_params.p + off_order) + c.order_off, c.n_groups, tiles_per_cta,
-                      c.n_slots, (persistent && c.hctb > c.n_slots) ? (uint32_t*)d_counters.p + ci : nullptr, ctx->n_sm, ctx->cabac_resident, st));
-      ctx->launches++;
-      ci++;
-    }
-  }
-  if (mask & HEIC_STAGE_TRANSFORM) {
-    CU(launch_transform(A, max_tu, max_log2_tb, ctx->n_sm, st));
-    ctx->launches += transform_launches(max_log2_tb);
-  }
-  if (mask & HEIC_STAGE_INTRA) {
-    int slots = tiles.size() >= (size_t)ctx->intra_single_warp_tiles ? 1 : intra_slots;
-    if (ctx->intra_slots > 0) slots = std::min(ctx->intra_slots, std::max(1, max_hctb));
-    CU(launch_intra(A, (const uint32_t*)((const uint8_t*)d_params.p + off_heavy), max_log2_ctb, max_hctb, slots, true, st));
-    coeff_clean = true;
-    ctx->launches++;
-  }
-  if (mask & HEIC_STAGE_DEBLOCK) {
-    CU(launch_deblock(A, max_w, max_h, st));
-    ctx->launches += 2;
-  }
-  const bool fuse = ctx->fuse_sao && (mask & HEIC_STAGE_SAO) && (mask & HEIC_STAGE_COLOR) && d_rgb.p;
+    constexpr size_t kClassCounters = 64;
+    d_counters.ensure(2 * kClassCounters * sizeof(uint32_t));
+    const bool persistent = ctx->cabac_persistent && classes.size() <= kClassCounters;
+    if (persistent) CU(cudaMemsetAsync(d_counters.p, 0, 2 * kClassCounters * sizeof(uint32_t), st));
+    if (overlap) {
+      CU(cudaEventRecord(ev_fork, st));
+      CU(cudaStreamWaitEvent(side, ev_fork, 0));
+    }
+    for (int phase = 0; phase < (overlap ? 2 : 1); phase++) {
+      size_t ci = 0;
+      for (const CabacClass& c : classes) {
+        const uint32_t g0 = phase ? c.n_groups_a : 0, n = overlap ? (phase ? c.n_groups - c.n_groups_a : c.n_groups_a) : c.n_groups;
+        uint32_t* counter = (persistent && c.hctb > c.n_slots) ? (uint32_t*)d_counters.p + phase * kClassCounters + ci : nullptr;
+        CU(launch_cabac(A, ctx->d_tabs, dev_params(off_order) + c.order_off + (size_t)g0 * tiles_per_cta, n, tiles_per_cta, c.n_slots,
+                        counter, ctx->n_sm, ctx->cabac_resident, overlap && !phase ? side : st));
+        if (n) ctx->launches++;
+        ci++;
+      }
+      if (trace) CU(cudaEventRecord(ev_trace[1 + phase], overlap && !phase ? side : st));
+    }
+  }
+  if (overlap) {
+    reconstruct(phase_arenas(0), dev_params(off_phase[0]), (uint32_t)phase_order[0].size(), mask, fuse, side);
+    if (trace) CU(cudaEventRecord(ev_trace[3], side));
+    CU(cudaEventRecord(ev_join, side));
+    reconstruct(phase_arenas(1), dev_params(off_phase[1]), (uint32_t)phase_order[1].size(), mask, fuse, st);
+    if (trace) CU(cudaEventRecord(ev_trace[4], st));
+    CU(cudaStreamWaitEvent(st, ev_join, 0));
+  } else {
+    reconstruct(A, nullptr, A.n_tiles, mask, fuse, st);
+    if (trace) CU(cudaEventRecord(ev_trace[3], st));
+  }
+  if (mask & HEIC_STAGE_INTRA) coeff_clean = true;
   if ((mask & HEIC_STAGE_SAO) && !fuse) {
     CU(launch_sao(A, max_pitch, max_h, st));
     final_stale = false;
     ctx->launches++;
   }
-  if (fuse) {
-    CU(launch_sao_sparse(A, max_hctb, st));
-    ctx->launches++;
-    final_stale = true;
-  }
+  if (fuse) final_stale = true;
   if ((mask & HEIC_STAGE_COLOR) && d_rgb.p) {
     size_t i = 0;
     while (i < images.size()) {
@@ -637,6 +715,18 @@
     }
   }
   stages_run |= mask;
+  if (trace) {
+    CU(cudaEventRecord(ev_trace[5], st));
+    CU(cudaEventSynchronize(ev_trace[5]));
+    float t[6] = {};
+    for (int k = 1; k < 6; k++)
+      if ((k != 2 && k != 4) || overlap) CU(cudaEventElapsedTime(&t[k], ev_trace[0], ev_trace[k]));
+    if (overlap)
+      std::fprintf(stderr, "[heic_b200] resident decode, %zu + %zu tiles: cabac A %8.2f  cabac B %8.2f  recon A %8.2f  recon B %8.2f  done %8.2f ms\n",
+                   phase_order[0].size(), phase_order[1].size(), t[1], t[2], t[3], t[4], t[5]);
+    else
+      std::fprintf(stderr, "[heic_b200] resident decode, %zu tiles: cabac %8.2f  recon %8.2f  done %8.2f ms\n", tiles.size(), t[1], t[3], t[5]);
+  }
 }
 
 namespace {
@@ -688,6 +778,8 @@
     c->pipe_chunk = std::max(0, env_int("HEIC_B200_PIPE_CHUNK", 0));
     c->low_latency_tiles = env_int("HEIC_B200_LOW_LATENCY_TILES", 384);
     c->fuse_sao = env_int("HEIC_B200_FUSE_SAO", 1) != 0;
+    c->overlap = env_int("HEIC_B200_OVERLAP", c->overlap) != 0;
+    c->overlap_split = std::min(100, std::max(0, env_int("HEIC_B200_OVERLAP_SPLIT", c->overlap_split)));
     c->cabac_persistent = env_int("HEIC_B200_CABAC_PERSISTENT", 1) != 0;
     c->cabac_resident = std::max(0, env_int("HEIC_B200_CABAC_RESIDENT", 0));
     c->cabac_plain_sort = env_int("HEIC_B200_CABAC_PLAIN_SORT", 0) != 0;
diff --git a/heif_b200/csrc/cuda/sao_kernel.cu b/heif_b200/csrc/cuda/sao_kernel.cu
--- a/heif_b200/csrc/cuda/sao_kernel.cu
+++ b/heif_b200/csrc/cuda/sao_kernel.cu
@@ -60,8 +60,8 @@
   }
 }
 
-__global__ void __launch_bounds__(128) sao_sparse_kernel(Arenas A, uint32_t max_hctb) {
-  const uint32_t tile = blockIdx.x / max_hctb, ry = blockIdx.x % max_hctb;
+__global__ void __launch_bounds__(128) sao_sparse_kernel(Arenas A, const uint32_t* __restrict__ tile_ids, uint32_t max_hctb) {
+  const uint32_t tile = tile_ids ? tile_ids[blockIdx.x / max_hctb] : blockIdx.x / max_hctb, ry = blockIdx.x % max_hctb;
   const TileParams* tp = A.tiles + tile;
   const PicParams* pp = A.pics + tp->pic;
   if (A.status[tile].code != 0 || ry >= (uint32_t)pp->hctb) return;
@@ -98,9 +98,9 @@
 
 }
 
-cudaError_t launch_sao_sparse(const Arenas& A, int max_hctb, cudaStream_t stream) {
-  if (!A.n_tiles || max_hctb <= 0) return cudaSuccess;
-  sao_sparse_kernel<<<A.n_tiles * (uint32_t)max_hctb, 128, 0, stream>>>(A, (uint32_t)max_hctb);
+cudaError_t launch_sao_sparse(const Arenas& A, const uint32_t* tile_ids, uint32_t n_tiles, int max_hctb, cudaStream_t stream) {
+  if (!n_tiles || max_hctb <= 0) return cudaSuccess;
+  sao_sparse_kernel<<<n_tiles * (uint32_t)max_hctb, 128, 0, stream>>>(A, tile_ids, (uint32_t)max_hctb);
   return cudaGetLastError();
 }
 
diff --git a/heif_b200/csrc/cuda/transform_kernel.cu b/heif_b200/csrc/cuda/transform_kernel.cu
--- a/heif_b200/csrc/cuda/transform_kernel.cu
+++ b/heif_b200/csrc/cuda/transform_kernel.cu
@@ -100,9 +100,10 @@
 #ifndef HEIC_LIST_MIN_CTAS
 #define HEIC_LIST_MIN_CTAS 1
 #endif
-__global__ void __launch_bounds__(kListThreads, HEIC_LIST_MIN_CTAS) tu_list_kernel(Arenas A, uint32_t blocks_per_tile) {
+__global__ void __launch_bounds__(kListThreads, HEIC_LIST_MIN_CTAS) tu_list_kernel(Arenas A, const uint32_t* __restrict__ tile_ids,
+                                                                                      uint32_t blocks_per_tile) {
   __shared__ uint32_t cta_cnt[LIST_CLASSES], cta_base[LIST_CLASSES], warp_base[kListThreads / 32][LIST_CLASSES];
-  const uint32_t tile = blockIdx.x / blocks_per_tile;
+  const uint32_t tile = tile_ids ? tile_ids[blockIdx.x / blocks_per_tile] : blockIdx.x / blocks_per_tile;
   const uint32_t first = (blockIdx.x % blocks_per_tile) * kListPerCta;
   const TileParams* tp = A.tiles + tile;
   const PicParams* pp = A.pics + tp->pic;
@@ -732,13 +733,14 @@
   return o;
 }
 
-cudaError_t launch_transform(const Arenas& A, uint32_t max_tu_per_tile, int max_log2_tb, int n_sm, cudaStream_t stream) {
-  if (!A.n_tiles) return cudaSuccess;
+cudaError_t launch_transform(const Arenas& A, const uint32_t* tile_ids, uint32_t n_tiles, uint32_t max_tu_per_tile, int max_log2_tb,
+                             int n_sm, cudaStream_t stream) {
+  if (!n_tiles) return cudaSuccess;
   cudaError_t e = cudaMemsetAsync(A.list_count, 0, LIST_CLASSES * LIST_COUNT_STRIDE * sizeof(uint32_t), stream);
   if (e != cudaSuccess) return e;
   const uint32_t bpt = (max_tu_per_tile + kListPerCta - 1) / kListPerCta;
-  tu_list_kernel<<<A.n_tiles * bpt, kListThreads, 0, stream>>>(A, bpt);
-  const size_t total = (size_t)A.n_tiles * max_tu_per_tile;
+  tu_list_kernel<<<n_tiles * bpt, kListThreads, 0, stream>>>(A, tile_ids, bpt);
+  const size_t total = (size_t)n_tiles * max_tu_per_tile;
   auto grid = [&](size_t max_steps, int resident) {
     return (unsigned)std::max<size_t>(1, std::min<size_t>((max_steps + kWarpsPerCta - 1) / kWarpsPerCta, (size_t)n_sm * resident));
   };
```
